# mims-harvard/SubGNN

Measured on AMD Instinct MI355X. Metric: subgraphs/sec fwd+bwd (all 3 channels on) + achieved HBM GB/s, higher is better.
Workload: dtype f32; 1 GPU; synthetic DENSITY-style BA base graph n=1000000 m=10 (9998512 undirected edges), 50000 BFS subgraphs x 20 nodes per GPU (weak form; BASELINE configs[3] "50k sharded across 8" as worded is --scaling strong), all_density hparams (N 10/43, P 57/183, S 42, 1 layer), D=64, full pass = sampling + similarities + fwd + bwd + Adam; subgraphs_per_gpu=50000, subgraphs_total=50000

## Files before the change

### include/subgnn_hip.h

```cpp
#ifndef SUBGNN_HIP_H
#define SUBGNN_HIP_H

#include <stdint.h>

#ifdef __cplusplus
extern "C" {
#endif

#define SGNN_OK                  0
#define SGNN_ERR_BAD_ARG        -1
#define SGNN_ERR_SET_TOO_LARGE  -2
#define SGNN_ERR_NNZ_TOO_LARGE  -3
#define SGNN_ERR_LAUNCH         -4
#define SGNN_ERR_UNSUPPORTED_D  -5

#define SGNN_ABI_VERSION 12
int sgnn_abi_version(void);
int sgnn_warm_up(void* stream);
const char* sgnn_last_error(void);

int sgnn_degree_sequence(const int64_t* rowptr, const int32_t* col, int64_t nnz,
                         const int32_t* full_degree, const uint8_t* self_loops,
                         const int64_t* set_ptr, const int32_t* set_nodes, int64_t n_sets,
                         int64_t max_set_size, int sorted,
// ... 25 lines not shown
                   int32_t* out_nodes, int32_t* out_pos, void* stream);
int sgnn_cc_compact_stats(const int64_t* sub_ptr, const int32_t* sub_nodes, const int32_t* labels,
                          int64_t n_subgraphs, int64_t max_sub_len, int32_t* out_n_components,
                          int32_t* out_longest, void* stream);
int sgnn_cc_compact(const int64_t* sub_ptr, const int32_t* sub_nodes, const int32_t* labels,
                    int64_t n_subgraphs, int64_t max_sub_len, int64_t C, int64_t L, int64_t* out, void* stream);
int64_t sgnn_cc_huge_workspace_bytes(int64_t total_nodes);
int sgnn_cc_labels_huge(const int64_t* rowptr, const int32_t* col, int64_t nnz, const int64_t* sub_ptr,
                        const int32_t* sub_nodes, int64_t n_subgraphs, int64_t total_nodes, int32_t* out_label,
                        void* workspace, int64_t workspace_bytes, void* stream);
int sgnn_cc_compact_huge(const int64_t* sub_ptr, const int32_t* sub_nodes, const int32_t* labels,
                         int64_t n_subgraphs, int64_t total_nodes, int write, int64_t C, int64_t L,
                         int32_t* out_n_components, int32_t* out_longest, int64_t* out, void* workspace,
                         int64_t workspace_bytes, void* stream);

int64_t sgnn_subgraph_properties_workspace_bytes(int64_t total_nodes);
int sgnn_subgraph_properties(const int64_t* rowptr, const int32_t* col_sorted, int64_t nnz, int64_t max_id, int rows_simple,
                             const int64_t* sub_ptr, const int32_t* sub_nodes, int64_t n_sets, int64_t max_len,
                             int64_t total_nodes, int64_t* out_counts, int32_t* out_core, void* workspace,
                             int64_t workspace_bytes, void* stream);

int64_t sgnn_khop_border_workspace_bytes(int64_t max_id, int64_t n_sets, int bitmap_in_lds);
int sgnn_khop_border_bitmap_fits_lds(int64_t max_id);
int sgnn_khop_border(const int64_t* rowptr, const int32_t* col, int64_t nnz, int64_t max_id,
                     const int64_t* set_ptr, const int32_t* set_nodes, int64_t n_sets,
                     int k, int ego_dict_mode,
                     int64_t* out_count, const int64_t* out_ptr, int32_t* out_nodes, uint8_t* out_hop,
                     void* workspace, int64_t workspace_bytes, int bitmap_in_lds, void* stream);
int sgnn_khop_border_arena(const int64_t* rowptr, const int32_t* col, int64_t nnz, int64_t max_id,
                           const int64_t* set_ptr, const int32_t* set_nodes, int64_t n_sets, int k,
                           const int64_t* arena_off, int32_t* arena, int64_t* out_count,
                           void* workspace, int64_t workspace_bytes, int bitmap_in_lds, void* stream);
int64_t sgnn_khop_border_sample_workspace_bytes(int64_t max_id, int64_t n_sets, int k, int rows_sorted, int bitmap_in_lds);
int sgnn_khop_border_sample(const int64_t* rowptr, const int32_t* col, const int32_t* col_sorted, int64_t nnz, int64_t max_id,
                            const int64_t* set_ptr, const int32_t* set_nodes, int64_t n_sets, int k,
                            int64_t n_slots, uint64_t seed, uint64_t stream_id, int64_t item_base,
                            int64_t* out_anchor, uint8_t* out_hop, uint8_t* out_allneg, int64_t* out_count,
                            const int32_t* set_order ,
                            void* workspace, int64_t workspace_bytes, int bitmap_in_lds, void* stream);
int sgnn_khop_sample_finish(int64_t* anchor, const uint8_t* hop, const uint8_t* allneg, const int64_t* counts,
                            const int64_t* width, int64_t n_sets, int64_t n_slots, float* sims, void* stream);
int sgnn_khop1_border_sorted(const int64_t* rowptr, const int32_t* col, const int32_t* col_sorted, int64_t nnz, int64_t max_id,
                             const int64_t* set_ptr, const int32_t* set_nodes, int64_t n_sets,
                             int64_t* out_count, const int64_t* out_ptr , int32_t* out_ids ,
                             void* workspace, int64_t workspace_bytes, int bitmap_in_lds, void* stream);

int sgnn_first_occurrence_mask(const int64_t* ids, int64_t n_rows, int64_t row_len, uint8_t* keep, void* stream);
int sgnn_filter_sets(const int64_t* set_ptr, const int32_t* set_nodes, const uint8_t* flags, int64_t n_sets, int64_t* counts,
                     const int64_t* out_ptr, int32_t* out_nodes, void* stream);
int sgnn_pack_rows_count(const int64_t* ids, const uint8_t* mask, int64_t n_rows, int64_t row_len, int64_t* counts,
                         void* stream);
int sgnn_pack_rows_write(const int64_t* ids, const uint8_t* mask, int64_t n_rows, int64_t row_len, const int64_t* ptr,
                         int32_t* nodes, void* stream);
int64_t sgnn_pack_fused_max_rows(void);
int64_t sgnn_pack_fused_max_entries(void);
int sgnn_pack_rows_fused(const int64_t* ids, const uint8_t* mask, int mode, int64_t n_rows, int64_t row_len, int64_t* ptr,
                         int32_t* nodes, void* stream);
int sgnn_filter_sets_fused(const int64_t* set_ptr, const int32_t* set_nodes, const uint8_t* flags, int64_t n_sets,
                           int64_t arena_entries, int64_t* out_ptr, int32_t* out_nodes, void* stream);

int sgnn_sample_anchors_padded(const int64_t* ids, int64_t n_rows, int64_t L, int64_t n_slots,
                               uint64_t seed, uint64_t stream_id, int64_t* out, void* stream);
int sgnn_sample_anchors_ragged(const int64_t* set_ptr, const int32_t* set_nodes, int64_t n_sets,
                               const uint8_t* row_has_pad, int64_t n_slots,
                               uint64_t seed, uint64_t stream_id, int64_t item_base, int64_t* out, void* stream);
int sgnn_sample_border_anchors(const int64_t* ptr, const int32_t* ids, const int64_t* counts, int64_t n_sets,
                               const int64_t* width, int64_t n_slots, uint64_t seed, uint64_t stream_id, int64_t item_base,
                               int hop, int64_t* out_anchor, float* out_sims, void* stream);

int sgnn_choice_ragged(const int64_t* ptr, const int32_t* seq, int64_t n_items, int64_t n_draws,
                       uint64_t seed, uint64_t stream_id, int64_t item_base, int64_t* out, void* stream);

int sgnn_set_keys(const int64_t* set_ptr, const int32_t* set_nodes, int64_t n_sets, uint64_t* out_keys, void* stream);
int sgnn_sample_anchors_ragged_keyed(const int64_t* set_ptr, const int32_t* set_nodes, int64_t n_sets,
                                     const uint8_t* row_has_pad, const uint64_t* keys, int64_t n_slots,
                                     uint64_t seed, uint64_t stream_id, int64_t* out, void* stream);
int sgnn_choice_ragged_keyed(const int64_t* ptr, const int32_t* seq, int64_t n_items, const uint64_t* keys, int64_t n_draws,
                             uint64_t seed, uint64_t stream_id, int64_t* out, void* stream);
int sgnn_sample_border_anchors_keyed(const int64_t* ptr, const int32_t* ids, const uint8_t* hops, int64_t n_sets,
                                     const uint8_t* row_has_pad, const uint64_t* keys, int64_t n_slots, uint64_t seed,
                                     uint64_t stream_id, int64_t* out_anchor, float* out_sims, void* stream);

#define SGNN_OCC_NODE 0
#define SGNN_OCC_COMPONENT 1
int64_t sgnn_occlusion_lds_max(void);
int64_t sgnn_occlusion_workspace_bytes(int64_t total_entries);
int sgnn_occlusion_count(const int64_t* set_ptr, const int32_t* set_nodes, int64_t n_sets, int64_t max_set_len, int mode,
                         const int32_t* labels, int64_t* out_units, int64_t* out_variants, int64_t* out_len,
                         int64_t total_entries, void* workspace, int64_t workspace_bytes, void* stream);
int sgnn_occlusion_write(const int64_t* set_ptr, const int32_t* set_nodes, int64_t n_sets, int64_t max_set_len, int mode,
                         const int32_t* labels, const int64_t* var_ptr, const int64_t* len_scan, int64_t n_variants,
                         int64_t* out_ptr, int32_t* out_nodes, int32_t* out_parent, int32_t* out_unit, uint64_t* out_keys,
                         int64_t total_entries, void* workspace, int64_t workspace_bytes, void* stream);

int sgnn_triangular_walks(const int64_t* rowptr, const int32_t* col, const int32_t* col_sorted, int64_t nnz,
                          const int32_t* node_order, int64_t n_nodes,
                          const int64_t* patch_ptr, const int32_t* patch_nodes,
                          const int64_t* inb_ptr, const int32_t* inb_nodes,
                          int mode, int64_t n_items, int64_t walks_per_patch, int64_t walk_len, double beta,
                          uint64_t seed, uint64_t stream_id, int64_t item_base, int64_t max_id, int kernel, int64_t* out,
                          void* stream);
int sgnn_triangular_walks_both(const int64_t* rowptr, const int32_t* col, const int32_t* col_sorted, int64_t nnz,
                               const int64_t* patch_ptr, const int32_t* patch_nodes, const int64_t* inb_ptr,
                               const int32_t* inb_nodes, int64_t n_items, int64_t walks_per_patch, int64_t walk_len,
                               double beta, uint64_t seed, uint64_t stream_id_int, uint64_t stream_id_bor,
                               int64_t item_base, int64_t max_id, int64_t* out, void* stream);

int sgnn_patch_in_border(const int64_t* rowptr, const int32_t* col, int64_t nnz,
                         const int32_t* node_order, const int32_t* node_pos, int64_t n_nodes,
                         const int64_t* patch_ptr, const int32_t* patch_nodes, int64_t n_patches,
                         uint8_t* out_flag, void* stream);
int64_t sgnn_patch_in_border_huge_workspace_bytes(int64_t total_nodes);
int sgnn_patch_in_border_huge(const int64_t* rowptr, const int32_t* col, int64_t nnz,
                              const int32_t* node_order, const int32_t* node_pos, int64_t n_nodes,
                              const int64_t* patch_ptr, const int32_t* patch_nodes, int64_t n_patches,
                              int64_t total_nodes, uint8_t* out_flag, void* workspace, int64_t workspace_bytes,
                              void* stream);

int sgnn_sp_similarity_dense(const double* apsp, int64_t n_cols,
                             const int64_t* set_ptr, const int32_t* set_nodes, int64_t n_sets,
                             float* out, void* stream);
int64_t sgnn_bfs_hops_workspace_bytes(int64_t max_id, int64_t n_sources, int max_hops);
int sgnn_bfs_hops(const int64_t* rowptr, const int32_t* col, int64_t nnz, int64_t max_id,
                  const int32_t* sources, int64_t n_sources, int max_hops, int node_major, int pull_alpha,
                  uint8_t* dist, void* workspace, int64_t workspace_bytes, void* stream);
int sgnn_min_hops_to_sets(const uint8_t* dist, int64_t n_sources, int64_t max_id, int node_major,
                          const int64_t* set_ptr, const int32_t* set_nodes, int64_t n_sets,
                          float* out, void* stream);
int64_t sgnn_bfs_min_hops_workspace_bytes(int64_t max_id, int64_t n_sources, int max_hops, int64_t n_sets);
int sgnn_bfs_min_hops_to_sets(const int64_t* rowptr, const int32_t* col, int64_t nnz, int64_t max_id,
                              const int32_t* sources, int64_t n_sources, int max_hops, int pull_alpha, int push_levels,
                              const int64_t* set_ptr, const int32_t* set_nodes, int64_t n_sets,
                              float* out, int32_t* out_status, void* workspace, int64_t workspace_bytes, void* stream);
int64_t sgnn_graph_component_labels_workspace_bytes(int64_t max_id);
int sgnn_graph_component_labels(const int64_t* rowptr, const int32_t* col, int64_t nnz, int64_t max_id,
                                int32_t* labels, void* workspace, int64_t workspace_bytes, void* stream);
int64_t sgnn_bfs_min_hops_closing_workspace_bytes(int64_t max_id, int64_t n_sources, int max_hops, int64_t n_sets);
int sgnn_bfs_min_hops_to_sets_closing(const int64_t* rowptr, const int32_t* col, int64_t nnz, int64_t max_id,
                                      const int32_t* sources, int64_t n_sources, int max_hops, int pull_alpha, int push_levels,
                                      const int32_t* labels, const int64_t* set_ptr, const int32_t* set_nodes,
                                      int64_t n_sets, float* out, int32_t* out_status, void* workspace, int64_t workspace_bytes,
                                      void* stream);

int sgnn_dtw_order_keys(const int64_t* x_ptr, const int32_t* x_val, int64_t n_x, int64_t* out_keys, void* stream);
int64_t sgnn_dtw_workspace_bytes(int64_t n_x, int64_t max_x_len, int64_t n_y, int64_t max_y_len);
int sgnn_dtw_similarity(const int64_t* x_ptr, const int32_t* x_val, int64_t n_x, int64_t max_x_len,
                        const int64_t* y_ptr, const int32_t* y_val, int64_t n_y, int64_t max_y_len,
                        int tie_order, int kernel, const int32_t* x_order, float* out, void* workspace,
                        int64_t workspace_bytes, void* stream);
int sgnn_dtw_similarity_live(const int64_t* x_ptr, const int32_t* x_val, int64_t n_x, int64_t max_x_len,
                             const int64_t* y_ptr, const int32_t* y_val, int64_t n_y, int64_t max_y_len,
                             int tie_order, int kernel, const int32_t* x_order, const int64_t* x_live_range, float* out,
                             void* workspace, int64_t workspace_bytes, void* stream);

int64_t sgnn_dtw_exact_workspace_bytes(int64_t n_x, int64_t max_x_len, int64_t n_y, int64_t max_y_len);
int sgnn_dtw_exact_similarity(const int64_t* x_ptr, const int32_t* x_val, int64_t n_x, int64_t max_x_len,
                              const int64_t* y_ptr, const int32_t* y_val, int64_t n_y, int64_t max_y_len,
                              int kernel, const int32_t* x_order, float* out, void* workspace,
                              int64_t workspace_bytes, void* stream);
int sgnn_dtw_exact_similarity_live(const int64_t* x_ptr, const int32_t* x_val, int64_t n_x, int64_t max_x_len,
                                   const int64_t* y_ptr, const int32_t* y_val, int64_t n_y, int64_t max_y_len,
                                   int kernel, const int32_t* x_order, const int64_t* x_live_range, float* out,
                                   void* workspace, int64_t workspace_bytes, void* stream);

#define SGNN_TOPK_DOT    0
#define SGNN_TOPK_COSINE 1
#define SGNN_TOPK_L2     2
int64_t sgnn_topk_max_k(void);
int64_t sgnn_topk_rows_workspace_bytes(int64_t Q, int64_t N, int64_t k, int64_t splits);
int sgnn_topk_rows(const float* q, int64_t q_stride, int64_t Q, const float* bank, int64_t b_stride, int64_t N,
                   int64_t D, int64_t k, int metric, const float* q_aux, const float* b_aux, const int64_t* exclude,
                   int64_t splits, float* out_score, int64_t* out_index, void* workspace, int64_t workspace_bytes,
                   void* stream);

int sgnn_cc_embed_fwd(const float* E, int64_t D,
                      const int64_t* set_ptr, const int32_t* set_nodes, int64_t n_sets,
                      int aggregator, int64_t padded_len, float* out, int32_t* out_arg, void* stream);
int sgnn_cc_embed_fwd_f16(const uint16_t* E_half, int64_t D,
                          const int64_t* set_ptr, const int32_t* set_nodes, int64_t n_sets,
                          int aggregator, int64_t padded_len, float* out, int32_t* out_arg, void* stream);
int sgnn_cc_embed_bwd(const float* grad_out, int64_t D,
                      const int64_t* set_ptr, const int32_t* set_nodes, int64_t n_sets,
                      int aggregator, const int32_t* arg, float* grad_E, void* stream);

#define SGNN_SRC_DENSE  0
#define SGNN_SRC_GATHER 1
#define SGNN_SRC_SHARED 2

typedef struct sgnn_mpn_args {
    int32_t src;
    int32_t sims_per_edge;
    int64_t R, A, D;
    const float*   x;
    const int64_t* ids;
    int64_t        id_div;
    const uint8_t* edge_mask;
    const uint8_t* row_mask;
    const float*   sims;
    int64_t        sims_ld;
    const int64_t* sim_col;
    const float*   wp;
    const float*   bp;
    int32_t        x_f16;
    const float*   z_act;
    int32_t        flags;
} sgnn_mpn_args;
#define SGNN_MPN_WP_PARTIAL 1
#define SGNN_MPN_RELU_Z     2

int sgnn_mpn_fwd_chunks(const sgnn_mpn_args* args);
int sgnn_mpn_fwd(const sgnn_mpn_args* args, float* agg , float* z , void* stream);
int64_t sgnn_mpn_fwd_many_max_bodies(void);
int sgnn_mpn_fwd_many(int64_t n, const sgnn_mpn_args* args, float* const* agg, float* const* z, void* stream);
int sgnn_mpn_bwd(const sgnn_mpn_args* args, const float* grad_agg, const float* grad_z,
                 float* grad_x, float* grad_wp, void* stream);

int sgnn_attn_scores_epilogue(const float* XU, const float* qW, const float* v, int64_t R, int64_t H,
                              int64_t rows_per_batch, float* out, void* stream);
int64_t sgnn_attn_scores_f16_workspace_bytes(int64_t H);
int sgnn_attn_scores_fwd_f16(const float* X, const float* U, const float* qW, const float* v,
                             int64_t R, int64_t H, int64_t rows_per_batch, float* out,
                             void* workspace, int64_t workspace_bytes, void* stream);

int sgnn_lstm_supported(int64_t hidden_size);
int sgnn_lstm_fwd(const float* pre_x, const float* whh_f, const float* whh_r, const float* bhh_f, const float* bhh_r,
                  int64_t B, int64_t T, int64_t hidden_size, float* y, float* gates, float* cell, float* hprev, void* stream);
int sgnn_lstm_bwd(const float* whh_f, const float* whh_r, const float* gates, const float* cell, const float* dy,
                  int64_t B, int64_t T, int64_t hidden_size, float* dgates, void* stream);

int sgnn_rows_gemm(const float* X, const int64_t* ids, int64_t ldx, int64_t R, int64_t K, const float* W0, const float* W1,
                   const float* b0, const float* b1, int64_t N, float* out, float* x_copy, void* stream);
int sgnn_rows_gemm_nt(const float* A, int64_t R, int64_t K, const float* W0, const float* W1, int64_t N, float* out, void* stream);
int sgnn_lstm_tail_fwd(const float* y, int64_t n_patches, int64_t n_walks, int64_t T, int64_t H2, int last_only,
                       const float* W_lin, const float* b_lin, int64_t D, float* s_out, float* X, void* stream);
int sgnn_lstm_tail_bwd(const float* dX, const float* s, int64_t n_patches, int64_t n_walks, int64_t T, int64_t H2,
                       int last_only, const float* W_lin, int64_t D, float* dy, float* dW_lin, float* db_lin, void* stream);

int sgnn_masked_sum_fwd(const float* x, const uint8_t* mask, int64_t B, int64_t C, int64_t H,
                        float* out, void* stream);
int sgnn_masked_sum_bwd(const float* grad_out, const uint8_t* mask, int64_t B, int64_t C, int64_t H,
                        float* grad_x, void* stream);

int sgnn_masked_sum_slot_fwd(const float* x, const uint8_t* mask, int64_t B, int64_t C, int64_t W, float* out,
                             int64_t out_ld, void* stream);
int sgnn_masked_sum_slot_bwd(const float* grad_out, int64_t grad_ld, const uint8_t* mask, int64_t B, int64_t C,
                             int64_t W, float* grad_x, void* stream);
int sgnn_masked_sum_slots_fwd(const float* const* xs, const int64_t* widths, const int64_t* offsets, int64_t n_pieces,
                              const uint8_t* mask, int64_t B, int64_t C, float* out, int64_t out_ld, void* stream);
int sgnn_masked_sum_slots_bwd(const float* grad_out, int64_t grad_ld, const uint8_t* mask, int64_t B, int64_t C,
                              float* const* grad_xs, const int64_t* widths, const int64_t* offsets, int64_t n_pieces, void* stream);

int64_t sgnn_cross_entropy_workspace_bytes(int64_t B);
int sgnn_cross_entropy_fwd(const float* logits, const int64_t* labels, int64_t B, int64_t K, float* lse, float* loss,
                           float* accuracy, void* workspace, int64_t workspace_bytes, void* stream);
int sgnn_cross_entropy_bwd(const float* logits, const int64_t* labels, const float* lse, const float* grad_loss,
                           int64_t B, int64_t K, float* grad_logits, void* stream);

int64_t sgnn_bce_logits_workspace_bytes(int64_t B);
int sgnn_bce_logits_fwd(const float* logits, const int64_t* targets, int64_t B, int64_t K, float* loss, float* accuracy,
                        void* workspace, int64_t workspace_bytes, void* stream);
int sgnn_bce_logits_bwd(const float* logits, const int64_t* targets, const float* grad_loss, int64_t B, int64_t K,
                        float* grad_logits, void* stream);

int64_t sgnn_column_sum_workspace_bytes(int64_t R, int64_t A);
int sgnn_column_sum(const float* x, int64_t ld, int64_t R, int64_t A, float* out, void* workspace, int64_t workspace_bytes,
                    void* stream);

int sgnn_readout_sum_fwd(const float* sims, int64_t sims_ld, const int64_t* sim_col, const float* s, const float* bp,
                         const uint8_t* row_mask, int64_t B, int64_t C, int64_t A, float* out, int64_t out_ld,
                         void* stream);
int64_t sgnn_readout_sum_bwd_workspace_bytes(int64_t B, int64_t C, int64_t A);
int sgnn_readout_sum_bwd(const float* grad_out, int64_t grad_ld, const float* sims, int64_t sims_ld,
                         const int64_t* sim_col, const float* s, const float* bp, const uint8_t* row_mask, int64_t B,
                         int64_t C, int64_t A, float* grad_s, float* grad_bp, void* workspace, int64_t workspace_bytes,
                         void* stream);

int64_t sgnn_readout_many_max(void);
int sgnn_readout_many_fwd(int64_t n, const float* const* sims, const int64_t* sims_ld, const int64_t* const* sim_col,
                          const float* const* X, const float* const* wp, const float* const* bp,
                          const int64_t* const* ids, const uint8_t* const* row_mask, float* const* s, const int64_t* A,
                          const int64_t* off, int64_t D, int64_t B, int64_t C, float* out, int64_t out_ld, void* stream);
int64_t sgnn_readout_many_bwd_workspace_bytes(int64_t n, const int64_t* A, int64_t B, int64_t C);
int sgnn_readout_many_bwd(int64_t n, const float* grad_out, int64_t grad_ld, const float* const* sims, const int64_t* sims_ld,
                          const int64_t* const* sim_col, const float* const* X, const float* const* wp,
                          const float* const* bp, const int64_t* const* ids, const uint8_t* const* row_mask,
                          float* const* s, const int64_t* A, const int64_t* off, int64_t D, int64_t B, int64_t C,
                          float* const* grad_X, float* const* grad_wp, float* const* grad_bp, void* workspace,
                          int64_t workspace_bytes, unsigned* tickets, void* stream);

int64_t sgnn_scatter_add_rows_workspace_bytes(int64_t n_edges, int64_t D);
int64_t sgnn_sort_edges_by_key_workspace_bytes(int64_t n_edges, int64_t max_key);
int sgnn_sort_edges_by_key(const int32_t* keys, int64_t n_edges, int64_t max_key, int32_t* key_sorted, int32_t* order,
                           void* workspace, int64_t workspace_bytes, void* stream);
int sgnn_scatter_add_rows_sorted(const int32_t* order, const int32_t* key_sorted, int64_t n_edges,
                                 const int32_t* edge_row, int64_t edges_per_row,
                                 const float* G, int64_t D, const float* c1, const float* c2, const float* v,
                                 const int32_t* arg, float* table,
                                 void* workspace, int64_t workspace_bytes, void* stream);
int64_t sgnn_scatter_add_rows_multi_workspace_bytes(int64_t total_edges, int64_t D, int64_t max_key);
int sgnn_scatter_add_rows_multi(int64_t n_lists, const int32_t* const* keys, const int64_t* n_edges,
                                const int32_t* const* edge_row, const int64_t* edges_per_row, const float* const* G,
                                const float* const* c1, const float* const* c2, const float* const* v, int64_t D,
                                int64_t max_key, float* table, void* workspace, int64_t workspace_bytes, void* stream);
int64_t sgnn_mpn_bwd_shared_det_workspace_bytes(int64_t R, int64_t A, int64_t D);
int sgnn_mpn_bwd_shared_det(const struct sgnn_mpn_args* args, const float* grad_agg, const float* grad_z,
                            float* grad_x, float* grad_wp, float* grad_bp, void* workspace, int64_t workspace_bytes,
                            void* stream);
int sgnn_mpn_bwd_edges(const struct sgnn_mpn_args* args, const float* grad_z, int32_t* out_keys, float* out_c1,
                       float* out_c2, void* stream);
int sgnn_mpn_bwd_wp_partial(const struct sgnn_mpn_args* args, const float* grad_z, float* partial, int64_t partial_ld,
                            void* stream);
int sgnn_mpn_bwd_edges_many(int64_t n, const struct sgnn_mpn_args* args, const float* const* grad_z, int32_t* const* out_keys,
                            float* const* out_c1, float* const* out_c2, void* stream);

int sgnn_update_fwd(const float* x, const float* aggr, const float* W, const float* b, int64_t R, int64_t D,
                    float* out, void* stream);
// ... 88 lines not shown
```

### subgnn_amd/SubGNN.py

```python
import json
import os
from pathlib import Path

import numpy as np
import torch
import torch.nn as nn
import torch.nn.functional as F
from torch.nn.parameter import Parameter

from . import config, gamma, ops, subgraph_utils
from . import anchor_patch_samplers as aps
from .datasets import SubgraphDataset
from .graph import load_graph
from .subgraph_mpn import SG_MPN

CHANNELS = (('neighborhood', 'N', 'use_neighborhood', 'neighborhood_mpns'),
            ('position', 'P', 'use_position', 'position_mpns'),
            ('structure', 'S', 'use_structure', 'structure_mpns'))
CC_SLOTS = ('N_I', 'N_B', 'S_I', 'S_B', 'P_I', 'P_B')


class LSTM(nn.Module):

    def __init__(self, n_features, h, dropout=0.0, num_layers=1, batch_first=True, aggregator='last'):
# ... 4 lines not shown
        self.lstm = nn.LSTM(n_features, h, num_layers=num_layers, batch_first=batch_first, dropout=dropout,
                            bidirectional=True)
        self.linear = nn.Linear(h * 2, n_features)

    def _fused(self, input):
        m = self.lstm
        out = input
        for l in range(self.num_layers):
            params = [getattr(m, '%s_l%d%s' % (n, l, sfx)) for sfx in ('', '_reverse')
                      for n in ('weight_ih', 'weight_hh', 'bias_ih', 'bias_hh')]
            out = ops.bilstm_layer(out, params)
            if l < self.num_layers - 1 and m.dropout > 0 and self.training:
                out = nn.functional.dropout(out, m.dropout, True)
        return out

    def forward_walks(self, table, walk_ids, n_walks):
        m = self.lstm
        if not (table.is_cuda and table.dtype == torch.float32 and m.batch_first and m.bias and walk_ids.dim() == 2
                and getattr(table, '_sgnn_half', None) is None and table.shape[1] == m.input_size
                and ops.lstm_fused_supported(m.input_size, m.hidden_size) and walk_ids.shape[0] % n_walks == 0):
            return None
        out = None
        for l in range(self.num_layers):
            params = [getattr(m, '%s_l%d%s' % (n, l, sfx)) for sfx in ('', '_reverse')
                      for n in ('weight_ih', 'weight_hh', 'bias_ih', 'bias_hh')]
            out = ops.bilstm_layer_fused(table, params, ids=walk_ids) if l == 0 else ops.bilstm_layer_fused(out, params)
            if l < self.num_layers - 1 and m.dropout > 0 and self.training:
                out = nn.functional.dropout(out, m.dropout, True)
        return ops.lstm_tail(out, self.linear.weight, self.linear.bias, n_walks, self.aggregator == 'last')

    def forward(self, input):
        m = self.lstm
        if (input.is_cuda and input.dtype == torch.float32 and m.batch_first and m.bias and input.dim() == 3
                and ops.lstm_supported(m.input_size, m.hidden_size)):
            out = self._fused(input)
        else:
            out, _ = m(input)
        agg = out[:, -1, :] if self.aggregator == 'last' else out.sum(dim=1)
        return self.linear(agg)


class _DeviceLoader:

    def __init__(self, model, split, batch_size, shuffle, drop_last):
        self.m, self.split, self.bs, self.shuffle, self.drop_last = model, split, batch_size, shuffle, drop_last
        self.n = len(getattr(model, split + '_sub_G'))

    def __len__(self):
        return self.n // self.bs if self.drop_last else (self.n + self.bs - 1) // self.bs

    def index_batches(self):
        order = torch.randperm(self.n) if self.shuffle else torch.arange(self.n)
        for i in range(len(self)):
            yield order[i * self.bs:(i + 1) * self.bs]

    def __iter__(self):
        for idx in self.index_batches():
            yield self.m.make_batch(self.split, idx)


def _save_npy(fname, arr):
    fname = Path(fname)
    tmp = fname.with_name('.%s.%d.tmp' % (fname.name, os.getpid()))
    try:
        with open(tmp, 'wb') as f:
            np.save(f, arr)
        os.replace(tmp, fname)
    finally:
        if tmp.exists():
            tmp.unlink()


class SubGNN(nn.Module):
    def __init__(self, hparams, graph_path, subgraph_path, embedding_path, similarities_path, shortest_paths_path,
                 degree_dict_path, ego_graph_path, _memory=None):
        super().__init__()
        self._memory = _memory
        self.device = torch.device('cuda' if torch.cuda.is_available() else 'cpu')
        self.hparams = hparams
        self.graph_path, self.subgraph_path, self.embedding_path = graph_path, subgraph_path, embedding_path
        self.similarities_path = Path(similarities_path)
        self.shortest_paths_path, self.degree_dict_path, self.ego_graph_path = \
            shortest_paths_path, degree_dict_path, ego_graph_path
        self.read_data()

        hp = self.hparams
        D, nl = hp['node_embed_size'], hp['n_layers']
        hid_dim = D
        for channel, tag, flag, attr in CHANNELS:
            layers = nn.ModuleList()
            if hp[flag]:
                if tag == 'N':
                    hid_dim += nl * 2 * D
                elif tag == 'P':
                    hid_dim += (hp['n_anchor_patches_pos_in'] + hp['n_anchor_patches_pos_out']) * nl
                else:
                    hid_dim += 2 * hp['n_anchor_patches_structure'] * nl
                for _ in range(nl):
                    layer = nn.ModuleDict({'internal': SG_MPN(hp), 'border': SG_MPN(hp)})
                    if hp.get('batch_norm', False):
                        layer['batch_norm'] = nn.BatchNorm1d(D)
                        layer['batch_norm_out'] = nn.BatchNorm1d(D)
                    layers.append(layer)
            setattr(self, attr, layers)
        self.hid_dim = hid_dim
        self.lin = nn.Linear(hid_dim, hp['linear_hidden_dim_1'])
        self.lin2 = nn.Linear(hp['linear_hidden_dim_1'], hp['linear_hidden_dim_2'])
        self.lin3 = nn.Linear(hp['linear_hidden_dim_2'], self.num_classes)
        self.lin_dropout = nn.Dropout(p=hp['lin_dropout'])
        self.lin_dropout2 = nn.Dropout(p=hp['lin_dropout'])
        self.loss = nn.BCEWithLogitsLoss() if self.multilabel else nn.CrossEntropyLoss()
        self.lstm = LSTM(D, D, dropout=hp['lstm_dropout'], num_layers=hp['lstm_n_layers'],
                         aggregator=hp['lstm_aggregator'])
        if hp.get('ff_attn', False):
            from .attention import AdditiveAttention
            self.attn_vector = Parameter(torch.zeros((hid_dim, 1), dtype=torch.float))
            nn.init.xavier_uniform_(self.attn_vector)
            self.attention = AdditiveAttention(hid_dim, hid_dim, half_operands=str(hp.get('embedding_dtype', 'fp32')).lower()
                                               in ('fp16', 'float16', 'half'))
        hp.setdefault('structure_similarity_fn', 'dtw')
        hp.setdefault('dtw_tie_order', config.DTW_TIE_ORDER)
        if hp['dtw_tie_order'] not in (0, 1, 2):
            raise ValueError("hparams['dtw_tie_order'] must be 0, 1 or 2")
        self._deterministic = bool(hp.get('deterministic', True))
        self.metric_scores = []
        self.to(self.device)
        self.warm_up_s = ops.warm_up(self.device) if (self.device.type == 'cuda' and hp.get('warm_up', True)) else 0.0

    def read_data(self):
        if self._memory is not None:
            return self._read_memory(self._memory)
        root = Path(config.PROJECT_ROOT)
        self.networkx_graph = load_graph(root / self.graph_path, self.device, root / self.degree_dict_path)
        (self.train_sub_G, self.train_sub_G_label, self.val_sub_G, self.val_sub_G_label, self.test_sub_G,
         self.test_sub_G_label) = subgraph_utils.read_subgraphs(root / self.subgraph_path)
        self.multilabel = isinstance(self.train_sub_G_label, list)
        self.multilabel_binarizer = None
        if self.multilabel:
            from sklearn.preprocessing import MultiLabelBinarizer
            self.multilabel_binarizer = MultiLabelBinarizer().fit(
                self.train_sub_G_label + self.val_sub_G_label + self.test_sub_G_label)
        if self.hparams.get('subset_data', False):
            bs = self.hparams['batch_size']
            for sp in ('train', 'val', 'test'):
                setattr(self, sp + '_sub_G', getattr(self, sp + '_sub_G')[:bs])
                setattr(self, sp + '_sub_G_label', getattr(self, sp + '_sub_G_label')[:bs])
        if self.multilabel:
            self.num_classes = max(max(l) for l in self.train_sub_G_label + self.val_sub_G_label + self.test_sub_G_label) + 1
        else:
            self.num_classes = int(torch.max(torch.cat((self.train_sub_G_label.view(-1), self.val_sub_G_label.view(-1),
                                                        self.test_sub_G_label.view(-1))))) + 1
        for sp in ('train', 'val', 'test'):
            setattr(self, sp + '_sub_G', [[n + 1 for n in sg] for sg in getattr(self, sp + '_sub_G')])
        pre = torch.load(root / self.embedding_path, map_location='cpu')
        self.hparams['node_embed_size'] = pre.shape[1]
        table = torch.cat((torch.zeros(1, pre.shape[1]), pre.float()), 0)
        self.node_embeddings = nn.Embedding.from_pretrained(table, freeze=self.hparams['freeze_node_embeds'],
                                                            padding_idx=config.PAD_VALUE)

    def _read_memory(self, mem):
        self.networkx_graph = mem['graph']
        for sp in ('train', 'val', 'test'):
            setattr(self, sp + '_sub_G', mem['sub_G'].get(sp, []))
            setattr(self, sp + '_sub_G_label', mem['labels'].get(sp, torch.zeros(0, dtype=torch.int64)))
        self.multilabel, self.multilabel_binarizer = False, None
        self.num_classes = mem.get('num_classes') or int(max(int(l.max()) for l in mem['labels'].values() if l.numel() > 0)) + 1
        pre = mem['embeddings']
        self.hparams['node_embed_size'] = pre.shape[1]
        table = torch.cat((torch.zeros(1, pre.shape[1], device=pre.device), pre.float()), 0)
        self.node_embeddings = nn.Embedding.from_pretrained(table, freeze=self.hparams['freeze_node_embeds'],
                                                            padding_idx=config.PAD_VALUE)

    @classmethod
    def from_memory(cls, hparams, graph, sub_G, labels, embeddings, num_classes=None):
        return cls(hparams, None, None, None, 'similarities', None, None, None,
                   _memory=dict(graph=graph, sub_G=sub_G, labels=labels, embeddings=embeddings, num_classes=num_classes))

    def initialize_cc_ids(self, subgraph_ids):
        subs = ops.Ragged.from_lists(subgraph_ids, self.device)
        labels = ops.cc_labels(self.networkx_graph, subs)
        return subgraph_utils.components_from_labels(subs.ptr, subs.nodes, labels, subs.max_len)

    def _half_table(self):
        if str(self.hparams.get('embedding_dtype', 'fp32')).lower() not in ('fp16', 'float16', 'half'):
            return None
        w = self.node_embeddings.weight
        st = self.__dict__.get('_half_state')
        if st is None or st[1].device != w.device or st[1].shape != w.shape:
            st = self.__dict__['_half_state'] = [None, torch.empty(w.shape, dtype=torch.float16, device=w.device), True]
        capturing = w.is_cuda and torch.cuda.is_current_stream_capturing()
        training_read = torch.is_grad_enabled() and w.requires_grad
        if st[2] or st[0] != w._version or capturing or training_read:
            st[1].copy_(w.detach())
            st[0] = w._version
        st[2] = training_read or capturing
        return st[1]

    def invalidate_half_table(self):
        st = self.__dict__.get('_half_state')
        if st is not None:
            st[2] = True

    def _table(self):
        t = self.__dict__.get('_tapped_table')
        if t is not None:
            return t
        half = self._half_table()
        return self.node_embeddings.weight if half is None else ops.tap_table(self.node_embeddings.weight, half)

    def initialize_cc_embeddings(self, cc_id_list, aggregator='sum'):
        S, C, L = cc_id_list.shape
        ids = getattr(cc_id_list, '_sgnn_ids32', None)
        if ids is None or ids.numel() != S * C * L:
            ids = cc_id_list.to(self.device).reshape(S * C * L).to(torch.int32)
        memo = self.__dict__.setdefault('_fixed_stride_ptr', {})
        ptr = memo.get((S * C, L))
        if ptr is None:
            if len(memo) > 64:
                memo.clear()
            ptr = memo[(S * C, L)] = torch.arange(S * C + 1, dtype=torch.int64, device=self.device) * L
        sets = ops.Ragged(ptr, ids.contiguous() if ids.numel() else torch.zeros(1, dtype=torch.int32, device=self.device),
                          max_len=L)
        pre = getattr(cc_id_list, '_sgnn_member_order', None)
        if pre is not None and pre[0].numel() != ids.numel():
            pre = None
        return ops.cc_embed(self._table(), sets, aggregator, padded_len=0, stride=L, presorted=pre).view(S, C, -1)

    def initialize_channel_embeddings(self, cc_embeddings, trainable=False):
        if trainable:
            return tuple(Parameter(cc_embeddings.detach().clone()) for _ in CC_SLOTS)
        return tuple(cc_embeddings for _ in CC_SLOTS)

    def init_all_embeddings(self, split='all', trainable=False, lazy=False):
        which = {'all': ('train', 'val', 'test'), 'train_val': ('train', 'val')}.get(split, (split,))
        pending = self.__dict__.setdefault('_lazy_cc_embed', set())
        for sp in which:
            if lazy and not (trainable and sp == 'train'):
                for nm in CC_SLOTS:
                    self.__dict__.pop('%s_%s_cc_embed' % (sp, nm), None)
                pending.add(sp)
                continue
            pending.discard(sp)
            with torch.no_grad():
                emb = self.initialize_cc_embeddings(getattr(self, sp + '_cc_ids'), self.hparams['cc_aggregator'])
            six = self.initialize_channel_embeddings(emb, trainable and sp == 'train')
            for nm, t in zip(CC_SLOTS, six):
                setattr(self, '%s_%s_cc_embed' % (sp, nm), t)

    def __getattr__(self, name):
        if name.endswith('_cc_embed'):
            sp = name.split('_', 1)[0]
            if sp in self.__dict__.get('_lazy_cc_embed', ()):
                self.init_all_embeddings(split=sp, trainable=False)
                return self.__dict__[name]
        return super().__getattr__(name)

    def _sim_dir(self):
        d = Path(config.PROJECT_ROOT) / self.similarities_path
        d.mkdir(parents=True, exist_ok=True)
        return d

    def _cached(self, fname, compute, dtype=None):
        if fname.exists() and not self.hparams['compute_similarities']:
            t = torch.from_numpy(np.load(fname, allow_pickle=True))
            return t.to(self.device) if dtype is None else t.to(self.device, dtype)
        t = compute()
        _save_npy(fname, t.detach().cpu().numpy())
        return t

    def initialize_border_sets(self, fname, cc_ids, radius, ego_graph_dict=None):
        t = subgraph_utils.border_sets(self.networkx_graph, cc_ids, radius, ego_dict_mode=ego_graph_dict is not None)
        _save_npy(fname, t.cpu().numpy())
        return t

    def get_border_sets(self, split):
        hp = self.hparams
        need = hp['use_neighborhood'] or (hp['use_structure'] and hp['structure_similarity_fn'] == 'edit_distance')
        splits = ('test',) if split == 'test' else ('train', 'val')
        if not need:
            for sp in splits:
                setattr(self, sp + '_N_border', None)
            return
        ego = (Path(config.PROJECT_ROOT) / self.ego_graph_path).exists()
        for sp in splits:
            f = self._sim_dir() / ('%d_%d_%s_border_set.npy' % (hp['neigh_sample_border_size'], config.PAD_VALUE, sp))
            cc = getattr(self, sp + '_cc_ids')
            setattr(self, sp + '_N_border', self._cached(
                f, lambda: subgraph_utils.border_sets(self.networkx_graph, cc, hp['neigh_sample_border_size'], ego)))

    def compute_shortest_path_similarities(self, fname, shortest_paths, cc_ids):
        S, C, L = cc_ids.shape
        sets = ops.Ragged.from_padded(cc_ids.reshape(S * C, L))
        sims = ops.sp_similarity_dense(shortest_paths, sets).view(S, C, -1)
        _save_npy(fname, sims.cpu().numpy())
        return sims

    def compute_structure_patch_similarities(self, degree_dict, fname, internal, cc_ids, sim_path=None,
                                             dataset_type=None, border_set=None):
        fn = self.hparams['structure_similarity_fn']
        if fn not in ops.DTW_FNS:
            raise NotImplementedError
        S, C, L = cc_ids.shape
        g = self.networkx_graph
        use_dict = g.full_degree is not None
        a_sets, a_seq = gamma.degree_sequences(g, self.structure_anchors, internal, use_dict)
        c_sets, c_seq = gamma.degree_sequences(g, cc_ids.reshape(S * C, L), internal, use_dict)
        sims = gamma.dtw_similarity_matrix(c_sets, c_seq, a_sets, a_seq, self.hparams['dtw_tie_order'], fn=fn).view(S, C, -1)
        _save_npy(fname, sims.cpu().numpy())
        return sims

    def get_similarities(self, split):
        hp = self.hparams
        d = self._sim_dir()
        splits = ('test',) if split == 'test' else ('train', 'val')
        pad = config.PAD_VALUE
        if hp['use_position'] or hp['use_neighborhood']:
            apsp = None
# ... 653 lines not shown
```

### subgnn_amd/_lib.py

```python
import ctypes
import os

_HERE = os.path.dirname(os.path.abspath(__file__))
LIB_PATH = os.path.join(_HERE, 'lib', 'libsubgnn_hip.so')

c_i64 = ctypes.c_int64
c_u64 = ctypes.c_uint64
c_int = ctypes.c_int
c_dbl = ctypes.c_double
c_ptr = ctypes.c_void_p


class MpnArgs(ctypes.Structure):
    _fields_ = [('src', ctypes.c_int32), ('sims_per_edge', ctypes.c_int32),
                ('R', c_i64), ('A', c_i64), ('D', c_i64),
                ('x', c_ptr), ('ids', c_ptr), ('id_div', c_i64), ('edge_mask', c_ptr), ('row_mask', c_ptr),
                ('sims', c_ptr), ('sims_ld', c_i64), ('sim_col', c_ptr), ('wp', c_ptr), ('bp', c_ptr),
                ('x_f16', ctypes.c_int32), ('z_act', c_ptr), ('flags', ctypes.c_int32)]


SIGNATURES = {
    'sgnn_abi_version': (c_int, []),
    'sgnn_warm_up': (c_int, [c_ptr]),
    'sgnn_last_error': (ctypes.c_char_p, []),
    'sgnn_degree_sequence': (c_int, [c_ptr, c_ptr, c_i64, c_ptr, c_ptr, c_ptr, c_ptr, c_i64, c_i64, c_int, c_ptr, c_ptr,
                                     c_ptr, c_ptr]),
    'sgnn_degree_sequence_sorted_rows': (c_int, [c_ptr, c_ptr, c_ptr, c_i64, c_ptr, c_ptr, c_ptr, c_ptr, c_i64, c_i64, c_int,
                                                 c_ptr, c_ptr, c_ptr, c_ptr]),
    'sgnn_degree_sequence_hub_bitmaps': (c_int, [c_ptr, c_ptr, c_ptr, c_i64, c_ptr, c_ptr, c_ptr, c_ptr, c_i64, c_ptr, c_int,
                                                 c_ptr, c_ptr, c_i64, c_i64, c_int, c_ptr, c_ptr, c_ptr, c_ptr]),
    'sgnn_degree_sequence_search_threshold': (c_i64, []),
    'sgnn_cc_embed_fwd_f16': (c_int, [c_ptr, c_i64, c_ptr, c_ptr, c_i64, c_int, c_i64, c_ptr, c_ptr, c_ptr]),
    'sgnn_cc_labels': (c_int, [c_ptr, c_ptr, c_i64, c_ptr, c_ptr, c_i64, c_i64, c_ptr, c_ptr]),
    'sgnn_cc_compact_stats': (c_int, [c_ptr, c_ptr, c_ptr, c_i64, c_i64, c_ptr, c_ptr, c_ptr]),
    'sgnn_cc_compact': (c_int, [c_ptr, c_ptr, c_ptr, c_i64, c_i64, c_i64, c_i64, c_ptr, c_ptr]),
    'sgnn_cc_huge_workspace_bytes': (c_i64, [c_i64]),
    'sgnn_degree_sequence_huge_workspace_bytes': (c_i64, [c_i64]),
    'sgnn_degree_sequence_huge': (c_int, [c_ptr, c_ptr, c_i64, c_ptr, c_ptr, c_ptr, c_i64, c_i64, c_ptr, c_ptr, c_ptr, c_i64, c_ptr]),
    'sgnn_cc_labels_huge': (c_int, [c_ptr, c_ptr, c_i64, c_ptr, c_ptr, c_i64, c_i64, c_ptr, c_ptr, c_i64, c_ptr]),
    'sgnn_cc_compact_huge': (c_int, [c_ptr, c_ptr, c_ptr, c_i64, c_i64, c_int, c_i64, c_i64, c_ptr, c_ptr, c_ptr, c_ptr, c_i64, c_ptr]),
    'sgnn_subgraph_properties_workspace_bytes': (c_i64, [c_i64]),
    'sgnn_subgraph_properties': (c_int, [c_ptr, c_ptr, c_i64, c_i64, c_int, c_ptr, c_ptr, c_i64, c_i64, c_i64, c_ptr, c_ptr, c_ptr, c_i64,
                                         c_ptr]),
    'sgnn_patch_in_border_huge_workspace_bytes': (c_i64, [c_i64]),
    'sgnn_patch_in_border_huge': (c_int, [c_ptr, c_ptr, c_i64, c_ptr, c_ptr, c_i64, c_ptr, c_ptr, c_i64, c_i64, c_ptr, c_ptr, c_i64, c_ptr]),
    'sgnn_sort_sets': (c_int, [c_ptr, c_ptr, c_i64, c_i64, c_ptr, c_ptr, c_ptr]),
    'sgnn_khop_border_workspace_bytes': (c_i64, [c_i64, c_i64, c_int]),
    'sgnn_khop_border_bitmap_fits_lds': (c_int, [c_i64]),
    'sgnn_khop_border': (c_int, [c_ptr, c_ptr, c_i64, c_i64, c_ptr, c_ptr, c_i64, c_int, c_int, c_ptr, c_ptr, c_ptr,
                                 c_ptr, c_ptr, c_i64, c_int, c_ptr]),
    'sgnn_khop_border_arena': (c_int, [c_ptr, c_ptr, c_i64, c_i64, c_ptr, c_ptr, c_i64, c_int, c_ptr, c_ptr, c_ptr, c_ptr,
                                       c_i64, c_int, c_ptr]),
    'sgnn_khop_border_sample_workspace_bytes': (c_i64, [c_i64, c_i64, c_int, c_int, c_int]),
    'sgnn_khop_border_sample': (c_int, [c_ptr, c_ptr, c_ptr, c_i64, c_i64, c_ptr, c_ptr, c_i64, c_int, c_i64, c_u64, c_u64, c_i64,
                                        c_ptr, c_ptr, c_ptr, c_ptr, c_ptr, c_ptr, c_i64, c_int, c_ptr]),
    'sgnn_khop1_border_sorted': (c_int, [c_ptr, c_ptr, c_ptr, c_i64, c_i64, c_ptr, c_ptr, c_i64, c_ptr, c_ptr, c_ptr, c_ptr, c_i64,
                                         c_int, c_ptr]),
    'sgnn_sample_border_anchors': (c_int, [c_ptr, c_ptr, c_ptr, c_i64, c_ptr, c_i64, c_u64, c_u64, c_i64, c_int, c_ptr, c_ptr,
                                           c_ptr]),
    'sgnn_sample_anchors_padded': (c_int, [c_ptr, c_i64, c_i64, c_i64, c_u64, c_u64, c_ptr, c_ptr]),
    'sgnn_sample_anchors_ragged': (c_int, [c_ptr, c_ptr, c_i64, c_ptr, c_i64, c_u64, c_u64, c_i64, c_ptr, c_ptr]),
    'sgnn_choice_ragged': (c_int, [c_ptr, c_ptr, c_i64, c_i64, c_u64, c_u64, c_i64, c_ptr, c_ptr]),
    'sgnn_set_keys': (c_int, [c_ptr, c_ptr, c_i64, c_ptr, c_ptr]),
    'sgnn_occlusion_lds_max': (c_i64, []),
    'sgnn_occlusion_workspace_bytes': (c_i64, [c_i64]),
    'sgnn_occlusion_count': (c_int, [c_ptr, c_ptr, c_i64, c_i64, c_int, c_ptr, c_ptr, c_ptr, c_ptr, c_i64, c_ptr, c_i64, c_ptr]),
    'sgnn_occlusion_write': (c_int, [c_ptr, c_ptr, c_i64, c_i64, c_int, c_ptr, c_ptr, c_ptr, c_i64, c_ptr, c_ptr, c_ptr, c_ptr, c_ptr,
                                     c_i64, c_ptr, c_i64, c_ptr]),
    'sgnn_sample_anchors_ragged_keyed': (c_int, [c_ptr, c_ptr, c_i64, c_ptr, c_ptr, c_i64, c_u64, c_u64, c_ptr, c_ptr]),
    'sgnn_choice_ragged_keyed': (c_int, [c_ptr, c_ptr, c_i64, c_ptr, c_i64, c_u64, c_u64, c_ptr, c_ptr]),
    'sgnn_sample_border_anchors_keyed': (c_int, [c_ptr, c_ptr, c_ptr, c_i64, c_ptr, c_ptr, c_i64, c_u64, c_u64, c_ptr, c_ptr,
                                                 c_ptr]),
    'sgnn_triangular_walks_both': (c_int, [c_ptr, c_ptr, c_ptr, c_i64, c_ptr, c_ptr, c_ptr, c_ptr, c_i64, c_i64, c_i64, c_dbl, c_u64,
                                           c_u64, c_u64, c_i64, c_i64, c_ptr, c_ptr]),
    'sgnn_triangular_walks': (c_int, [c_ptr, c_ptr, c_ptr, c_i64, c_ptr, c_i64, c_ptr, c_ptr, c_ptr, c_ptr, c_int,
                                      c_i64, c_i64, c_i64, c_dbl, c_u64, c_u64, c_i64, c_i64, c_int, c_ptr, c_ptr]),
    'sgnn_patch_in_border': (c_int, [c_ptr, c_ptr, c_i64, c_ptr, c_ptr, c_i64, c_ptr, c_ptr, c_i64, c_ptr, c_ptr]),
    'sgnn_sp_similarity_dense': (c_int, [c_ptr, c_i64, c_ptr, c_ptr, c_i64, c_ptr, c_ptr]),
    'sgnn_bfs_hops_workspace_bytes': (c_i64, [c_i64, c_i64, c_int]),
    'sgnn_bfs_min_hops_workspace_bytes': (c_i64, [c_i64, c_i64, c_int, c_i64]),
    'sgnn_bfs_min_hops_to_sets': (c_int, [c_ptr, c_ptr, c_i64, c_i64, c_ptr, c_i64, c_int, c_int, c_int, c_ptr, c_ptr, c_i64, c_ptr, c_ptr,
                                          c_ptr, c_i64, c_ptr]),
    'sgnn_graph_component_labels_workspace_bytes': (c_i64, [c_i64]),
    'sgnn_graph_component_labels': (c_int, [c_ptr, c_ptr, c_i64, c_i64, c_ptr, c_ptr, c_i64, c_ptr]),
    'sgnn_bfs_min_hops_closing_workspace_bytes': (c_i64, [c_i64, c_i64, c_int, c_i64]),
    'sgnn_bfs_min_hops_to_sets_closing': (c_int, [c_ptr, c_ptr, c_i64, c_i64, c_ptr, c_i64, c_int, c_int, c_int, c_ptr, c_ptr,
                                                  c_ptr, c_i64, c_ptr, c_ptr, c_ptr, c_i64, c_ptr]),
    'sgnn_bfs_hops': (c_int, [c_ptr, c_ptr, c_i64, c_i64, c_ptr, c_i64, c_int, c_int, c_int, c_ptr, c_ptr, c_i64, c_ptr]),
    'sgnn_min_hops_to_sets': (c_int, [c_ptr, c_i64, c_i64, c_int, c_ptr, c_ptr, c_i64, c_ptr, c_ptr]),
    'sgnn_dtw_workspace_bytes': (c_i64, [c_i64, c_i64, c_i64, c_i64]),
    'sgnn_dtw_similarity': (c_int, [c_ptr, c_ptr, c_i64, c_i64, c_ptr, c_ptr, c_i64, c_i64, c_int, c_int, c_ptr, c_ptr, c_ptr,
                                    c_i64, c_ptr]),
    'sgnn_dtw_order_keys': (c_int, [c_ptr, c_ptr, c_i64, c_ptr, c_ptr]),
    'sgnn_dtw_similarity_live': (c_int, [c_ptr, c_ptr, c_i64, c_i64, c_ptr, c_ptr, c_i64, c_i64, c_int, c_int, c_ptr, c_ptr, c_ptr,
                                         c_ptr, c_i64, c_ptr]),
    'sgnn_topk_max_k': (c_i64, []),
    'sgnn_topk_rows_workspace_bytes': (c_i64, [c_i64, c_i64, c_i64, c_i64]),
    'sgnn_topk_rows': (c_int, [c_ptr, c_i64, c_i64, c_ptr, c_i64, c_i64, c_i64, c_i64, c_int, c_ptr, c_ptr, c_ptr, c_i64, c_ptr,
                               c_ptr, c_ptr, c_i64, c_ptr]),
    'sgnn_dtw_exact_workspace_bytes': (c_i64, [c_i64, c_i64, c_i64, c_i64]),
    'sgnn_dtw_exact_similarity': (c_int, [c_ptr, c_ptr, c_i64, c_i64, c_ptr, c_ptr, c_i64, c_i64, c_int, c_ptr, c_ptr, c_ptr,
                                          c_i64, c_ptr]),
    'sgnn_dtw_exact_similarity_live': (c_int, [c_ptr, c_ptr, c_i64, c_i64, c_ptr, c_ptr, c_i64, c_i64, c_int, c_ptr, c_ptr, c_ptr,
                                               c_ptr, c_i64, c_ptr]),
    'sgnn_cc_embed_fwd': (c_int, [c_ptr, c_i64, c_ptr, c_ptr, c_i64, c_int, c_i64, c_ptr, c_ptr, c_ptr]),
    'sgnn_cc_embed_bwd': (c_int, [c_ptr, c_i64, c_ptr, c_ptr, c_i64, c_int, c_ptr, c_ptr, c_ptr]),
    'sgnn_mpn_fwd_chunks': (c_int, [ctypes.POINTER(MpnArgs)]),
    'sgnn_mpn_fwd': (c_int, [ctypes.POINTER(MpnArgs), c_ptr, c_ptr, c_ptr]),
    'sgnn_mpn_fwd_many_max_bodies': (c_i64, []),
    'sgnn_mpn_fwd_many': (c_int, [c_i64, c_ptr, c_ptr, c_ptr, c_ptr]),
    'sgnn_mpn_bwd': (c_int, [ctypes.POINTER(MpnArgs), c_ptr, c_ptr, c_ptr, c_ptr, c_ptr]),
    'sgnn_attn_scores_epilogue': (c_int, [c_ptr, c_ptr, c_ptr, c_i64, c_i64, c_i64, c_ptr, c_ptr]),
    'sgnn_attn_scores_f16_workspace_bytes': (c_i64, [c_i64]),
    'sgnn_attn_scores_fwd_f16': (c_int, [c_ptr, c_ptr, c_ptr, c_ptr, c_i64, c_i64, c_i64, c_ptr, c_ptr, c_i64, c_ptr]),
    'sgnn_lstm_supported': (c_int, [c_i64]),
    'sgnn_lstm_fwd': (c_int, [c_ptr, c_ptr, c_ptr, c_ptr, c_ptr, c_i64, c_i64, c_i64, c_ptr, c_ptr, c_ptr, c_ptr, c_ptr]),
    'sgnn_lstm_bwd': (c_int, [c_ptr, c_ptr, c_ptr, c_ptr, c_ptr, c_i64, c_i64, c_i64, c_ptr, c_ptr]),
    'sgnn_masked_sum_fwd': (c_int, [c_ptr, c_ptr, c_i64, c_i64, c_i64, c_ptr, c_ptr]),
    'sgnn_masked_sum_bwd': (c_int, [c_ptr, c_ptr, c_i64, c_i64, c_i64, c_ptr, c_ptr]),
    'sgnn_masked_sum_slot_fwd': (c_int, [c_ptr, c_ptr, c_i64, c_i64, c_i64, c_ptr, c_i64, c_ptr]),
    'sgnn_masked_sum_slot_bwd': (c_int, [c_ptr, c_i64, c_ptr, c_i64, c_i64, c_i64, c_ptr, c_ptr]),
    'sgnn_masked_sum_slots_fwd': (c_int, [c_ptr, c_ptr, c_ptr, c_i64, c_ptr, c_i64, c_i64, c_ptr, c_i64, c_ptr]),
    'sgnn_masked_sum_slots_bwd': (c_int, [c_ptr, c_i64, c_ptr, c_i64, c_i64, c_ptr, c_ptr, c_ptr, c_i64, c_ptr]),
    'sgnn_readout_sum_fwd': (c_int, [c_ptr, c_i64, c_ptr, c_ptr, c_ptr, c_ptr, c_i64, c_i64, c_i64, c_ptr, c_i64, c_ptr]),
    'sgnn_first_occurrence_mask': (c_int, [c_ptr, c_i64, c_i64, c_ptr, c_ptr]),
    'sgnn_filter_sets': (c_int, [c_ptr, c_ptr, c_ptr, c_i64, c_ptr, c_ptr, c_ptr, c_ptr]),
    'sgnn_pack_rows_count': (c_int, [c_ptr, c_ptr, c_i64, c_i64, c_ptr, c_ptr]),
    'sgnn_pack_rows_write': (c_int, [c_ptr, c_ptr, c_i64, c_i64, c_ptr, c_ptr, c_ptr]),
    'sgnn_pack_fused_max_rows': (c_i64, []),
    'sgnn_pack_fused_max_entries': (c_i64, []),
    'sgnn_pack_rows_fused': (c_int, [c_ptr, c_ptr, c_int, c_i64, c_i64, c_ptr, c_ptr, c_ptr]),
    'sgnn_filter_sets_fused': (c_int, [c_ptr, c_ptr, c_ptr, c_i64, c_i64, c_ptr, c_ptr, c_ptr]),
    'sgnn_khop_sample_finish': (c_int, [c_ptr, c_ptr, c_ptr, c_ptr, c_ptr, c_i64, c_i64, c_ptr, c_ptr]),
    'sgnn_cross_entropy_workspace_bytes': (c_i64, [c_i64]),
    'sgnn_cross_entropy_fwd': (c_int, [c_ptr, c_ptr, c_i64, c_i64, c_ptr, c_ptr, c_ptr, c_ptr, c_i64, c_ptr]),
    'sgnn_cross_entropy_bwd': (c_int, [c_ptr, c_ptr, c_ptr, c_ptr, c_i64, c_i64, c_ptr, c_ptr]),
    'sgnn_bce_logits_workspace_bytes': (c_i64, [c_i64]),
    'sgnn_bce_logits_fwd': (c_int, [c_ptr, c_ptr, c_i64, c_i64, c_ptr, c_ptr, c_ptr, c_i64, c_ptr]),
    'sgnn_bce_logits_bwd': (c_int, [c_ptr, c_ptr, c_ptr, c_i64, c_i64, c_ptr, c_ptr]),
    'sgnn_column_sum_workspace_bytes': (c_i64, [c_i64, c_i64]),
    'sgnn_column_sum': (c_int, [c_ptr, c_i64, c_i64, c_i64, c_ptr, c_ptr, c_i64, c_ptr]),
    'sgnn_readout_sum_bwd_workspace_bytes': (c_i64, [c_i64, c_i64, c_i64]),
    'sgnn_readout_sum_bwd': (c_int, [c_ptr, c_i64, c_ptr, c_i64, c_ptr, c_ptr, c_ptr, c_ptr, c_i64, c_i64, c_i64, c_ptr, c_ptr,
                                     c_ptr, c_i64, c_ptr]),
    'sgnn_gather_rows_many_max': (c_i64, []),
    'sgnn_rows_gemm': (c_int, [c_ptr, c_ptr, c_i64, c_i64, c_i64, c_ptr, c_ptr, c_ptr, c_ptr, c_i64, c_ptr, c_ptr, c_ptr]),
    'sgnn_rows_gemm_nt': (c_int, [c_ptr, c_i64, c_i64, c_ptr, c_ptr, c_i64, c_ptr, c_ptr]),
    'sgnn_lstm_tail_fwd': (c_int, [c_ptr, c_i64, c_i64, c_i64, c_i64, c_int, c_ptr, c_ptr, c_i64, c_ptr, c_ptr, c_ptr]),
    'sgnn_lstm_tail_bwd': (c_int, [c_ptr, c_ptr, c_i64, c_i64, c_i64, c_i64, c_int, c_ptr, c_i64, c_ptr, c_ptr, c_ptr, c_ptr]),
    'sgnn_readout_many_max': (c_i64, []),
    'sgnn_readout_many_fwd': (c_int, [c_i64, c_ptr, c_ptr, c_ptr, c_ptr, c_ptr, c_ptr, c_ptr, c_ptr, c_ptr, c_ptr, c_ptr, c_i64, c_i64,
                                      c_i64, c_ptr, c_i64, c_ptr]),
    'sgnn_readout_many_bwd_workspace_bytes': (c_i64, [c_i64, c_ptr, c_i64, c_i64]),
    'sgnn_readout_many_bwd': (c_int, [c_i64, c_ptr, c_i64, c_ptr, c_ptr, c_ptr, c_ptr, c_ptr, c_ptr, c_ptr, c_ptr, c_ptr, c_ptr, c_ptr,
                                      c_i64, c_i64, c_i64, c_ptr, c_ptr, c_ptr, c_ptr, c_i64, c_ptr, c_ptr]),
    'sgnn_gather_rows_many': (c_int, [c_i64, c_ptr, c_ptr, c_ptr, c_ptr, c_ptr, c_i64, c_ptr, c_ptr]),
    'sgnn_head_supported': (c_int, [c_i64, c_i64, c_i64]),
    'sgnn_head_blocks': (c_i64, [c_i64]),
    'sgnn_head_partial_floats': (c_i64, [c_i64, c_i64, c_i64]),
    'sgnn_head_fwd_workspace_bytes': (c_i64, [c_i64]),
    'sgnn_head_fwd': (c_int, [c_ptr, c_i64, c_i64, c_i64, c_i64, c_ptr, c_ptr, c_ptr, c_ptr, c_ptr, ctypes.c_float, c_ptr, c_ptr, c_ptr,
                              c_ptr, c_ptr, c_ptr, c_ptr, c_i64, c_ptr]),
    'sgnn_head_bwd': (c_int, [c_ptr, c_ptr, c_ptr, c_ptr, c_ptr, c_ptr, c_ptr, c_ptr, c_ptr, c_ptr, c_i64, c_i64, c_i64, c_i64,
                              ctypes.c_float, c_ptr, c_ptr, c_ptr]),
    'sgnn_head_fwd_ml': (c_int, [c_ptr, c_i64, c_i64, c_i64, c_i64, c_ptr, c_ptr, c_ptr, c_ptr, c_ptr, ctypes.c_float, c_ptr, c_ptr, c_ptr,
                                 c_ptr, c_ptr, c_ptr, c_i64, c_ptr]),
    'sgnn_head_bwd_ml': (c_int, [c_ptr, c_ptr, c_ptr, c_ptr, c_ptr, c_ptr, c_ptr, c_ptr, c_ptr, c_i64, c_i64, c_i64, c_i64,
                                 ctypes.c_float, c_ptr, c_ptr, c_ptr]),
    'sgnn_contract_rows_max_jobs': (c_i64, []),
    'sgnn_contract_rows_blocks': (c_i64, [c_i64, c_i64, c_i64]),
    'sgnn_contract_rows_partial': (c_int, [c_i64, c_ptr, c_ptr, c_ptr, c_ptr, c_ptr, c_ptr, c_ptr, c_ptr, c_ptr, c_ptr]),
    'sgnn_reduce_partials_max_jobs': (c_i64, []),
    'sgnn_reduce_partials': (c_int, [c_i64, c_ptr, c_ptr, c_ptr, c_ptr, c_ptr]),
    'sgnn_probe_stream_copy': (c_int, [c_ptr, c_ptr, c_i64, c_int, c_ptr]),
    'sgnn_scatter_add_rows_workspace_bytes': (c_i64, [c_i64, c_i64]),
    'sgnn_mpn_bwd_shared_det_workspace_bytes': (c_i64, [c_i64, c_i64, c_i64]),
    'sgnn_mpn_bwd_shared_det': (c_int, [c_ptr, c_ptr, c_ptr, c_ptr, c_ptr, c_ptr, c_ptr, c_i64, c_ptr]),
    'sgnn_adam_step': (c_int, [c_ptr, c_ptr, c_ptr, c_ptr, c_i64, ctypes.c_float, ctypes.c_float, ctypes.c_float, ctypes.c_float,
                               ctypes.c_float, c_i64, c_ptr, c_ptr]),
    'sgnn_optim_partials': (c_i64, [c_ptr, c_i64]),
    'sgnn_optim_sumsq': (c_int, [c_ptr, c_ptr, c_i64, c_ptr, c_ptr, c_ptr, c_ptr]),
    'sgnn_optim_count': (c_int, [c_ptr, c_ptr, c_i64, c_ptr]),
    'sgnn_optim_adam': (c_int, [c_ptr, c_ptr, c_ptr, c_ptr, c_ptr, c_ptr, c_i64, ctypes.c_float, ctypes.c_float, ctypes.c_float,
                                ctypes.c_float, c_ptr, c_ptr, c_ptr, c_ptr, c_ptr, c_ptr, c_i64, ctypes.c_float, c_ptr, c_ptr]),
    'sgnn_optim_adam_lr_table': (c_int, [c_ptr, c_ptr, c_ptr, c_ptr, c_ptr, c_ptr, c_i64, c_ptr, c_i64, ctypes.c_float,
                                         ctypes.c_float, ctypes.c_float, c_ptr, c_ptr, c_ptr, c_ptr, c_ptr, c_ptr, c_i64,
                                         ctypes.c_float, c_ptr, c_ptr]),
    'sgnn_update_fwd': (c_int, [c_ptr, c_ptr, c_ptr, c_ptr, c_i64, c_i64, c_ptr, c_ptr]),
    'sgnn_update_fwd_chunks_max_rows': (c_i64, []),
    'sgnn_update_fwd_chunks': (c_int, [c_ptr, c_ptr, c_i64, c_ptr, c_ptr, c_i64, c_i64, c_ptr, c_ptr, c_ptr]),
    'sgnn_update_many_max_bodies': (c_i64, []),
    'sgnn_update_fwd_many': (c_int, [c_i64, c_ptr, c_ptr, c_ptr, c_ptr, c_ptr, c_i64, c_i64, c_ptr, c_ptr, c_ptr]),
    'sgnn_update_bwd_many': (c_int, [c_i64, c_ptr, c_ptr, c_ptr, c_ptr, c_ptr, c_i64, c_i64, c_ptr, c_ptr, c_ptr, c_ptr, c_ptr, c_i64,
                                     c_ptr]),
    'sgnn_update_bwd_workspace_bytes': (c_i64, [c_i64, c_i64]),
    'sgnn_update_bwd': (c_int, [c_ptr, c_ptr, c_ptr, c_ptr, c_ptr, c_i64, c_i64, c_ptr, c_ptr, c_ptr, c_ptr, c_ptr, c_i64, c_ptr]),
    'sgnn_sort_edges_by_key_workspace_bytes': (c_i64, [c_i64, c_i64]),
    'sgnn_sort_edges_by_key': (c_int, [c_ptr, c_i64, c_i64, c_ptr, c_ptr, c_ptr, c_i64, c_ptr]),
    'sgnn_scatter_add_rows_sorted': (c_int, [c_ptr, c_ptr, c_i64, c_ptr, c_i64, c_ptr, c_i64, c_ptr, c_ptr, c_ptr, c_ptr, c_ptr,
                                             c_ptr, c_i64, c_ptr]),
    'sgnn_scatter_add_rows_multi_workspace_bytes': (c_i64, [c_i64, c_i64, c_i64]),
    'sgnn_scatter_add_rows_multi': (c_int, [c_i64, c_ptr, c_ptr, c_ptr, c_ptr, c_ptr, c_ptr, c_ptr, c_ptr, c_i64, c_i64, c_ptr, c_ptr,
                                            c_i64, c_ptr]),
    'sgnn_mpn_bwd_edges': (c_int, [ctypes.POINTER(MpnArgs), c_ptr, c_ptr, c_ptr, c_ptr, c_ptr]),
    'sgnn_mpn_bwd_edges_many': (c_int, [c_i64, c_ptr, c_ptr, c_ptr, c_ptr, c_ptr, c_ptr]),
    'sgnn_mpn_bwd_wp_partial': (c_int, [ctypes.POINTER(MpnArgs), c_ptr, c_ptr, c_i64, c_ptr]),
    'sgnn_ne_chunk_entries': (c_i64, []),
    'sgnn_ne_aggregate': (c_int, [c_ptr, c_ptr, c_ptr, c_ptr, c_ptr, c_ptr, c_i64, c_i64, c_ptr, c_ptr, c_i64, c_ptr, c_ptr, c_i64,
                                  c_int, ctypes.c_uint32, ctypes.c_float, c_u64, c_u64, c_ptr, c_ptr, c_ptr]),
    'sgnn_ne_relu_drop_bwd': (c_int, [c_ptr, c_ptr, c_ptr, c_i64, ctypes.c_float, c_ptr]),
    'sgnn_ne_negatives': (c_int, [c_ptr, c_ptr, c_i64, c_i64, c_u64, c_u64, c_i64, c_int, c_ptr, c_ptr, c_ptr]),
    'sgnn_ne_link_loss_workspace_bytes': (c_i64, []),
    'sgnn_ne_link_loss': (c_int, [c_ptr, c_i64, c_ptr, c_ptr, c_i64, c_i64, c_ptr, c_ptr, c_ptr, c_ptr, c_i64, c_ptr]),
}

ERRORS = {-1: 'SGNN_ERR_BAD_ARG', -2: 'SGNN_ERR_SET_TOO_LARGE', -3: 'SGNN_ERR_NNZ_TOO_LARGE',
          -4: 'SGNN_ERR_LAUNCH', -5: 'SGNN_ERR_UNSUPPORTED_D'}

_lib = None


class SubgnnHipError(RuntimeError):
    pass


def load():
    global _lib
    if _lib is not None:
        return _lib
    import torch
    if not os.path.exists(LIB_PATH):
        raise SubgnnHipError('libsubgnn_hip.so is missing (%s): build it with `python -m subgnn_amd.build`; '
                             'this package has no CPU fallback' % LIB_PATH)
    lib = ctypes.CDLL(LIB_PATH)
    for name, (res, args) in SIGNATURES.items():
        fn = getattr(lib, name)
        fn.restype = res
        fn.argtypes = args
    if lib.sgnn_abi_version() != 12:
        raise SubgnnHipError('ABI version mismatch')
    _lib = lib
    return lib


def check(rc, what):
    if rc != 0:
        lib = load()
        detail = lib.sgnn_last_error().decode() if rc == -4 else ''
# ... 2 lines not shown
```

### subgnn_amd/csrc/dtw.hip

```cpp
#include "common.h"
#include "dtw_cost.h"
#include <type_traits>
#include <cstdlib>

#define DTW_THREADS 256
#ifndef DTW_BLOCKS
#define DTW_BLOCKS (256 * 2)
#endif
#define DTW_NT ((int64_t)DTW_THREADS * DTW_BLOCKS)
#ifndef DTW_REG_BLOCKS
#define DTW_REG_BLOCKS (256 * 32)
#endif
#define DTW_REG_NT ((int64_t)DTW_THREADS * DTW_REG_BLOCKS)
#define DTW_MAX_LEVELS 16

struct DtwLayout {
    int64_t MX, MY;
    int64_t XL, YL;
    int64_t n_dbl;
    int64_t n_i32;
    int64_t n_dir;
    int64_t xoff[DTW_MAX_LEVELS], yoff[DTW_MAX_LEVELS];
};

// ... 623 lines not shown
#undef DTW2_CELL
#undef DTW2_PAIR
#undef DTW2_COLUMN
    if constexpr (!ROW_MAJOR) {
        if (!act) return;
        DTW_BACKTRACE_CELLS(false)
    } else {
#ifndef DTW_PROBE_NO_BACKTRACK
        int j = act ? ly - 1 : -1;
#pragma unroll
        for (int i = RR - 1; i >= 0; --i) {
            const uint32_t h = hull[i >> 1];
            const int uhi = (int)(h & 0xffffu) - 1, ulo = 0x7fff - (int)(h >> 16);
            if (i < lx && j >= 0) {
                const int pos = uhi - j;
                const uint32_t valid = (uhi - ulo + 1) >= 32 ? ~0u : ((1u << (uhi - ulo + 1)) - 1u);
                const uint32_t A = mA[i], B = mB[i];
                const uint32_t is_left = (TIE == 0 ? (~A & B) : (~A & ~B)) & valid;
                const uint32_t tl = (pos >= 0 && pos < 32) ? (is_left >> pos) : 0u;
                int run = __ffs((int)~tl) - 1;
                if (run < 0) run = 32;
                if (run > j) run = j;
                const int first = j - run;
                FLQ(i) = (j << 16) | first;
                const int p2 = pos + run;
                const uint32_t a2 = (p2 >= 0 && p2 < 32) ? ((A >> p2) & 1u) : 0u, b2 = (p2 >= 0 && p2 < 32) ? ((B >> p2) & 1u) : 0u;
                const bool up = TIE == 0 ? (a2 != 0u) : (a2 == 0u && b2 != 0u);
                const bool left_still = TIE == 0 ? (a2 == 0u && b2 != 0u) : (a2 == 0u && b2 == 0u);
                j = left_still ? -1 : (up ? first : first - 1);
            }
        }
#endif
    }
}
#undef FLQ
#undef DTW_LOAD_ROWS
#undef DTW_BACKTRACE_CELLS

template <int RMAX, int TIE, int MINB, bool WLDS>
__global__ __launch_bounds__(DTW_THREADS, MINB) void dtw_similarity_reg_kernel(
    const double* __restrict__ xpyr, const int32_t* __restrict__ xlen, int64_t n_x,
    const double* __restrict__ ypyr, const int32_t* __restrict__ ylen, int64_t n_y,
    float* __restrict__ out, uint32_t* __restrict__ wq, DtwLayout L, const int32_t* __restrict__ x_order,
    const int64_t* __restrict__ x_live)
{
    constexpr int RH = ((RMAX / 2) + 1) & ~1;
    __shared__ int32_t s_fl[RH * DTW_THREADS];
    extern __shared__ uint32_t s_words[];
    int32_t* fl = s_fl + threadIdx.x;
    uint32_t* wl = s_words + threadIdx.x;
    const int64_t NT = (int64_t)gridDim.x * blockDim.x;
    const int64_t tid = blockIdx.x * (int64_t)blockDim.x + threadIdx.x;
    const int lane = threadIdx.x & 63;
    const int64_t first_live = x_live ? x_live[0] : 0;
    const int64_t n_live = x_live ? x_live[1] : n_x;
    const int64_t chunks = (n_live + 63) / 64;
    const int64_t n_tasks = chunks * n_y;
    const int64_t n_waves = NT / 64;
    const int64_t wave0 = __builtin_amdgcn_readfirstlane((int)(tid >> 6));
    for (int64_t task = wave0; task < n_tasks; task += n_waves) {
        const int64_t a = task / chunks;
        const int64_t p0 = first_live + (task - a * chunks) * 64 + lane;
        const bool have = p0 < first_live + n_live;
        const int64_t pos = have ? p0 : first_live;
        const int64_t r = x_order ? x_order[pos] : pos;
        const int ly0 = ylen[a];
        const int lx0 = have ? xlen[pos] : 0;
        const bool valid = have && lx0 > 0 && ly0 > 0;
        int n_levels = 0;
        if (valid) {
            n_levels = 1;
            int lx = lx0, ly = ly0;
            while (lx >= 3 && ly >= 3) { lx >>= 1; ly >>= 1; ++n_levels; }
        }
        const int max_levels = (int)(dtw_wave_pkmax((uint32_t)n_levels) & 0xffff);
        const double* __restrict__ yp = ypyr + a * L.YL;
        double result = 0.0;
        for (int lev = max_levels - 1; lev >= 0; --lev) {
            const bool act = lev < n_levels;
            const int lx = act ? lx0 >> lev : 0, ly = ly0 >> lev;
            const int lxc = lx0 >> (lev + 1), lyc = ly0 >> (lev + 1);
            const double* xcol = xpyr + L.xoff[lev] * n_x + pos;
            const double* xrcol = xcol + L.XL * n_x;
            const double* ycol = yp + L.yoff[lev];
            const double* yrcol = ycol + L.YL * n_y;
            uint32_t* w = wq + (L.yoff[lev] - L.MY) * NT + tid;
            const bool coarsest = lev == n_levels - 1;
#ifdef DTW_PROBE_NO_FINEST
            if (lev == 0) continue;
#endif
#ifdef DTW_PROBE_NO_COARSE
            if (lev != 0) continue;
#endif
            if (lev == 0)
                result = dtw_wave_level<RMAX, TIE, WLDS, true>(fl, xcol, xrcol, n_x, ycol, yrcol, act, lx, ly, lxc, lyc,
                                                               coarsest, wl, w, NT, lev);
            else if constexpr (2 * RH <= 27) {
                if (WLDS && ly <= 32) {
                    constexpr int R2 = (((RMAX >> 2) + 1) & ~1) < 2 ? 2 : (((RMAX >> 2) + 1) & ~1);
                    constexpr int R3 = (((RMAX >> 3) + 1) & ~1) < 2 ? 2 : (((RMAX >> 3) + 1) & ~1);
                    if (lev == 1)
                        dtw_wave_level_2col<RH, TIE, WLDS, true>(fl, xcol, xrcol, n_x, ycol, yrcol, act, lx, ly, lxc, lyc, coarsest, wl, w, NT, lev);
                    else if (lev == 2)
                        dtw_wave_level_2col<R2, TIE, WLDS, true>(fl, xcol, xrcol, n_x, ycol, yrcol, act, lx, ly, lxc, lyc, coarsest, wl, w, NT, lev);
                    else
                        dtw_wave_level_2col<R3, TIE, WLDS, true>(fl, xcol, xrcol, n_x, ycol, yrcol, act, lx, ly, lxc, lyc, coarsest, wl, w, NT, lev);
                }
                else
                    dtw_wave_level_2col<RH, TIE, WLDS, false>(fl, xcol, xrcol, n_x, ycol, yrcol, act, lx, ly, lxc, lyc, coarsest, wl, w, NT, lev);
            }
            else
                dtw_wave_level<RH, TIE, WLDS, false>(fl, xcol, xrcol, n_x, ycol, yrcol, act, lx, ly, lxc, lyc, coarsest,
                                                     wl, w, NT, lev);
        }
        if (have) out[r * n_y + a] = valid ? (float)(1.0 / (result + 1.0)) : 0.f;
    }
}

__global__ void dtw_order_keys_kernel(const int64_t* __restrict__ x_ptr, const int32_t* __restrict__ x_val, int64_t n_x,
                                      int64_t* __restrict__ keys)
{
    const int64_t i = blockIdx.x * (int64_t)blockDim.x + threadIdx.x;
    if (i >= n_x) return;
    const int64_t b = x_ptr[i], len = x_ptr[i + 1] - b;
    int64_t key = (len > 0xFFF ? (int64_t)0xFFF : len) << 48;
#ifndef DTW_KEY_STEPS
#define DTW_KEY_STEPS 4.f
#endif
    auto q8 = [](float v) { const int q = (int)lrintf(DTW_KEY_STEPS * log2f(1.f + (v < 0.f ? 0.f : v))); return (int64_t)(q > 255 ? 255 : q); };
    const int64_t n2 = len / 4;
    if (n2 == 0) {
        for (int64_t f = 0; f < len; ++f) key |= q8((float)x_val[b + f]) << (40 - 8 * f);
    } else {
        const int64_t nf = n2 < 6 ? n2 : 6;
        for (int64_t f = 0; f < nf; ++f) {
            const int64_t g = b + 4 * ((f * n2) / nf);
            const float v = 0.25f * ((float)x_val[g] + (float)x_val[g + 1] + (float)x_val[g + 2] + (float)x_val[g + 3]);
            key |= q8(v) << (40 - 8 * f);
        }
    }
    keys[i] = key;
}

extern "C" int sgnn_dtw_order_keys(const int64_t* x_ptr, const int32_t* x_val, int64_t n_x, int64_t* out_keys, void* stream)
{
    if (!x_ptr || !x_val || !out_keys || n_x < 0) return SGNN_ERR_BAD_ARG;
    if (n_x == 0) return SGNN_OK;
    hipLaunchKernelGGL(dtw_order_keys_kernel, dim3((unsigned)((n_x + 255) / 256)), dim3(256), 0, (hipStream_t)stream, x_ptr,
                       x_val, n_x, out_keys);
    SGNN_CHECK_LAUNCH();
    return SGNN_OK;
}

static int dtw_run(const int64_t* x_ptr, const int32_t* x_val, int64_t n_x, int64_t max_x_len,
                   const int64_t* y_ptr, const int32_t* y_val, int64_t n_y, int64_t max_y_len,
                   int tie_order, int kernel, const int32_t* x_order, const int64_t* x_live, float* out, void* workspace,
                   int64_t workspace_bytes, void* stream)
{
    if (!x_ptr || !x_val || !y_ptr || !y_val || !out || !workspace || n_x < 0 || n_y < 0) return SGNN_ERR_BAD_ARG;
    if (tie_order < 0 || tie_order > 2 || kernel < 0 || kernel > 1) return SGNN_ERR_BAD_ARG;
    if (max_x_len < 1) max_x_len = 1;
    if (max_y_len < 1) max_y_len = 1;
    if (max_x_len > 32767 || max_y_len > 32767) return SGNN_ERR_SET_TOO_LARGE;
    if (workspace_bytes < sgnn_dtw_workspace_bytes(n_x, max_x_len, n_y, max_y_len)) return SGNN_ERR_BAD_ARG;
    if (n_x * n_y == 0) return SGNN_OK;
    const DtwLayout L = dtw_layout(max_x_len, max_y_len);
    hipStream_t st = (hipStream_t)stream;
    char* w = (char*)workspace;
    const int64_t scratch = dtw_scratch_bytes(L);
    double* wd = (double*)w;
    int32_t* wi = (int32_t*)(w + DTW_NT * L.n_dbl * 8);
    uint32_t* wb = (uint32_t*)(w + DTW_NT * (L.n_dbl * 8 + dtw_align8(L.n_i32 * 4)));
    uint32_t* wq = (uint32_t*)w;           w += scratch;
    double* xpyr = (double*)w;             w += 2 * n_x * L.XL * 8;
    double* ypyr = (double*)w;             w += 2 * n_y * L.YL * 8;
    int32_t* xlen = (int32_t*)w;           w += dtw_align8(n_x * 4);
    int32_t* ylen = (int32_t*)w;
    const bool use_reg = max_x_len <= DTW_R && kernel == 0;
    dtw_launch_pyramid(x_ptr, x_val, n_x, max_x_len, L.XL, 1, xpyr, xpyr + n_x * L.XL, xlen,
                       use_reg ? x_order : (const int32_t*)nullptr, st);
    SGNN_CHECK_LAUNCH();
    dtw_launch_pyramid(y_ptr, y_val, n_y, max_y_len, L.YL, 0, ypyr, ypyr + n_y * L.YL, ylen, (const int32_t*)nullptr, st);
    SGNN_CHECK_LAUNCH();
    if (use_reg) {
        const int64_t words = max_y_len >> 1;
        const bool wlds = dtw_words_in_lds(max_y_len);
        size_t dyn = wlds ? (size_t)((words > 0 ? words : 1) * DTW_THREADS * 4) : 0;
#ifdef DTW_PROBE_LDS_PAD
        static const long lds_pad = getenv("SGNN_DTW_LDS_PAD") ? atol(getenv("SGNN_DTW_LDS_PAD")) : 0;
        if (lds_pad > 0) dyn += (size_t)(lds_pad < (long)(48 * 1024 - (long)dyn) ? lds_pad : (48 * 1024 > (long)dyn ? 48 * 1024 - (long)dyn : 0));
#endif
#define DTW_LAUNCH2(RMAX, TIE, MINB, WL) \
        hipLaunchKernelGGL((dtw_similarity_reg_kernel<RMAX, TIE, MINB, WL>), dim3(DTW_REG_BLOCKS), dim3(DTW_THREADS), dyn, st, \
                           xpyr, xlen, n_x, ypyr, ylen, n_y, out, wq, L, x_order, x_live)
#define DTW_LAUNCH(RMAX, TIE, MINB) do { if (wlds) DTW_LAUNCH2(RMAX, TIE, MINB, true); else DTW_LAUNCH2(RMAX, TIE, MINB, false); } while (0)
#define DTW_LAUNCH_T(RMAX, MINB) do { if (tie_order == 0) DTW_LAUNCH(RMAX, 0, MINB); else if (tie_order == 1) DTW_LAUNCH(RMAX, 1, MINB); else DTW_LAUNCH(RMAX, 2, MINB); } while (0)
        if (max_x_len <= 12) DTW_LAUNCH_T(12, DTW_MINB12);
        else if (max_x_len <= 20) DTW_LAUNCH_T(20, DTW_MINB20);
        else DTW_LAUNCH_T(32, DTW_MINB32);
#undef DTW_LAUNCH_T
#undef DTW_LAUNCH2
#undef DTW_LAUNCH
    } else {
        hipLaunchKernelGGL(dtw_similarity_kernel, dim3(DTW_BLOCKS), dim3(DTW_THREADS), 0, st, xpyr, xlen, n_x, ypyr,
                           ylen, n_y, tie_order, out, wd, wi, wb, L);
    }
    SGNN_CHECK_LAUNCH();
    return SGNN_OK;
}

extern "C" int sgnn_dtw_similarity(const int64_t* x_ptr, const int32_t* x_val, int64_t n_x, int64_t max_x_len,
                                   const int64_t* y_ptr, const int32_t* y_val, int64_t n_y, int64_t max_y_len,
                                   int tie_order, int kernel, const int32_t* x_order, float* out, void* workspace,
                                   int64_t workspace_bytes, void* stream)
{
    return dtw_run(x_ptr, x_val, n_x, max_x_len, y_ptr, y_val, n_y, max_y_len, tie_order, kernel, x_order, nullptr, out, workspace,
                   workspace_bytes, stream);
}

extern "C" int sgnn_dtw_similarity_live(const int64_t* x_ptr, const int32_t* x_val, int64_t n_x, int64_t max_x_len,
                                        const int64_t* y_ptr, const int32_t* y_val, int64_t n_y, int64_t max_y_len,
                                        int tie_order, int kernel, const int32_t* x_order, const int64_t* x_live_range,
                                        float* out, void* workspace, int64_t workspace_bytes, void* stream)
{
    if (x_live_range && !x_order) return SGNN_ERR_BAD_ARG;
    return dtw_run(x_ptr, x_val, n_x, max_x_len, y_ptr, y_val, n_y, max_y_len, tie_order, kernel, x_order, x_live_range, out,
                   workspace, workspace_bytes, stream);
}

SGNN_DEFINE_WARM(dtw)
```

### subgnn_amd/csrc/dtw_exact.hip

```cpp
#include "common.h"
#include "dtw_cost.h"

#define DTWX_THREADS 256
#define DTWX_BLOCKS 256
#define DTWX_NT ((int64_t)DTWX_THREADS * DTWX_BLOCKS)
#define DTWX_REG_BLOCKS (256 * 32)
#define DTWX_R 32

static inline int64_t dtwx_align8(int64_t b) { return (b + 7) / 8 * 8; }

extern "C" int64_t sgnn_dtw_exact_workspace_bytes(int64_t n_x, int64_t max_x_len, int64_t n_y, int64_t max_y_len) {
    if (max_x_len < 1) max_x_len = 1;
    if (max_y_len < 1) max_y_len = 1;
    return DTWX_NT * max_x_len * 8
         + 2 * (n_x * max_x_len * 8 + n_y * max_y_len * 8)
         + dtwx_align8(n_x * 4) + dtwx_align8(n_y * 4);
}

__global__ void dtw_exact_prepare_kernel(const int64_t* __restrict__ ptr, const int32_t* __restrict__ val, int64_t n, int64_t M,
                                         int transposed, double* __restrict__ out, double* __restrict__ rec,
                                         int32_t* __restrict__ len_out, const int32_t* __restrict__ order)
{
    const int64_t total = n * M;
    for (int64_t idx = blockIdx.x * (int64_t)blockDim.x + threadIdx.x; idx < total; idx += (int64_t)gridDim.x * blockDim.x) {
        const int64_t s = transposed ? idx % n : idx / M, e = transposed ? idx / n : idx % M;
        const int64_t src = order ? order[s] : s;
        const int64_t b = ptr[src];
        int64_t len = ptr[src + 1] - b;
        if (len > M) len = M;
        if (e == 0) len_out[s] = (int32_t)len;
        if (e < len) {
            const double v1 = (double)val[b + e] + 1.0;
            out[idx] = v1;
            rec[idx] = 1.0 / v1;
        }
    }
}

__global__ __launch_bounds__(DTWX_THREADS) void dtw_exact_kernel(
    const double* __restrict__ xa, const double* __restrict__ xr, const int32_t* __restrict__ xlen, int64_t n_x,
    const double* __restrict__ ya, const double* __restrict__ yr, const int32_t* __restrict__ ylen, int64_t n_y, int64_t MY,
    float* __restrict__ out, double* __restrict__ wd)
{
    const int64_t NT = (int64_t)gridDim.x * blockDim.x;
    const int64_t tid = blockIdx.x * (int64_t)blockDim.x + threadIdx.x;
    const double INF = __longlong_as_double(0x7ff0000000000000ll);
    const int64_t total = n_x * n_y;
    for (int64_t pair = tid; pair < total; pair += NT) {
        const int64_t a = pair / n_x, r = pair % n_x;
        const int lx = xlen[r], ly = ylen[a];
        if (lx == 0 || ly == 0) { out[r * n_y + a] = 0.f; continue; }
        for (int i = 0; i < lx; ++i) wd[(int64_t)i * NT + tid] = INF;
        double up = INF;
        for (int j = 0; j < ly; ++j) {
            const double y1 = ya[a * MY + j], yrc = yr[a * MY + j];
            double diag = j == 0 ? 0.0 : INF;
            up = INF;
            for (int i = 0; i < lx; ++i) {
                const double c = dtw_cost_rcp(xa[(int64_t)i * n_x + r], xr[(int64_t)i * n_x + r], y1, yrc);
                const double old = wd[(int64_t)i * NT + tid];
                up = __dadd_rn(fmin(fmin(old, diag), up), c);
                wd[(int64_t)i * NT + tid] = up;
                diag = old;
            }
        }
        out[r * n_y + a] = (float)(1.0 / (up + 1.0));
    }
}

template <int RMAX, int MINB, bool KEEP>
__global__ __launch_bounds__(DTWX_THREADS, MINB) void dtw_exact_reg_kernel(
    const double* __restrict__ xa, const double* __restrict__ xr, const int32_t* __restrict__ xlen, int64_t n_x,
    const double* __restrict__ ya, const double* __restrict__ yr, const int32_t* __restrict__ ylen, int64_t n_y, int64_t MY,
    float* __restrict__ out, const int32_t* __restrict__ x_order, const int64_t* __restrict__ x_live)
{
    const int64_t NT = (int64_t)gridDim.x * blockDim.x;
    const int64_t tid = blockIdx.x * (int64_t)blockDim.x + threadIdx.x;
    const int lane = threadIdx.x & 63;
    const double INF = __longlong_as_double(0x7ff0000000000000ll);
    const int64_t first_live = x_live ? x_live[0] : 0;
    const int64_t n_live = x_live ? x_live[1] : n_x;
    const int64_t chunks = (n_live + 63) / 64;
    const int64_t n_tasks = chunks * n_y;
    const int64_t n_waves = NT / 64;
    const int64_t wave0 = __builtin_amdgcn_readfirstlane((int)(tid >> 6));
    for (int64_t task = wave0; task < n_tasks; task += n_waves) {
        const int64_t a = task / chunks;
        const int64_t p0 = first_live + (task - a * chunks) * 64 + lane;
        const bool have = p0 < first_live + n_live;
        const int64_t pos = have ? p0 : first_live;
        const int64_t r = x_order ? x_order[pos] : pos;
        const int ly = ylen[a];
        const int lx = have ? xlen[pos] : 0;
        int lxm = lx;
#pragma unroll
        for (int d = 32; d >= 1; d >>= 1) { const int o = __shfl_xor(lxm, d, 64); lxm = o > lxm ? o : lxm; }
        lxm = __builtin_amdgcn_readfirstlane(lxm);
        double x1[RMAX], xrc[RMAX], col[RMAX], cst[KEEP ? RMAX : 1];
#pragma unroll
        for (int i = 0; i < RMAX; ++i) {
            x1[i] = i < lx ? xa[(int64_t)i * n_x + pos] : 1.0;
            xrc[i] = i < lx ? xr[(int64_t)i * n_x + pos] : 1.0;
            col[i] = INF;
        }
        const long long* __restrict__ ybits = reinterpret_cast<const long long*>(ya + a * MY);
        const double* __restrict__ yrow_r = yr + a * MY;
        long long prev_bits = 0;
        for (int j = 0; j < ly; ++j) {
            const long long yb = ybits[j];
            const double y1 = __longlong_as_double(yb), yrc = yrow_r[j];
            if constexpr (KEEP) {
                if (j == 0 || yb != prev_bits) {
#pragma unroll
                    for (int i = 0; i < RMAX; ++i) {
                        if ((i & 1) == 0 && i >= lxm) break;
                        cst[i] = dtw_cost_rcp(x1[i], xrc[i], y1, yrc);
                    }
                }
                prev_bits = yb;
            }
            double diag = j == 0 ? 0.0 : INF, up = INF;
#pragma unroll
            for (int i = 0; i < RMAX; ++i) {
                if ((i & 1) == 0 && i >= lxm) break;
                const double c = KEEP ? cst[KEEP ? i : 0] : dtw_cost_rcp(x1[i], xrc[i], y1, yrc);
                const double old = col[i];
                up = __dadd_rn(fmin(fmin(old, diag), up), c);
                col[i] = up;
                diag = old;
            }
        }
        double result = 0.0;
#pragma unroll
        for (int i = 0; i < RMAX; ++i) result = i == lx - 1 ? col[i] : result;
        if (have) out[r * n_y + a] = (lx > 0 && ly > 0) ? (float)(1.0 / (result + 1.0)) : 0.f;
    }
}

#define DTWX_MINB12 4
#define DTWX_MINB20 2
#define DTWX_MINB32 2

static int dtw_exact_run(const int64_t* x_ptr, const int32_t* x_val, int64_t n_x, int64_t max_x_len,
                         const int64_t* y_ptr, const int32_t* y_val, int64_t n_y, int64_t max_y_len,
                         int kernel, const int32_t* x_order, const int64_t* x_live, float* out, void* workspace,
                         int64_t workspace_bytes, void* stream)
{
    if (!x_ptr || !x_val || !y_ptr || !y_val || !out || !workspace || n_x < 0 || n_y < 0) return SGNN_ERR_BAD_ARG;
    if (kernel < 0 || kernel > 1) return SGNN_ERR_BAD_ARG;
    if (max_x_len < 1) max_x_len = 1;
    if (max_y_len < 1) max_y_len = 1;
    if (max_x_len > 32767 || max_y_len > 32767) return SGNN_ERR_SET_TOO_LARGE;
    if (workspace_bytes < sgnn_dtw_exact_workspace_bytes(n_x, max_x_len, n_y, max_y_len)) return SGNN_ERR_BAD_ARG;
    if (n_x * n_y == 0) return SGNN_OK;
    hipStream_t st = (hipStream_t)stream;
    const int64_t MX = max_x_len, MY = max_y_len;
    char* w = (char*)workspace;
    double* wd = (double*)w;               w += DTWX_NT * MX * 8;
    double* xa = (double*)w;               w += n_x * MX * 8;
    double* xr = (double*)w;               w += n_x * MX * 8;
    double* ya = (double*)w;               w += n_y * MY * 8;
    double* yr = (double*)w;               w += n_y * MY * 8;
    int32_t* xlen = (int32_t*)w;           w += dtwx_align8(n_x * 4);
    int32_t* ylen = (int32_t*)w;
    const bool use_reg = MX <= DTWX_R && kernel == 0;
    hipLaunchKernelGGL(dtw_exact_prepare_kernel, dim3(sgnn_grid_for(n_x * MX, 256)), dim3(256), 0, st, x_ptr, x_val, n_x, MX, 1,
                       xa, xr, xlen, use_reg ? x_order : (const int32_t*)nullptr);
    SGNN_CHECK_LAUNCH();
    hipLaunchKernelGGL(dtw_exact_prepare_kernel, dim3(sgnn_grid_for(n_y * MY, 256)), dim3(256), 0, st, y_ptr, y_val, n_y, MY, 0,
                       ya, yr, ylen, (const int32_t*)nullptr);
    SGNN_CHECK_LAUNCH();
    if (use_reg) {
#define DTWX_LAUNCH(RMAX, MINB, KEEP) \
        hipLaunchKernelGGL((dtw_exact_reg_kernel<RMAX, MINB, KEEP>), dim3(DTWX_REG_BLOCKS), dim3(DTWX_THREADS), 0, st, \
                           xa, xr, xlen, n_x, ya, yr, ylen, n_y, MY, out, x_order, x_live)
        if (MX <= 12) DTWX_LAUNCH(12, DTWX_MINB12, true);
        else if (MX <= 20) DTWX_LAUNCH(20, DTWX_MINB20, true);
        else DTWX_LAUNCH(32, DTWX_MINB32, false);
#undef DTWX_LAUNCH
    } else {
        hipLaunchKernelGGL(dtw_exact_kernel, dim3(DTWX_BLOCKS), dim3(DTWX_THREADS), 0, st, xa, xr, xlen, n_x, ya, yr, ylen, n_y, MY,
                           out, wd);
    }
    SGNN_CHECK_LAUNCH();
    return SGNN_OK;
}

extern "C" int sgnn_dtw_exact_similarity(const int64_t* x_ptr, const int32_t* x_val, int64_t n_x, int64_t max_x_len,
                                         const int64_t* y_ptr, const int32_t* y_val, int64_t n_y, int64_t max_y_len,
                                         int kernel, const int32_t* x_order, float* out, void* workspace,
                                         int64_t workspace_bytes, void* stream)
{
    return dtw_exact_run(x_ptr, x_val, n_x, max_x_len, y_ptr, y_val, n_y, max_y_len, kernel, x_order, nullptr, out, workspace,
                         workspace_bytes, stream);
}

extern "C" int sgnn_dtw_exact_similarity_live(const int64_t* x_ptr, const int32_t* x_val, int64_t n_x, int64_t max_x_len,
                                              const int64_t* y_ptr, const int32_t* y_val, int64_t n_y, int64_t max_y_len,
                                              int kernel, const int32_t* x_order, const int64_t* x_live_range, float* out,
                                              void* workspace, int64_t workspace_bytes, void* stream)
{
    if (x_live_range && !x_order) return SGNN_ERR_BAD_ARG;
    return dtw_exact_run(x_ptr, x_val, n_x, max_x_len, y_ptr, y_val, n_y, max_y_len, kernel, x_order, x_live_range, out,
                         workspace, workspace_bytes, stream);
}

SGNN_DEFINE_WARM(dtw_exact)
```

### subgnn_amd/hotpath.py

```python
import time

import collections

import torch

from . import ops, tape, gamma, subgraph_utils
from .graph_step import record, recording_key
from . import anchor_patch_samplers as aps

MAX_PINT_BYTES = 16 << 30


class StageTimer:

    def __init__(self, enabled=True):
        self.enabled, self.marks, self.host = enabled, [], []

    def mark(self, name):
        if self.enabled:
            e = torch.cuda.Event(enable_timing=True)
            e.record()
            self.marks.append((name, e))
            self.host.append(time.perf_counter())

# ... 67 lines not shown
        last, more, first_pull = status.tolist()[:3]
        model.__dict__.setdefault('_bfs_push_hint', {})[key] = first_pull
        if more:
            raise RuntimeError('position-channel BFS: level %d still reached new nodes -- hparams["max_bfs_hops"] = %d '
                               'is smaller than the depth of this graph from the anchors' % (max_hops, max_hops))
        hint[key] = last
        return
    pool = model.__dict__.setdefault('_bfs_status_pool', [])
    host = pool.pop() if pool else torch.empty(4, dtype=torch.int32).pin_memory()
    host.copy_(status, non_blocking=True)
    ev = torch.cuda.Event()
    ev.record(torch.cuda.current_stream())
    st.bfs_checks.append((key, host, ev, max_hops, enqueued, redo))


class BfsLevelsExhausted(RuntimeError):
    """A recorded pass's hinted position-channel search ran out of levels (the hint has been raised to the cap)."""


def _verify_bfs(model, st, keep=False):
    hint = model.__dict__.setdefault('_bfs_level_hint', {})
    checks = list(st.bfs_checks)
    results = []
    try:
        for key, host, ev, cap, enqueued, redo in checks:
            if ev is not None:
                ev.synchronize()
            results.append((int(host[0]), int(host[1])))
            if int(host[2]) > 0:
                ph = model.__dict__.setdefault('_bfs_push_hint', {})
                ph[key] = max(ph.get(key) or 0, int(host[2]))
    finally:
        if not keep:
            st.bfs_checks = []
            pool = model.__dict__.setdefault('_bfs_status_pool', [])
            for key, host, ev, cap, enqueued, redo in checks:
                if ev is not None:
                    pool.append(host)
    for (key, host, ev, cap, enqueued, redo), (last, more) in zip(checks, results):
        if more and enqueued < cap:
            if redo is None:
                hint[key] = cap
                raise BfsLevelsExhausted(key)
            last, more = redo(cap)[:2]
            model.__dict__['_bfs_redone'] = model.__dict__.get('_bfs_redone', 0) + 1
        if more:
            raise RuntimeError('position-channel BFS: level %d still reached new nodes -- hparams["max_bfs_hops"] = %d '
                               'is smaller than the depth of this graph from the anchors' % (cap, cap))
        hint[key] = max(hint.get(key) or 0, last)


def release_checks(model, checks):
    pool = model.__dict__.setdefault('_bfs_status_pool', [])
    for c in checks:
        if c[1] is not None and not any(c[1] is h for h in pool):
            pool.append(c[1])


def check_pending(model):
    return None


def _pint_sims_streamed(g, uniq, inv, cc_sets, S, C, max_hops, chunk_bytes=1 << 30):
    U = int(uniq.numel())
    rows = S * C
    block = max(64, min(U, (chunk_bytes // (4 * max(rows, 1))) // 64 * 64))
    w = torch.zeros((S, C, inv.shape[1]), dtype=torch.float32, device=inv.device)
    src = uniq.to(torch.int32).contiguous()
    rix = (torch.arange(S, device=inv.device).view(S, 1, 1) * C + torch.arange(C, device=inv.device).view(1, C, 1))
    for a in range(0, U, block):
        b = min(U, a + block)
        part, status = ops.bfs_min_hops_to_sets(g, src[a:b], cc_sets, max_hops=max_hops, want_status=True)
        if int(status[1]):
            raise RuntimeError('position-channel BFS: level %d still reached new nodes -- hparams["max_bfs_hops"] = %d '
                               'is smaller than the depth of this graph from the anchors' % (max_hops, max_hops))
        hit = (inv >= a) & (inv < b)
        col = (inv - a).clamp(0, b - a - 1).view(S, 1, -1).expand(S, C, -1)
        got = part[rix.expand(S, C, inv.shape[1]), col]
        w = torch.where(hit.view(S, 1, -1), got, w)
    return w


def _deal_rows(shard, n, compute, tail_shape, dtype, device, key=None):
    from . import dist as sdist
    per = -(-n // shard.world)
    lo = min(shard.rank * per, n)
    hi = min(lo + per, n)
    part = compute(lo, hi) if hi > lo else torch.zeros((0,) + tuple(tail_shape), dtype=dtype, device=device)
    emu = getattr(shard, 'emulator', None)
    if emu is not None:
        def everybody():
            return torch.cat([compute(min(r * per, n), min(r * per + per, n)) for r in range(shard.world) if min(r * per, n) < n], 0)
        return emu.exchange(key, part, lo, hi, everybody)
    if part.shape[0] < per:
        part = torch.cat([part, part.new_zeros((per - part.shape[0],) + tuple(part.shape[1:]))], 0)
    return sdist.all_gather_rows(part.contiguous(), equal_rows=True)[:n]


def _emulated_position_sims(g, anchors, cc_sets, cc_ids, shard, max_hops, key):
    from . import dist as sdist
    emu = shard.emulator
    S, C, Lc = cc_ids.shape
    A = anchors.numel()
    rows = S * C
    mine = cc_ids.reshape(rows, Lc)
    all_cc = emu.exchange(('cc_ids', key), mine, shard.rank * rows, (shard.rank + 1) * rows, lambda: emu.provided['cc_ids_all'])
    if all_cc.shape[0] != rows * shard.world or all_cc.shape[1] != Lc:
        raise ValueError('EmulatedPeers: the supplied component ids are %s, this rank holds %s of %d ranks' % (tuple(all_cc.shape), (rows, Lc), shard.world))
    all_sets = ops.Ragged.from_padded(all_cc)
    a, b = sdist.shard_range(A, shard.rank, shard.world)
    status = torch.zeros(4, dtype=torch.int32, device=cc_ids.device)
    part = None
    if b > a:
        part, status = ops.bfs_min_hops_to_sets(g, anchors[a:b].to(torch.int32).contiguous(), all_sets, max_hops=max_hops, want_status=True)

    def everybody():
        full, st = ops.bfs_min_hops_to_sets(g, anchors.to(torch.int32).contiguous(), cc_sets, max_hops=max_hops, want_status=True)
        if int(st[1]):
            raise RuntimeError('position-channel BFS: hparams["max_bfs_hops"] = %d is smaller than the depth of this graph' % max_hops)
        return full
    block = part[shard.rank * rows:(shard.rank + 1) * rows] if part is not None else torch.zeros((rows, 0), dtype=torch.float32, device=cc_ids.device)
    return emu.exchange(('P_out', key), block, a, b, everybody, dim=1), status


def _dealt_position_sims(g, anchors, cc_sets, cc_ids, shard, max_hops):
    from . import dist as sdist
    S, C, Lc = cc_ids.shape
    A = anchors.numel()
    all_cc = sdist.all_gather_rows(cc_ids.reshape(S * C, Lc), equal_rows=True)
    all_sets = ops.Ragged.from_padded(all_cc)
    a, b = sdist.shard_range(A, shard.rank, shard.world)
    width = (A + shard.world - 1) // shard.world
    part = torch.zeros((all_sets.n, width), dtype=torch.float32, device=cc_ids.device)
    status = torch.zeros(4, dtype=torch.int32, device=cc_ids.device)
    if b > a:
        part[:, :b - a], status = ops.bfs_min_hops_to_sets(g, anchors[a:b].to(torch.int32).contiguous(), all_sets,
                                                           max_hops=max_hops, want_status=True)
    status = sdist.all_reduce_max_(status)
    got = sdist.all_to_all_row_blocks(part)
    rows = S * C
    cols = [got[j * rows:(j + 1) * rows, :sdist.shard_range(A, j, shard.world)[1] - sdist.shard_range(A, j, shard.world)[0]]
            for j in range(shard.world)]
    return torch.cat(cols, dim=1), status


class PassState:

    def __init__(self, split):
        self.split = split
        self.attrs = {}
        self.per_split = {}
        self.sim_cols = None
        self.dtw_inputs = None
        self.bfs_checks = []
        self.pool_reused = False

    def tensors(self):
        return [self.attrs, self.per_split, self.sim_cols[1] if self.sim_cols else None]


def pool_of(st):
    sp = st.split
    return {'structure_anchors': st.attrs['structure_anchors'],
            'int_w': st.attrs['int_structure_anchor_random_walks'], 'bor_w': st.attrs['bor_structure_anchor_random_walks'],
            'int_sims': st.attrs[sp + '_int_struc_similarities'], 'bor_sims': st.attrs[sp + '_bor_struc_similarities']}


def prepare_pass(model, split='train', timer=None, shard=None, defer_dtw=False, pool=None, epoch=None):
    hp, g, dev = model.hparams, model.networkx_graph, model.device
    if pool is not None and (shard is not None and shard.deal_shared):
        raise ValueError('pool reuse is not combined with the dealt (strong-scaling) form')
    seed = int(hp.get('seed', 0)) & tape.MASK64
    ep = int(model.__dict__.get('_resample_epoch', 0)) if epoch is None else int(epoch)
    st = PassState(split)
    st.pool_reused = pool is not None
    t = timer or StageTimer(False)
    L = hp['n_layers']
    main = torch.cuda.current_stream()
    if hp.get('overlap_streams', True) and (hp.get('overlap_streams_dealt', True) or not (shard is not None and shard.deal_shared)):
        if getattr(model, '_side_stream', None) is None:
            model._side_stream = torch.cuda.Stream()
        side = model._side_stream
    else:
        side = main
    t.mark('start')
    subs = ops.Ragged.from_lists(getattr(model, split + '_sub_G'), dev) if not hasattr(model, '_subs_' + split) \
        else getattr(model, '_subs_' + split)
    setattr(model, '_subs_' + split, subs)
    labels = ops.cc_labels(g, subs)
    kept = model.__dict__.setdefault('_cc_dims', {})
    tag = (id(getattr(model, split + '_sub_G')), subs.n)
    hit = kept.get(split)
    cc_ids = subgraph_utils.components_from_labels(subs.ptr, subs.nodes, labels, subs.max_len,
                                                   dims_reduce=shard.reduce_max if shard is not None else None,
                                                   dims=hit[1] if hit is not None and hit[0] == tag else None)
    kept[split] = (tag, tuple(cc_ids.shape[1:]))
    st.attrs[split + '_cc_ids'] = cc_ids
    S, C, Lc = cc_ids.shape
    if getattr(model, '_deterministic', ops.DETERMINISTIC):
        mo = model.__dict__.setdefault('_cc_member_order', {})
        if mo.get(split) is None or mo[split][0].numel() != cc_ids.numel():
            mo[split] = ops.sort_edges_by_key(cc_ids.reshape(-1).to(torch.int32), g.max_id)
        cc_ids._sgnn_member_order = mo[split]
    cc_ids._sgnn_ids32 = cc_ids.reshape(-1).to(torch.int32)
    base = shard.start if shard is not None else 0
    cc_sets = ops.Ragged.from_padded(cc_ids.reshape(S * C, Lc))
    real = (cc_ids[:, :, 0] != 0)
    cc_ids._sgnn_mask = real
    cc_ids._sgnn_mask_u8 = real.reshape(-1).to(torch.uint8)
    t.mark('components')
    orders = model.__dict__.setdefault('_degseq_order', {})
    if orders.get(split) is None or orders[split].numel() != cc_sets.n:
        orders[split] = ops.heaviest_first(g, cc_sets)
        t.mark('set_dispatch_order(first pass only)')
    set_order = orders[split]
    sims = {}
    a_sets = ai = ae = None
    det = bool(getattr(model, '_deterministic', ops.DETERMINISTIC))
    side.wait_stream(main)
    with torch.cuda.stream(side):
        new_patches = hp['use_structure'] and pool is None and (split != 'test' or getattr(model, 'structure_anchors', None) is None)
        structure_anchors = getattr(model, 'structure_anchors', None) if pool is None else pool['structure_anchors']
        if new_patches:
            if shard is not None and shard.deal_shared and hp['structure_patch_type'] == 'triangular_random_walk':
                n_p = hp['max_sim_epochs'] * hp['n_anchor_patches_structure'] * hp['n_layers']
                structure_anchors = _deal_rows(shard, n_p, lambda lo, hi: aps.sample_structure_anchor_patches(
                    hp, g, dev, hp['max_sim_epochs'], trim=False, share=(lo, hi)), (hp['sample_walk_len'],), torch.int64, dev,
                    key=('S_patches', split))
                st.attrs['structure_anchors'] = structure_anchors
            else:
                structure_anchors = st.attrs['structure_anchors'] = aps.sample_structure_anchor_patches(hp, g, dev, hp['max_sim_epochs'], trim=False)
            if side is main:
                t.mark('S_patches_walks')
        patch_ev = None
        if hp['use_structure'] and side is not main:
            patch_ev = torch.cuda.Event()
            patch_ev.record(side)
        def position_block():
            if hp['use_position']:
                anchors_pos_ext = getattr(model, 'anchors_pos_ext', None)
                if anchors_pos_ext is None or split != 'test':
                    anchors_pos_ext = st.attrs['anchors_pos_ext'] = aps.init_anchors_pos_ext(hp, g, dev, epoch=ep)
                    if det:
                        for v in anchors_pos_ext.values():
                            ops.presort_ids(v, g.max_id)
                pint = {l: ops.choice_ragged(subs, hp['n_anchor_patches_pos_in'], seed,
                                             tape.stream_id(tape.STREAM_P_INT, split, l, ep), item_base=base) for l in range(L)}
                st.per_split['anchors_pos_int'] = pint
                until = _position_until(hp)
                for l in range(L):
                    if shard is not None and shard.deal_shared:
                        cap = hp.get('max_bfs_hops', 32)
                        if getattr(shard, 'emulator', None) is not None:
                            w, status = _emulated_position_sims(g, anchors_pos_ext[l], cc_sets, cc_ids, shard, cap, (split, l))
                        else:
                            w, status = _dealt_position_sims(g, anchors_pos_ext[l], cc_sets, cc_ids, shard, cap)
                        w = w.view(S, C, -1)
                        model.__dict__.setdefault('_bfs_level_hint', {}).setdefault(('P_out_dealt', split, l), 0)
                        _bfs_note(model, st, ('P_out_dealt', split, l), status, cap, cap, None)
                    else:
                        cap = hp.get('max_bfs_hops', 32)
                        nlev = _bfs_levels(model, ('P_out', split, l), cap)
                        src = anchors_pos_ext[l].to(torch.int32).contiguous()
                        w, status = ops.bfs_min_hops_to_sets(g, src, cc_sets, max_hops=nlev, want_status=True,
                                                             push_levels=_bfs_push_levels(model, ('P_out', split, l)), until=until)

                        def redo(levels, src=src, l=l, sims=sims, until=until):
                            _hand_over(torch.cuda.current_stream(), src, cc_sets)
                            w2, st2 = ops.bfs_min_hops_to_sets(g, src, cc_sets, max_hops=levels, want_status=True, until=until)
                            sims[('P', 'out', l)] = w2.view(S, C, -1).contiguous()
                            return st2.tolist()
                        _bfs_note(model, st, ('P_out', split, l), status, cap, nlev, redo)
                        w = w.view(S, C, -1)
                    sims[('P', 'out', l)] = w.contiguous()
                    if C == 1:
                        sims[('P', 'in', l)] = ops.ZeroSims((S, C, hp['n_anchor_patches_pos_in']), dev)
                    else:
                        uniq, inv = torch.unique(pint[l], return_inverse=True)
                        if uniq.numel() * (g.max_id + 1) <= MAX_PINT_BYTES:
                            d = ops.bfs_hops(g, uniq.to(torch.int32).contiguous(), max_hops=hp.get('max_bfs_hops', 32),
                                             node_major=True)
                            full = ops.min_hops_to_sets(d, cc_sets, node_major=True).view(S, C, -1)
                            w = torch.gather(full, 2, inv.view(S, 1, -1).expand(S, C, -1))
                        else:
                            w = _pint_sims_streamed(g, uniq, inv, cc_sets, S, C, hp.get('max_bfs_hops', 32))
                        sims[('P', 'in', l)] = (w * real.unsqueeze(-1)).contiguous()
                if side is main:
                    t.mark('P_bfs_sims')
        late_bfs = bool(hp.get('bfs_beside_dtw', False)) and side is not main and hp['use_structure'] and hp['use_position'] \
            and not defer_dtw and not (shard is not None and shard.deal_shared)
        wos = hp.get('walks_on_side_stream')
        walks_on_side = (bool(wos) if wos is not None else cc_sets.n <= WALKS_ON_SIDE_MAX_SETS) and side is not main and hp['use_structure']

        def structure_walks(degree_sequences=True):
            nonlocal a_sets, ai, ae
            if new_patches and shard is not None and shard.deal_shared:
                W_, T_ = hp['n_triangular_walks'], hp['random_walk_len']

                def both(lo, hi):
                    mine = structure_anchors[lo:hi].contiguous()
                    v = aps.patch_node_views(mine)
                    iw, bw = aps.perform_random_walks_both(hp, g, mine, v, first_patch=lo)
                    return torch.stack([bw, iw], 1)
                walks = _deal_rows(shard, structure_anchors.shape[0], both, (2, W_, T_), torch.int64, dev, key=('S_walks', split))
                bor_w = st.attrs['bor_structure_anchor_random_walks'] = walks[:, 0].contiguous()
                int_w = st.attrs['int_structure_anchor_random_walks'] = walks[:, 1].contiguous()
            elif new_patches:
                views = aps.patch_node_views(structure_anchors)
                int_w, bor_w = aps.perform_random_walks_both(hp, g, structure_anchors, views)
                st.attrs['bor_structure_anchor_random_walks'], st.attrs['int_structure_anchor_random_walks'] = bor_w, int_w
            if pool is not None:
                int_w, bor_w = pool['int_w'], pool['bor_w']
                st.attrs['structure_anchors'] = structure_anchors
                st.attrs['int_structure_anchor_random_walks'], st.attrs['bor_structure_anchor_random_walks'] = int_w, bor_w
            if new_patches or pool is not None:
                a_struct = st.attrs['anchors_structure'] = aps.init_anchors_structure(hp, structure_anchors, int_w, bor_w,
                                                                                      indices_on_device=True, epoch=ep)
                if det:
                    for v in a_struct.values():
                        v[2]._sgnn_both = ops.presort_ids(torch.cat([v[2], v[3]], 0), g.max_id)
                    if L > 1:
                        a_struct[0][2]._sgnn_all = ops.presort_ids(
                            torch.cat([t for l in range(L) for t in (a_struct[l][2], a_struct[l][3])], 0), g.max_id)
                st.sim_cols = (a_struct, model.sim_cols_of(a_struct))
            if pool is not None or not degree_sequences:
                return
            patch_degree_sequences()

        def patch_degree_sequences():
            nonlocal a_sets, ai, ae
            a_sets = ops.Ragged.from_padded(structure_anchors)
            ai, ae = ops.degree_sequence(g, a_sets, sort=True, use_degree_dict=g.full_degree is not None)
        if walks_on_side:
            structure_walks(degree_sequences=False)
        if not late_bfs:
            position_block()
        if hp['use_structure'] and side is main:
            structure_walks()
            t.mark('S_patches_walks')
    if hp['use_neighborhood']:
        k = hp['neigh_sample_border_size']
        has_pad_c = (cc_sets.lengths < Lc).to(torch.uint8)
        cc_canon = ops.sort_ragged(cc_sets)
        ni, nb, plans = {}, {}, {}
        border = _kept_border(model, split, subs, cc_sets, k)
        for l in range(L):
            ni[l] = ops.sample_anchors_ragged(cc_canon, hp['n_anchor_patches_N_in'], seed,
                                              tape.stream_id(tape.STREAM_N_INT, split, l, ep), has_pad_c,
                                              canonical=True, item_base=base * C).view(S, C, -1)
            sims[('N', 'in', l)] = ops.ZeroSims(ni[l].shape, dev)
            widths = model.__dict__.setdefault('_border_width', {})
            wkey = (split, k, cc_sets.n, shard.world if shard is not None else 1)
            if border is not None:
                if wkey not in widths:
                    wmax = border.counts.max().view(1)
                    widths[wkey] = shard.reduce_max(wmax) if shard is not None else wmax
                a, w, counts = ops.draw_border_anchors(border, hp['n_anchor_patches_N_out'], seed,
                                                       tape.stream_id(tape.STREAM_N_BOR, split, l, ep), item_base=base * C,
                                                       width=widths[wkey])
            else:
                a, w, counts = ops.khop_border_sample(g, cc_sets, k, hp['n_anchor_patches_N_out'], seed,
                                                      tape.stream_id(tape.STREAM_N_BOR, split, l, ep),
                                                      item_base=base * C,
                                                      count_reduce=shard.reduce_max if shard is not None else None,
                                                      width=widths.get(wkey))
            if wkey not in widths:
                wmax = counts.max().view(1)
                widths[wkey] = shard.reduce_max(wmax) if shard is not None else wmax
            nb[l] = a.view(S, C, -1)
            sims[('N', 'out', l)] = w.view(S, C, -1).contiguous()
            D = hp['node_embed_size']
            if det and hp.get('fused_forward', True) and D % 4 == 0 and D <= 256 and (D // 4) & (D // 4 - 1) == 0:
                plan = ops.mpn_edge_plan(sims[('N', 'out', l)], nb[l], cc_ids._sgnn_mask_u8, R=S * C,
                                         A=nb[l].shape[-1], D=D, max_key=g.max_id, sims_per_edge=True)
                plan['anchors'] = nb[l]
                plans[('N', False, l)] = plan
        st.per_split['anchors_neigh_int'], st.per_split['anchors_neigh_border'] = ni, nb
        st.per_split['_mpn_edge_plans'] = plans
        t.mark('border_bfs+N_anchors')
    ci = ce = None
    if hp['use_structure'] and pool is None:
        ci, ce = ops.degree_sequence(g, cc_sets, sort=True, use_degree_dict=g.full_degree is not None,
                                     order=set_order)
        t.mark('degree_sequences')
    if hp['use_structure'] and side is not main:
        main.wait_event(patch_ev)
        _hand_over(main, structure_anchors)
        if walks_on_side:
            if pool is None:
                patch_degree_sequences()
            t.mark('S_patch_degree_sequences')
        else:
            structure_walks()
            t.mark('S_walks')
    st.dtw_inputs = (cc_sets, ci, ce, a_sets, ai, ae, (S, C)) if (hp['use_structure'] and pool is None) else None
    if pool is not None and hp['use_structure']:
        st.attrs[split + '_int_struc_similarities'], st.attrs[split + '_bor_struc_similarities'] = pool['int_sims'], pool['bor_sims']
    if late_bfs:
        dtw_ev = torch.cuda.Event()
        dtw_ev.record(main)
        with torch.cuda.stream(side):
            side.wait_event(dtw_ev)
            position_block()
    if not defer_dtw:
        finish_pass(model, st, t)
    if side is not main:
        main.wait_stream(side)
        _hand_over(main, sims, st.attrs.get('anchors_pos_ext'), st.per_split.get('anchors_pos_int'),
                   st.attrs.get('structure_anchors'), st.attrs.get('int_structure_anchor_random_walks'),
                   st.attrs.get('bor_structure_anchor_random_walks'), st.sim_cols[1] if st.sim_cols else None)
        for v in (st.attrs.get('anchors_structure') or {}).values():
            _hand_over(main, v[0], v[2], v[3])
    if side is not main:
        t.mark('side_stream_join(S_patches,P_bfs)')
    st.attrs[split + '_neigh_pos_similarities'] = sims if sims else None
    st.attrs[split + '_N_border'] = None
    return st


KEPT_BORDER_BYTES = 4 << 30


def _kept_border(model, split, subs, cc_sets, k):
    hp, g = model.hparams, model.networkx_graph
    budget = int(hp.get('kept_border_bytes', KEPT_BORDER_BYTES))
    if k != 1 or budget <= 0:
        return None
    kept = model.__dict__.setdefault('_kept_borders', {})
    sub_g = getattr(model, split + '_sub_G')
    tag = (id(sub_g), subs.n, cc_sets.n, id(g), budget)
    rec = kept.get(split)
    if rec is None or rec[0] != tag:
        if torch.cuda.is_current_stream_capturing():
            return None
        border = ops.khop1_borders_sorted(g, cc_sets, max_bytes=budget) if ops.khop1_applies(g, cc_sets.n) else None
        rec = kept[split] = (tag, border, sub_g, g)
    border = rec[1]
    if border is not None:
        border.wait(torch.cuda.current_stream())
    return border


def finish_pass(model, st, timer=None):
    t = timer or StageTimer(False)
    split = st.split
    if st.dtw_inputs is not None:
        cc_sets, ci, ce, a_sets, ai, ae, (S, C) = st.dtw_inputs
        st.dtw_inputs = None
        mx, my = max(cc_sets.max_len, 1), max(a_sets.max_len, 1)
        tie = int(model.hparams['dtw_tie_order'])
        fn = 'dtw_exact' if model.hparams.get('structure_similarity_fn') == 'dtw_exact' else 'dtw'
        group = model.__dict__.setdefault('_dtw_group_rows', {})
        rec = group.get(split)
        if rec is None or rec.n != cc_sets.n:
            rec = group[split] = _DtwRows(cc_sets.n, *(_DtwSide(ops.distinct_rows_async(cc_sets.ptr, x, mx)) for x in (ci, ce)))
            t.mark('dtw_row_grouping_counts_queued(first pass only)')
        elif rec.internal.group is None and not torch.cuda.is_current_stream_capturing():
            _settle_dtw_grouping(model, split, wait=False)
        for name, side, x, y in (('_int', rec.internal, ci, ai), ('_bor', rec.external, ce, ae)):
            sim = ops.dtw_similarity(cc_sets.ptr, x, mx, a_sets.ptr, y, my, tie, dedupe=bool(side.group), x_prep=side.prep, fn=fn)
            st.attrs[split + name + '_struc_similarities'] = sim.view(S, C, -1)
        t.mark('dtw')
    elif split + '_int_struc_similarities' not in st.attrs:
        st.attrs[split + '_int_struc_similarities'] = None
        st.attrs[split + '_bor_struc_similarities'] = None
    return st


class _DtwSide:

    def __init__(self, pending):
        self.group, self.pending, self.prep = None, pending, ops.DtwRowPrep()


_DtwRows = collections.namedtuple('_DtwRows', 'n internal external')


def _settle_dtw_grouping(model, split, wait):
    rec = model.__dict__.get('_dtw_group_rows', {}).get(split)
    if rec is None or rec.internal.group is not None:
        return
    sides = (rec.internal, rec.external)
    fr = [ops.distinct_rows_ready(s.pending, wait=wait) for s in sides]
    if all(f is not None for f in fr):
        for s, f in zip(sides, fr):
            s.group, s.pending, s.prep = f <= 0.5, None, ops.DtwRowPrep()


def install_pass(model, st, timer=None):
    t = timer or StageTimer(False)
    _verify_bfs(model, st)
    for k, v in st.attrs.items():
        setattr(model, k, v)
    for k, v in st.per_split.items():
        d = getattr(model, k, None)
        if d is None:
            d = {}
            setattr(model, k, d)
        d[st.split] = v
    if st.sim_cols is not None:
        model.set_sim_cols(*st.sim_cols)
    model._build_sim_cols()
    if getattr(model, '_table_sync', None) is not None:
        model._table_sync()
        t.mark('table_all_gather_wait')
    model.init_all_embeddings(split=st.split, trainable=model.hparams['trainable_cc'], lazy=True)
    t.mark('cc_embed')
    model.__dict__['_sparse_prepared'] = True
    model._bump_generation()
    return t


def prepare_sparse(model, split='train', timer=None, shard=None):
    t = timer or StageTimer(False)
    install_pass(model, prepare_pass(model, split, t, shard), t)
    return t


class PassPipeline:

    def __init__(self, model, split='train', shard=None, pool_epochs=1):
        self.model, self.split, self.shard = model, split, shard
        self.stream = torch.cuda.Stream()
        self.pending = collections.deque()
        self.timer = None
        self.pool_epochs, self._n_started, self._pool = max(1, int(pool_epochs)), 0, None

    @property
    def state(self):
        return self.pending[0][0] if self.pending else None

    def start(self, timed=False, after=None):
        main = torch.cuda.current_stream()
        if after is not None:
            self.stream.wait_event(after)
        else:
            self.stream.wait_stream(main)
        timer = StageTimer(timed)
        reuse = self._pool if (self.pool_epochs > 1 and self._n_started % self.pool_epochs != 0) else None
        with torch.cuda.stream(self.stream):
            state = prepare_pass(self.model, self.split, timer, self.shard, pool=reuse)
            if reuse is None and self.pool_epochs > 1 and self.model.hparams['use_structure']:
                self._pool = pool_of(state)
            self._n_started += 1
            timer.mark('prepared')
            done = torch.cuda.Event()
            done.record()
        self.pending.append((state, timer, done))

    def install(self, timer=None, installer=None):
        if not self.pending:
            raise RuntimeError('PassPipeline.install without a started pass')
        st, self.timer, done = self.pending.popleft()
        main = torch.cuda.current_stream()
        main.wait_event(done)
        _hand_over(main, *st.tensors())
        for v in (st.attrs.get('anchors_structure') or {}).values():
            _hand_over(main, v[0], v[2], v[3])
        if installer is not None:
            installer(st, timer)
            return timer
        return install_pass(self.model, st, timer)


_TENSOR_ATTRS = ('_sgnn_ids32', '_sgnn_sorted', '_sgnn_both', '_sgnn_all', '_sgnn_member_order', '_sgnn_mask', '_sgnn_mask_u8')


def _copy_into(dst, src, path, replaced, memo=None):
    memo = {} if memo is None else memo
    if isinstance(src, torch.Tensor):
        if isinstance(dst, torch.Tensor) and dst.shape == src.shape and dst.dtype == src.dtype and dst.device == src.device:
            key = (src.data_ptr(), src.numel(), src.dtype, dst.data_ptr())
            if dst.data_ptr() != src.data_ptr() and key not in memo:
                pairs = memo.get('__pairs__')
                if pairs is not None and dst.is_contiguous() and src.is_contiguous():
                    pairs.append((dst, src))
                else:
                    dst.copy_(src)
                memo[key] = True
            for nm in _TENSOR_ATTRS:
                v = getattr(src, nm, None)
                if v is not None:
                    setattr(dst, nm, _copy_into(getattr(dst, nm, None), v, path + '.' + nm, replaced, memo))
            return dst
        replaced.append(path)
        return src
    if isinstance(src, dict):
        if not isinstance(dst, dict):
            replaced.append(path)
            return src
        for k, v in src.items():
            dst[k] = _copy_into(dst.get(k), v, '%s[%r]' % (path, k), replaced, memo)
        return dst
    if isinstance(src, (list, tuple)):
        if not isinstance(dst, (list, tuple)) or len(dst) != len(src):
            replaced.append(path)
            return src
        return type(src)(_copy_into(d, v, '%s[%d]' % (path, i), replaced, memo) for i, (d, v) in enumerate(zip(dst, src)))
    return src


_SHAPE_ONLY = ('structure_anchors', 'anchors_structure', 'int_structure_anchor_random_walks', 'bor_structure_anchor_random_walks')


def install_pass_static(model, st, timer=None):
    t = timer or StageTimer(False)
    _verify_bfs(model, st)
    replaced, memo = [], {'__pairs__': []}
    for k, v in st.attrs.items():
        setattr(model, k, _copy_into(getattr(model, k, None), v, k, replaced, memo))
    for k, v in st.per_split.items():
        d = getattr(model, k, None)
        if d is None:
# ... 217 lines not shown
```

### subgnn_amd/ops.py

```python
import collections
import ctypes
import functools
import threading

import numpy as np
import torch

from . import _lib
from ._lib import MpnArgs, check

PAD = 0


def _ptr(t):
    return None if t is None else ctypes.c_void_p(t.data_ptr())


_RAW_STREAM = getattr(torch._C, '_cuda_getCurrentRawStream', None)
_CUR_DEVICE = getattr(torch._C, '_cuda_getDevice', None)


def _stream():
    if _RAW_STREAM is not None and _CUR_DEVICE is not None:
        return ctypes.c_void_p(_RAW_STREAM(_CUR_DEVICE()))
# ... 788 lines not shown
        out[0] = triangular_walks(g, 1, n_items, walk_len, beta, seed, stream_id_int, patches=patches,
                                  walks_per_patch=walks_per_patch, item_base=item_base)
        out[1] = triangular_walks(g, 2, n_items, walk_len, beta, seed, stream_id_bor, patches=patches, in_border=in_border,
                                  walks_per_patch=walks_per_patch, item_base=item_base)
        return out
    check(rc, 'sgnn_triangular_walks_both')
    return out


def patch_in_border(g, patches):
    lib = _lib.load()
    out = torch.zeros(patches.nodes.numel(), dtype=torch.uint8, device=g.device)
    check(lib.sgnn_patch_in_border(_ptr(g.rowptr), _ptr(g.col), g.nnz, _ptr(g.node_order), _ptr(g.node_pos),
                                   g.n_nodes, _ptr(patches.ptr), _ptr(patches.nodes), patches.n, _ptr(out), _stream()),
          'sgnn_patch_in_border')
    ws, wsb, total = _huge_ws(lib, patches.max_len, lambda: patches.total, g.device, 'sgnn_patch_in_border_huge_workspace_bytes')
    if ws is not None:
        check(lib.sgnn_patch_in_border_huge(_ptr(g.rowptr), _ptr(g.col), g.nnz, _ptr(g.node_order), _ptr(g.node_pos),
                                            g.n_nodes, _ptr(patches.ptr), _ptr(patches.nodes), patches.n, total, _ptr(out),
                                            _ptr(ws), wsb, _stream()), 'sgnn_patch_in_border_huge')
    return out


def sp_similarity_dense(apsp, sets):
    lib = _lib.load()
    _req(apsp, torch.float64, 'apsp')
    n_cols = apsp.shape[1]
    out = torch.empty((sets.n, n_cols), dtype=torch.float32, device=apsp.device)
    check(lib.sgnn_sp_similarity_dense(_ptr(apsp), n_cols, _ptr(sets.ptr), _ptr(sets.nodes), sets.n, _ptr(out),
                                       _stream()), 'sgnn_sp_similarity_dense')
    return out


def probe_stream_copy(src, dst, bytes_per_lane):
    nbytes = src.numel() * src.element_size()
    assert dst.numel() * dst.element_size() == nbytes and src.is_cuda and dst.is_cuda
    check(_lib.load().sgnn_probe_stream_copy(_ptr(src), _ptr(dst), nbytes, int(bytes_per_lane), _stream()),
          'sgnn_probe_stream_copy')


def bfs_hops(g, sources, max_hops=64, node_major=False, pull_alpha=-1):
    lib = _lib.load()
    _req(sources, torch.int32, 'sources')
    ns = sources.numel()
    shape = (g.max_id + 1, ns) if node_major else (ns, g.max_id + 1)
    dist = torch.empty(shape, dtype=torch.uint8, device=g.device)
    wsb = lib.sgnn_bfs_hops_workspace_bytes(g.max_id, ns, max_hops)
    ws = torch.empty(wsb // 8 + 1, dtype=torch.int64, device=g.device)
    check(lib.sgnn_bfs_hops(_ptr(g.rowptr), _ptr(g.col), g.nnz, g.max_id, _ptr(sources), ns, max_hops,
                            1 if node_major else 0, int(pull_alpha), _ptr(dist), _ptr(ws), wsb, _stream()), 'sgnn_bfs_hops')
    return dist


def bfs_min_hops_to_sets(g, sources, sets, max_hops=64, want_status=False, pull_alpha=-1, push_levels=-1, until='nodes'):
    lib = _lib.load()
    _req(sources, torch.int32, 'sources')
    ns = sources.numel()
    out = torch.empty((sets.n, ns), dtype=torch.float32, device=g.device)
    status = torch.zeros(4, dtype=torch.int32, device=g.device) if want_status else None
    if until == 'sets':
        labels = g.component_labels()
        wsb = lib.sgnn_bfs_min_hops_closing_workspace_bytes(g.max_id, ns, max_hops, sets.n)
        ws = torch.empty(wsb // 8 + 1, dtype=torch.int64, device=g.device)
        check(lib.sgnn_bfs_min_hops_to_sets_closing(_ptr(g.rowptr), _ptr(g.col), g.nnz, g.max_id, _ptr(sources), ns, max_hops,
                                                    int(pull_alpha), int(push_levels), _ptr(labels), _ptr(sets.ptr),
                                                    _ptr(sets.nodes), sets.n, _ptr(out), _ptr(status), _ptr(ws), wsb, _stream()),
              'sgnn_bfs_min_hops_to_sets_closing')
        return (out, status) if want_status else out
    if until != 'nodes':
        raise ValueError("until must be 'nodes' or 'sets', not %r" % (until,))
    wsb = lib.sgnn_bfs_min_hops_workspace_bytes(g.max_id, ns, max_hops, sets.n)
    ws = torch.empty(wsb // 8 + 1, dtype=torch.int64, device=g.device)
    check(lib.sgnn_bfs_min_hops_to_sets(_ptr(g.rowptr), _ptr(g.col), g.nnz, g.max_id, _ptr(sources), ns, max_hops,
                                        int(pull_alpha), int(push_levels), _ptr(sets.ptr), _ptr(sets.nodes), sets.n, _ptr(out), _ptr(status), _ptr(ws), wsb,
                                        _stream()), 'sgnn_bfs_min_hops_to_sets')
    return (out, status) if want_status else out


def min_hops_to_sets(dist, sets, node_major=False):
    lib = _lib.load()
    _req(dist, torch.uint8, 'dist')
    if node_major:
        n_ids, ns = dist.shape
    else:
        ns, n_ids = dist.shape
    out = torch.empty((sets.n, ns), dtype=torch.float32, device=dist.device)
    check(lib.sgnn_min_hops_to_sets(_ptr(dist), ns, n_ids - 1, 1 if node_major else 0, _ptr(sets.ptr), _ptr(sets.nodes),
                                    sets.n, _ptr(out), _stream()), 'sgnn_min_hops_to_sets')
    return out


_HASH_COEF = {}


def _row_representatives(rows):
    n, w = rows.shape
    dev = rows.device
    coef = _HASH_COEF.get((w, dev))
    if coef is None:
        g = torch.Generator(device='cpu').manual_seed(0x5DEECE66D)
        coef = _HASH_COEF[(w, dev)] = (torch.randint(-(1 << 62), 1 << 62, (w,), generator=g, dtype=torch.int64) | 1).to(dev)
    h = (rows.to(torch.int64) * coef).sum(dim=1)
    hs, perm = torch.sort(h)
    pos = torch.arange(n, device=dev)
    first = torch.ones(n, dtype=torch.bool, device=dev)
    if n > 1:
        first[1:] = hs[1:] != hs[:-1]
    gid = torch.cumsum(first, 0) - 1
    run_start = torch.empty(n + 1, dtype=torch.int64, device=dev)
    run_start.scatter_(0, torch.where(first, gid, n), pos)
    start = run_start[gid]
    rep = torch.empty(n, dtype=torch.int64, device=dev)
    rep[perm] = perm[start]
    same = (rows.index_select(0, rep) == rows).all(dim=1)
    return torch.where(same, rep, pos)


def _unique_rows(rows):
    rep = _row_representatives(rows)
    is_rep = rep == torch.arange(rows.shape[0], device=rows.device)
    gid = torch.cumsum(is_rep, 0) - 1
    return rows[is_rep], gid[rep]


def distinct_rows_async(x_ptr, x_val, max_x):
    n = x_ptr.numel() - 1
    if n <= 1024 or max_x > 64:
        return None
    rows = Ragged(x_ptr, x_val, max_len=max_x).to_padded(width=max_x, fill=-1, dtype=torch.int32)
    rep = _row_representatives(rows)
    cnt = (rep == torch.arange(n, device=rows.device)).sum().view(1)
    host = torch.empty(1, dtype=torch.int64).pin_memory()
    host.copy_(cnt, non_blocking=True)
    ev = torch.cuda.Event()
    ev.record()
    return host, ev, n


def distinct_rows_ready(pending, wait=False):
    if pending is None:
        return 1.0
    host, ev, n = pending
    if wait:
        ev.synchronize()
    elif not ev.query():
        return None
    return float(int(host[0])) / n


_DTW_ENTRIES = {
    'dtw': ('sgnn_dtw_workspace_bytes', 'sgnn_dtw_similarity', True),
    'dtw_exact': ('sgnn_dtw_exact_workspace_bytes', 'sgnn_dtw_exact_similarity', False),
}
DTW_FNS = tuple(_DTW_ENTRIES)

DtwGrouping = collections.namedtuple('DtwGrouping', 'ptr rep entry_dst live')


class DtwRowPrep:
    __slots__ = ('shape', 'grouping', 'order', 'grouped_order')

    def __init__(self):
        self.shape = self.grouping = self.order = self.grouped_order = None

    def fit(self, x_ptr, x_val):
        shape = (x_ptr.numel() - 1, x_val.numel())
        if shape != self.shape:
            self.shape, self.grouping, self.order, self.grouped_order = shape, None, None, None
        return self


def _group_rows(x_ptr, x_val, max_x, want_live):
    n, spare, dev = x_ptr.numel() - 1, x_val.numel(), x_ptr.device
    rows = Ragged(x_ptr, x_val, max_len=max_x).to_padded(width=max_x, fill=-1, dtype=torch.int32)
    rep = _row_representatives(rows)
    kept = rep == torch.arange(n, device=dev)
    lens = torch.where(kept, x_ptr[1:] - x_ptr[:-1], 0)
    uptr = torch.zeros(n + 1, dtype=torch.int64, device=dev)
    torch.cumsum(lens, 0, out=uptr[1:])
    e = torch.arange(spare, device=dev)
    shift = torch.cat([torch.where(kept, uptr[:-1] - x_ptr[:-1], spare), uptr.new_full((1,), spare)])
    entry_dst = (shift[torch.searchsorted(x_ptr[1:], e, right=True)] + e).clamp_(max=spare)
    live = None
    if want_live:
        n_live = (lens > 0).sum()
        live = torch.stack((n - n_live, n_live))
    return DtwGrouping(uptr, rep, entry_dst, live)


def _dtw_row_order(x_ptr, x_val):
    nx = x_ptr.numel() - 1
    key = torch.empty(nx, dtype=torch.int64, device=x_ptr.device)
    check(_lib.load().sgnn_dtw_order_keys(_ptr(x_ptr), _ptr(x_val), nx, _ptr(key), _stream()), 'sgnn_dtw_order_keys')
    return torch.argsort(key).to(torch.int32).contiguous()


def _dtw_launch(x_ptr, x_val, max_x, y_ptr, y_val, max_y, tie_order, kernel, fn, order, live):
    lib = _lib.load()
    for t, dt, nm in ((x_ptr, torch.int64, 'x_ptr'), (y_ptr, torch.int64, 'y_ptr'), (x_val, torch.int32, 'x_val'),
                      (y_val, torch.int32, 'y_val')):
        _req(t, dt, nm)
    nx, ny = x_ptr.numel() - 1, y_ptr.numel() - 1
    out = (torch.empty if live is None else torch.zeros)((nx, ny), dtype=torch.float32, device=x_ptr.device)
    ws_entry, entry, takes_tie = _DTW_ENTRIES[fn]
    wsb = getattr(lib, ws_entry)(nx, max_x, ny, max_y)
    ws = torch.empty(wsb // 8 + 1, dtype=torch.int64, device=x_ptr.device)
    args = [_ptr(x_ptr), _ptr(x_val), nx, max_x, _ptr(y_ptr), _ptr(y_val), ny, max_y]
    if takes_tie:
        args.append(tie_order)
    args += [int(kernel), _ptr(order)]
    if live is not None and order is not None:
        entry += '_live'
        args.append(_ptr(live))
    check(getattr(lib, entry)(*args, _ptr(out), _ptr(ws), wsb, _stream()), entry)
    return out


def dtw_similarity(x_ptr, x_val, max_x, y_ptr, y_val, max_y, tie_order=None, order_rows=True, dedupe=True, order=None,
                   x_prep=None, kernel=0, fn='dtw'):
    if fn not in DTW_FNS:
        raise ValueError('structure similarity function %r: one of %s' % (fn, ', '.join(map(repr, DTW_FNS))))
    if tie_order is None:
        from .config import DTW_TIE_ORDER as tie_order
    prep = (x_prep if x_prep is not None else DtwRowPrep()).fit(x_ptr, x_val)
    ptr, val, g = x_ptr, x_val, None
    if dedupe and x_ptr.numel() - 1 > 1024 and max_x <= 64:
        g = prep.grouping = prep.grouping or _group_rows(x_ptr, x_val, max_x, order is None and order_rows)
        ptr, val = g.ptr, torch.zeros(x_val.numel() + 1, dtype=torch.int32, device=x_ptr.device)
        val.scatter_(0, g.entry_dst, x_val)
    live = g.live if g is not None and order is None else None
    if order is not None:
        order = order.to(torch.int32).contiguous()
    elif order_rows and ptr.numel() - 1 > 64:
        which = 'order' if g is None else 'grouped_order'
        order = getattr(prep, which)
        if order is None:
            order = _dtw_row_order(ptr, val)
            setattr(prep, which, order)
    out = _dtw_launch(ptr, val, max_x, y_ptr, y_val, max_y, int(tie_order), kernel, fn, order, live)
    return out if g is None else out.index_select(0, g.rep)



DETERMINISTIC = True
_DET_SCOPE = None


class deterministic:

    def __init__(self, flag):
        self.flag = bool(flag)

    def __enter__(self):
        global _DET_SCOPE
        self.old, _DET_SCOPE = _DET_SCOPE, self.flag

    def __exit__(self, *exc):
        global _DET_SCOPE
        _DET_SCOPE = self.old


def _det_now():
    return DETERMINISTIC if _DET_SCOPE is None else _DET_SCOPE


def sort_edges_by_key(keys, max_key):
    lib = _lib.load()
    _req(keys, torch.int32, 'keys')
    E = keys.numel()
    sk, order = torch.empty_like(keys), torch.empty_like(keys)
    if E:
        wsb = lib.sgnn_sort_edges_by_key_workspace_bytes(E, int(max_key))
        if wsb < 0:
            raise RuntimeError('sgnn_sort_edges_by_key_workspace_bytes failed')
        ws = torch.empty(wsb // 8 + 1, dtype=torch.int64, device=keys.device)
        check(lib.sgnn_sort_edges_by_key(_ptr(keys), E, int(max_key), _ptr(sk), _ptr(order), _ptr(ws), wsb, _stream()),
              'sgnn_sort_edges_by_key')
    return sk, order


SCATTER_MAX_D = 256
SCATTER_TOGETHER_BELOW = 1 << 16


def scatter_add_rows(table, keys, G=None, edge_row=None, edges_per_row=1, c1=None, c2=None, v=None, arg=None,
                     presorted=None, together=None):
    lib = _lib.load()
    E = keys.numel()
    if E == 0:
        return table
    _req(keys, torch.int32, 'keys')
    _req(table, torch.float32, 'table')
    for t, nm in ((G, 'G'), (c1, 'c1'), (c2, 'c2'), (v, 'v')):
        _req(t, torch.float32, nm)
    _req(edge_row, torch.int32, 'edge_row')
    _req(arg, torch.int32, 'arg')
    D = table.shape[1]
    if together is not None and presorted is None and arg is None and E < SCATTER_TOGETHER_BELOW and D <= 256 \
            and (G is None or (G.dim() == 2 and G.shape[1] == D and G.is_contiguous())):
        together.jobs.append((keys.reshape(-1), G, edge_row, int(edges_per_row), c1, c2, v))
        return table
    sk, order = presorted if presorted is not None else sort_edges_by_key(keys.reshape(-1), table.shape[0] - 1)
    if sk.numel() != E or order.numel() != E:
        raise ValueError('presorted order does not belong to these keys')
    wsb = lib.sgnn_scatter_add_rows_workspace_bytes(E, D)
    ws = torch.empty(wsb // 4 + 1, dtype=torch.int32, device=table.device)
    check(lib.sgnn_scatter_add_rows_sorted(_ptr(order), _ptr(sk), E, _ptr(edge_row), int(edges_per_row), _ptr(G), D, _ptr(c1),
                                           _ptr(c2), _ptr(v), _ptr(arg), _ptr(table), _ptr(ws), wsb, _stream()),
          'sgnn_scatter_add_rows_sorted')
    return table


class _GradAcc:

    def __init__(self, owner=None):
        self.buf = None
        self.owner = owner
        self.jobs = []
        self.producers = []

    def buffer(self, shape, device):
        if self.buf is None:
            self.buf = take_zeroed(self.owner, shape, device)
        return self.buf

    def flush(self):
        producers, self.producers = self.producers, []
        lib = _lib.load()
        cap = int(lib.sgnn_mpn_fwd_many_max_bodies()) if producers else 1
        for lo in range(0, len(producers), cap):
            group = producers[lo:lo + cap]
            arr = (MpnArgs * len(group))(*[g[0] for g in group])
            pz, pk, p1, p2 = (_ptr_table([g[i] for g in group]) for i in (1, 2, 3, 4))
            check(lib.sgnn_mpn_bwd_edges_many(len(group), ctypes.cast(arr, ctypes.c_void_p), pz.ctypes.data, pk.ctypes.data,
                                              p1.ctypes.data, p2.ctypes.data, _stream()), 'sgnn_mpn_bwd_edges_many')
        jobs, self.jobs = self.jobs, []
        if not jobs:
            return
        if self.owner is None:
            raise RuntimeError('pending table-gradient lists without a table')
        table = self.buffer(tuple(self.owner.shape), jobs[0][0].device)
        if len(jobs) == 1:
            keys, G, edge_row, epr, c1, c2, v = jobs[0]
            scatter_add_rows(table, keys, G=G, edge_row=edge_row, edges_per_row=epr, c1=c1, c2=c2, v=v)
            return
        n = len(jobs)
        D = table.shape[1]

        def ptrs(k):
            return np.array([0 if j[k] is None else j[k].data_ptr() for j in jobs], dtype=np.uint64)
        keys_p, G_p, row_p, c1_p, c2_p, v_p = ptrs(0), ptrs(1), ptrs(2), ptrs(4), ptrs(5), ptrs(6)
        n_edges = np.array([j[0].numel() for j in jobs], dtype=np.int64)
        epr = np.array([j[3] for j in jobs], dtype=np.int64)
        total, max_key = int(n_edges.sum()), table.shape[0] - 1
        wsb = lib.sgnn_scatter_add_rows_multi_workspace_bytes(total, D, max_key)
        ws = torch.empty(wsb // 8 + 1, dtype=torch.int64, device=table.device)
        check(lib.sgnn_scatter_add_rows_multi(n, keys_p.ctypes.data, n_edges.ctypes.data, row_p.ctypes.data, epr.ctypes.data,
                                              G_p.ctypes.data, c1_p.ctypes.data, c2_p.ctypes.data, v_p.ctypes.data, D, max_key,
                                              _ptr(table), _ptr(ws), wsb, _stream()), 'sgnn_scatter_add_rows_multi')


def take_zeroed(owner, shape, device):
    buf = owner.__dict__.pop('_sgnn_zeroed', None) if owner is not None else None
    if buf is not None and tuple(buf.shape) == tuple(shape) and buf.device == torch.device(device):
        return buf
    return torch.zeros(shape, dtype=torch.float32, device=device)


def release_zeroed(owner, buf):
    owner._sgnn_zeroed = buf


def drop_zeroed(owner):
    owner.__dict__.pop('_sgnn_zeroed', None)


class _TableTap(torch.autograd.Function):

    @staticmethod
    def forward(ctx, E, acc):
        ctx.acc = acc
        ctx.set_materialize_grads(False)
        return E.view_as(E)

    @staticmethod
    def backward(ctx, g):
        ctx.acc.flush()
        buf, ctx.acc.buf = ctx.acc.buf, None
        if buf is None:
            return g, None
        return (buf if g is None else buf.add_(g)), None

# ... 1737 lines not shown
```

Baseline: 6.940 million subgraphs/s.

## Cache prepared DTW row pyramids and grouped values for fixed subgraph sets

Splits DTW into a prepare-rows step, which builds the x-side pyramid, and a similarity step that reads a prepared buffer through a header. This applies to both the heuristic and exact variants. When the x sets are fixed (per-split subgraph sets), the grouped values and prepared rows are cached on the row-prep object and reused across calls, with events handling cross-stream hand-off. The aim is to skip re-scattering and re-building the x pyramid every pass, at the cost of extra persistent memory and invalidation logic.

```diff
diff --git a/include/subgnn_hip.h b/include/subgnn_hip.h
--- a/include/subgnn_hip.h
+++ b/include/subgnn_hip.h
@@ -201,6 +201,19 @@
                              const int64_t* y_ptr, const int32_t* y_val, int64_t n_y, int64_t max_y_len,
                              int tie_order, int kernel, const int32_t* x_order, const int64_t* x_live_range, float* out,
                              void* workspace, int64_t workspace_bytes, void* stream);
+int64_t sgnn_dtw_rows_bytes(int64_t n_x, int64_t max_x_len);
+int64_t sgnn_dtw_rows_header_words(void);
+int64_t sgnn_dtw_rows_workspace_bytes(int64_t n_x, int64_t max_x_len, int64_t n_y, int64_t max_y_len);
+int sgnn_dtw_prepare_rows(const int64_t* x_ptr, const int32_t* x_val, int64_t n_x, int64_t max_x_len, int kernel,
+                          const int32_t* x_order, void* rows, int64_t rows_bytes, int64_t* header, void* stream);
+int sgnn_dtw_similarity_rows(const int64_t* rows_header, int64_t n_x, int64_t max_x_len,
+                             const int64_t* y_ptr, const int32_t* y_val, int64_t n_y, int64_t max_y_len,
+                             int tie_order, int kernel, const int32_t* x_order, float* out, void* workspace,
+                             int64_t workspace_bytes, void* stream);
+int sgnn_dtw_similarity_rows_live(const int64_t* rows_header, int64_t n_x, int64_t max_x_len,
+                                  const int64_t* y_ptr, const int32_t* y_val, int64_t n_y, int64_t max_y_len,
+                                  int tie_order, int kernel, const int32_t* x_order, const int64_t* x_live_range, float* out,
+                                  void* workspace, int64_t workspace_bytes, void* stream);
 
 int64_t sgnn_dtw_exact_workspace_bytes(int64_t n_x, int64_t max_x_len, int64_t n_y, int64_t max_y_len);
 int sgnn_dtw_exact_similarity(const int64_t* x_ptr, const int32_t* x_val, int64_t n_x, int64_t max_x_len,
@@ -211,6 +224,18 @@
                                    const int64_t* y_ptr, const int32_t* y_val, int64_t n_y, int64_t max_y_len,
                                    int kernel, const int32_t* x_order, const int64_t* x_live_range, float* out,
                                    void* workspace, int64_t workspace_bytes, void* stream);
+int64_t sgnn_dtwx_rows_bytes(int64_t n_x, int64_t max_x_len);
+int64_t sgnn_dtwx_rows_workspace_bytes(int64_t n_x, int64_t max_x_len, int64_t n_y, int64_t max_y_len);
+int sgnn_dtwx_prepare_rows(const int64_t* x_ptr, const int32_t* x_val, int64_t n_x, int64_t max_x_len, int kernel,
+                                const int32_t* x_order, void* rows, int64_t rows_bytes, int64_t* header, void* stream);
+int sgnn_dtwx_similarity_rows(const int64_t* rows_header, int64_t n_x, int64_t max_x_len,
+                                   const int64_t* y_ptr, const int32_t* y_val, int64_t n_y, int64_t max_y_len,
+                                   int kernel, const int32_t* x_order, float* out, void* workspace,
+                                   int64_t workspace_bytes, void* stream);
+int sgnn_dtwx_similarity_rows_live(const int64_t* rows_header, int64_t n_x, int64_t max_x_len,
+                                        const int64_t* y_ptr, const int32_t* y_val, int64_t n_y, int64_t max_y_len,
+                                        int kernel, const int32_t* x_order, const int64_t* x_live_range, float* out,
+                                        void* workspace, int64_t workspace_bytes, void* stream);
 
 #define SGNN_TOPK_DOT    0
 #define SGNN_TOPK_COSINE 1
diff --git a/subgnn_amd/SubGNN.py b/subgnn_amd/SubGNN.py
--- a/subgnn_amd/SubGNN.py
+++ b/subgnn_amd/SubGNN.py
@@ -180,17 +180,25 @@
                                                         self.test_sub_G_label.view(-1))))) + 1
         for sp in ('train', 'val', 'test'):
             setattr(self, sp + '_sub_G', [[n + 1 for n in sg] for sg in getattr(self, sp + '_sub_G')])
+        self._forget_split_caches()
         pre = torch.load(root / self.embedding_path, map_location='cpu')
         self.hparams['node_embed_size'] = pre.shape[1]
         table = torch.cat((torch.zeros(1, pre.shape[1]), pre.float()), 0)
         self.node_embeddings = nn.Embedding.from_pretrained(table, freeze=self.hparams['freeze_node_embeds'],
                                                             padding_idx=config.PAD_VALUE)
 
+    def _forget_split_caches(self):
+        from . import hotpath
+        hotpath.forget_split_facts(self)
+        for sp in ('train', 'val', 'test'):
+            self.__dict__.pop('_subs_' + sp, None)
+
     def _read_memory(self, mem):
         self.networkx_graph = mem['graph']
         for sp in ('train', 'val', 'test'):
             setattr(self, sp + '_sub_G', mem['sub_G'].get(sp, []))
             setattr(self, sp + '_sub_G_label', mem['labels'].get(sp, torch.zeros(0, dtype=torch.int64)))
+        self._forget_split_caches()
         self.multilabel, self.multilabel_binarizer = False, None
         self.num_classes = mem.get('num_classes') or int(max(int(l.max()) for l in mem['labels'].values() if l.numel() > 0)) + 1
         pre = mem['embeddings']
diff --git a/subgnn_amd/_lib.py b/subgnn_amd/_lib.py
--- a/subgnn_amd/_lib.py
+++ b/subgnn_amd/_lib.py
@@ -94,6 +94,21 @@
     'sgnn_dtw_order_keys': (c_int, [c_ptr, c_ptr, c_i64, c_ptr, c_ptr]),
     'sgnn_dtw_similarity_live': (c_int, [c_ptr, c_ptr, c_i64, c_i64, c_ptr, c_ptr, c_i64, c_i64, c_int, c_int, c_ptr, c_ptr, c_ptr,
                                          c_ptr, c_i64, c_ptr]),
+    'sgnn_dtw_rows_bytes': (c_i64, [c_i64, c_i64]),
+    'sgnn_dtw_rows_header_words': (c_i64, []),
+    'sgnn_dtw_rows_workspace_bytes': (c_i64, [c_i64, c_i64, c_i64, c_i64]),
+    'sgnn_dtw_prepare_rows': (c_int, [c_ptr, c_ptr, c_i64, c_i64, c_int, c_ptr, c_ptr, c_i64, c_ptr, c_ptr]),
+    'sgnn_dtw_similarity_rows': (c_int, [c_ptr, c_i64, c_i64, c_ptr, c_ptr, c_i64, c_i64, c_int, c_int, c_ptr, c_ptr, c_ptr,
+                                         c_i64, c_ptr]),
+    'sgnn_dtw_similarity_rows_live': (c_int, [c_ptr, c_i64, c_i64, c_ptr, c_ptr, c_i64, c_i64, c_int, c_int, c_ptr, c_ptr, c_ptr,
+                                              c_ptr, c_i64, c_ptr]),
+    'sgnn_dtwx_rows_bytes': (c_i64, [c_i64, c_i64]),
+    'sgnn_dtwx_rows_workspace_bytes': (c_i64, [c_i64, c_i64, c_i64, c_i64]),
+    'sgnn_dtwx_prepare_rows': (c_int, [c_ptr, c_ptr, c_i64, c_i64, c_int, c_ptr, c_ptr, c_i64, c_ptr, c_ptr]),
+    'sgnn_dtwx_similarity_rows': (c_int, [c_ptr, c_i64, c_i64, c_ptr, c_ptr, c_i64, c_i64, c_int, c_ptr, c_ptr, c_ptr,
+                                               c_i64, c_ptr]),
+    'sgnn_dtwx_similarity_rows_live': (c_int, [c_ptr, c_i64, c_i64, c_ptr, c_ptr, c_i64, c_i64, c_int, c_ptr, c_ptr, c_ptr,
+                                                    c_ptr, c_i64, c_ptr]),
     'sgnn_topk_max_k': (c_i64, []),
     'sgnn_topk_rows_workspace_bytes': (c_i64, [c_i64, c_i64, c_i64, c_i64]),
     'sgnn_topk_rows': (c_int, [c_ptr, c_i64, c_i64, c_ptr, c_i64, c_i64, c_i64, c_i64, c_int, c_ptr, c_ptr, c_ptr, c_i64, c_ptr,
diff --git a/subgnn_amd/csrc/dtw.hip b/subgnn_amd/csrc/dtw.hip
--- a/subgnn_amd/csrc/dtw.hip
+++ b/subgnn_amd/csrc/dtw.hip
@@ -799,34 +799,73 @@
     return SGNN_OK;
 }
 
-static int dtw_run(const int64_t* x_ptr, const int32_t* x_val, int64_t n_x, int64_t max_x_len,
-                   const int64_t* y_ptr, const int32_t* y_val, int64_t n_y, int64_t max_y_len,
-                   int tie_order, int kernel, const int32_t* x_order, const int64_t* x_live, float* out, void* workspace,
-                   int64_t workspace_bytes, void* stream)
-{
-    if (!x_ptr || !x_val || !y_ptr || !y_val || !out || !workspace || n_x < 0 || n_y < 0) return SGNN_ERR_BAD_ARG;
-    if (tie_order < 0 || tie_order > 2 || kernel < 0 || kernel > 1) return SGNN_ERR_BAD_ARG;
+#define DTW_ROWS_MAGIC 0x53474e4e44545752ll
+#define DTW_ROWS_HEAD 8
+enum { DTW_ROWS_ORDERED = 1, DTW_ROWS_NATURAL = 2 };
+
+static inline int64_t dtw_rows_bytes(int64_t n_x, const DtwLayout& L) { return 2 * n_x * L.XL * 8 + dtw_align8(n_x * 4); }
+static inline int dtw_rows_layout(int64_t max_x_len, int kernel, const int32_t* x_order) {
+    return (max_x_len <= DTW_R && kernel == 0 && x_order) ? DTW_ROWS_ORDERED : DTW_ROWS_NATURAL;
+}
+
+extern "C" int64_t sgnn_dtw_rows_bytes(int64_t n_x, int64_t max_x_len) {
     if (max_x_len < 1) max_x_len = 1;
-    if (max_y_len < 1) max_y_len = 1;
-    if (max_x_len > 32767 || max_y_len > 32767) return SGNN_ERR_SET_TOO_LARGE;
-    if (workspace_bytes < sgnn_dtw_workspace_bytes(n_x, max_x_len, n_y, max_y_len)) return SGNN_ERR_BAD_ARG;
-    if (n_x * n_y == 0) return SGNN_OK;
+    if (n_x < 0) n_x = 0;
+    return dtw_rows_bytes(n_x, dtw_layout(max_x_len, 1));
+}
+
+extern "C" int64_t sgnn_dtw_rows_header_words(void) { return DTW_ROWS_HEAD; }
+
+extern "C" int64_t sgnn_dtw_rows_workspace_bytes(int64_t n_x, int64_t max_x_len, int64_t n_y, int64_t max_y_len) {
+    return sgnn_dtw_workspace_bytes(n_x, max_x_len, n_y, max_y_len) - sgnn_dtw_rows_bytes(n_x, max_x_len);
+}
+
+static void dtw_prepare_rows(const int64_t* x_ptr, const int32_t* x_val, int64_t n_x, int64_t max_x_len, const DtwLayout& L,
+                             int layout, const int32_t* x_order, char* rows, hipStream_t st)
+{
+    double* xpyr = (double*)rows;
+    int32_t* xlen = (int32_t*)(rows + 2 * n_x * L.XL * 8);
+    dtw_launch_pyramid(x_ptr, x_val, n_x, max_x_len, L.XL, 1, xpyr, xpyr + n_x * L.XL, xlen,
+                       layout == DTW_ROWS_ORDERED ? x_order : (const int32_t*)nullptr, st);
+}
+
+extern "C" int sgnn_dtw_prepare_rows(const int64_t* x_ptr, const int32_t* x_val, int64_t n_x, int64_t max_x_len, int kernel,
+                                     const int32_t* x_order, void* rows, int64_t rows_bytes, int64_t* header, void* stream)
+{
+    if (!x_ptr || !x_val || !rows || !header || n_x < 0 || kernel < 0 || kernel > 1) return SGNN_ERR_BAD_ARG;
+    if (max_x_len < 1) max_x_len = 1;
+    if (max_x_len > 32767) return SGNN_ERR_SET_TOO_LARGE;
+    const DtwLayout L = dtw_layout(max_x_len, 1);
+    if (rows_bytes < dtw_rows_bytes(n_x, L)) return SGNN_ERR_BAD_ARG;
+    const int layout = dtw_rows_layout(max_x_len, kernel, x_order);
+    header[0] = 0;
+    if (n_x > 0) {
+        dtw_prepare_rows(x_ptr, x_val, n_x, max_x_len, L, layout, x_order, (char*)rows, (hipStream_t)stream);
+        SGNN_CHECK_LAUNCH();
+    }
+    header[1] = layout; header[2] = n_x; header[3] = max_x_len; header[4] = (int64_t)(intptr_t)rows; header[5] = rows_bytes;
+    header[6] = header[7] = 0;
+    header[0] = DTW_ROWS_MAGIC;
+    return SGNN_OK;
+}
+
+static int dtw_run_rows(const char* rows, int64_t n_x, int64_t max_x_len,
+                        const int64_t* y_ptr, const int32_t* y_val, int64_t n_y, int64_t max_y_len,
+                        int tie_order, int kernel, const int32_t* x_order, const int64_t* x_live, float* out, void* workspace,
+                        hipStream_t st)
+{
     const DtwLayout L = dtw_layout(max_x_len, max_y_len);
-    hipStream_t st = (hipStream_t)stream;
     char* w = (char*)workspace;
     const int64_t scratch = dtw_scratch_bytes(L);
     double* wd = (double*)w;
     int32_t* wi = (int32_t*)(w + DTW_NT * L.n_dbl * 8);
     uint32_t* wb = (uint32_t*)(w + DTW_NT * (L.n_dbl * 8 + dtw_align8(L.n_i32 * 4)));
     uint32_t* wq = (uint32_t*)w;           w += scratch;
-    double* xpyr = (double*)w;             w += 2 * n_x * L.XL * 8;
     double* ypyr = (double*)w;             w += 2 * n_y * L.YL * 8;
-    int32_t* xlen = (int32_t*)w;           w += dtw_align8(n_x * 4);
     int32_t* ylen = (int32_t*)w;
+    const double* xpyr = (const double*)rows;
+    const int32_t* xlen = (const int32_t*)(rows + 2 * n_x * L.XL * 8);
     const bool use_reg = max_x_len <= DTW_R && kernel == 0;
-    dtw_launch_pyramid(x_ptr, x_val, n_x, max_x_len, L.XL, 1, xpyr, xpyr + n_x * L.XL, xlen,
-                       use_reg ? x_order : (const int32_t*)nullptr, st);
-    SGNN_CHECK_LAUNCH();
     dtw_launch_pyramid(y_ptr, y_val, n_y, max_y_len, L.YL, 0, ypyr, ypyr + n_y * L.YL, ylen, (const int32_t*)nullptr, st);
     SGNN_CHECK_LAUNCH();
     if (use_reg) {
@@ -856,6 +895,45 @@
     return SGNN_OK;
 }
 
+static int dtw_run(const int64_t* x_ptr, const int32_t* x_val, int64_t n_x, int64_t max_x_len,
+                   const int64_t* y_ptr, const int32_t* y_val, int64_t n_y, int64_t max_y_len,
+                   int tie_order, int kernel, const int32_t* x_order, const int64_t* x_live, float* out, void* workspace,
+                   int64_t workspace_bytes, void* stream)
+{
+    if (!x_ptr || !x_val || !y_ptr || !y_val || !out || !workspace || n_x < 0 || n_y < 0) return SGNN_ERR_BAD_ARG;
+    if (tie_order < 0 || tie_order > 2 || kernel < 0 || kernel > 1) return SGNN_ERR_BAD_ARG;
+    if (max_x_len < 1) max_x_len = 1;
+    if (max_y_len < 1) max_y_len = 1;
+    if (max_x_len > 32767 || max_y_len > 32767) return SGNN_ERR_SET_TOO_LARGE;
+    if (workspace_bytes < sgnn_dtw_workspace_bytes(n_x, max_x_len, n_y, max_y_len)) return SGNN_ERR_BAD_ARG;
+    if (n_x * n_y == 0) return SGNN_OK;
+    const DtwLayout L = dtw_layout(max_x_len, max_y_len);
+    char* rows = (char*)workspace + sgnn_dtw_rows_workspace_bytes(n_x, max_x_len, n_y, max_y_len);
+    dtw_prepare_rows(x_ptr, x_val, n_x, max_x_len, L, dtw_rows_layout(max_x_len, kernel, x_order), x_order, rows, (hipStream_t)stream);
+    SGNN_CHECK_LAUNCH();
+    return dtw_run_rows(rows, n_x, max_x_len, y_ptr, y_val, n_y, max_y_len, tie_order, kernel, x_order, x_live, out, workspace,
+                        (hipStream_t)stream);
+}
+
+static int dtw_run_prepared(const int64_t* header, int64_t n_x, int64_t max_x_len,
+                            const int64_t* y_ptr, const int32_t* y_val, int64_t n_y, int64_t max_y_len,
+                            int tie_order, int kernel, const int32_t* x_order, const int64_t* x_live, float* out, void* workspace,
+                            int64_t workspace_bytes, void* stream)
+{
+    if (!header || !y_ptr || !y_val || !out || !workspace || n_x < 0 || n_y < 0) return SGNN_ERR_BAD_ARG;
+    if (tie_order < 0 || tie_order > 2 || kernel < 0 || kernel > 1) return SGNN_ERR_BAD_ARG;
+    if (max_x_len < 1) max_x_len = 1;
+    if (max_y_len < 1) max_y_len = 1;
+    if (max_x_len > 32767 || max_y_len > 32767) return SGNN_ERR_SET_TOO_LARGE;
+    if (header[0] != DTW_ROWS_MAGIC || header[2] != n_x || header[3] != max_x_len || !header[4]) return SGNN_ERR_BAD_ARG;
+    if (header[1] != dtw_rows_layout(max_x_len, kernel, x_order)) return SGNN_ERR_BAD_ARG;
+    if (header[5] < dtw_rows_bytes(n_x, dtw_layout(max_x_len, 1))) return SGNN_ERR_BAD_ARG;
+    if (workspace_bytes < sgnn_dtw_rows_workspace_bytes(n_x, max_x_len, n_y, max_y_len)) return SGNN_ERR_BAD_ARG;
+    if (n_x * n_y == 0) return SGNN_OK;
+    return dtw_run_rows((const char*)(intptr_t)header[4], n_x, max_x_len, y_ptr, y_val, n_y, max_y_len, tie_order, kernel, x_order,
+                        x_live, out, workspace, (hipStream_t)stream);
+}
+
 extern "C" int sgnn_dtw_similarity(const int64_t* x_ptr, const int32_t* x_val, int64_t n_x, int64_t max_x_len,
                                    const int64_t* y_ptr, const int32_t* y_val, int64_t n_y, int64_t max_y_len,
                                    int tie_order, int kernel, const int32_t* x_order, float* out, void* workspace,
@@ -875,4 +953,23 @@
                    workspace, workspace_bytes, stream);
 }
 
+extern "C" int sgnn_dtw_similarity_rows(const int64_t* rows_header, int64_t n_x, int64_t max_x_len,
+                                        const int64_t* y_ptr, const int32_t* y_val, int64_t n_y, int64_t max_y_len,
+                                        int tie_order, int kernel, const int32_t* x_order, float* out, void* workspace,
+                                        int64_t workspace_bytes, void* stream)
+{
+    return dtw_run_prepared(rows_header, n_x, max_x_len, y_ptr, y_val, n_y, max_y_len, tie_order, kernel, x_order, nullptr, out,
+                            workspace, workspace_bytes, stream);
+}
+
+extern "C" int sgnn_dtw_similarity_rows_live(const int64_t* rows_header, int64_t n_x, int64_t max_x_len,
+                                             const int64_t* y_ptr, const int32_t* y_val, int64_t n_y, int64_t max_y_len,
+                                             int tie_order, int kernel, const int32_t* x_order, const int64_t* x_live_range,
+                                             float* out, void* workspace, int64_t workspace_bytes, void* stream)
+{
+    if (x_live_range && !x_order) return SGNN_ERR_BAD_ARG;
+    return dtw_run_prepared(rows_header, n_x, max_x_len, y_ptr, y_val, n_y, max_y_len, tie_order, kernel, x_order, x_live_range,
+                            out, workspace, workspace_bytes, stream);
+}
+
 SGNN_DEFINE_WARM(dtw)
diff --git a/subgnn_amd/csrc/dtw_exact.hip b/subgnn_amd/csrc/dtw_exact.hip
--- a/subgnn_amd/csrc/dtw_exact.hip
+++ b/subgnn_amd/csrc/dtw_exact.hip
@@ -141,32 +141,66 @@
 #define DTWX_MINB20 2
 #define DTWX_MINB32 2
 
-static int dtw_exact_run(const int64_t* x_ptr, const int32_t* x_val, int64_t n_x, int64_t max_x_len,
-                         const int64_t* y_ptr, const int32_t* y_val, int64_t n_y, int64_t max_y_len,
-                         int kernel, const int32_t* x_order, const int64_t* x_live, float* out, void* workspace,
-                         int64_t workspace_bytes, void* stream)
-{
-    if (!x_ptr || !x_val || !y_ptr || !y_val || !out || !workspace || n_x < 0 || n_y < 0) return SGNN_ERR_BAD_ARG;
-    if (kernel < 0 || kernel > 1) return SGNN_ERR_BAD_ARG;
-    if (max_x_len < 1) max_x_len = 1;
-    if (max_y_len < 1) max_y_len = 1;
-    if (max_x_len > 32767 || max_y_len > 32767) return SGNN_ERR_SET_TOO_LARGE;
-    if (workspace_bytes < sgnn_dtw_exact_workspace_bytes(n_x, max_x_len, n_y, max_y_len)) return SGNN_ERR_BAD_ARG;
-    if (n_x * n_y == 0) return SGNN_OK;
-    hipStream_t st = (hipStream_t)stream;
-    const int64_t MX = max_x_len, MY = max_y_len;
+#define DTWX_ROWS_MAGIC 0x53474e4e44545758ll
+#define DTWX_ROWS_HEAD 8
+enum { DTWX_ROWS_ORDERED = 1, DTWX_ROWS_NATURAL = 2 };
+
+static inline int dtwx_rows_layout(int64_t MX, int kernel, const int32_t* x_order) {
+    return (MX <= DTWX_R && kernel == 0 && x_order) ? DTWX_ROWS_ORDERED : DTWX_ROWS_NATURAL;
+}
+
+extern "C" int64_t sgnn_dtwx_rows_bytes(int64_t n_x, int64_t max_x_len) {
+    if (max_x_len < 1) max_x_len = 1;
+    if (n_x < 0) n_x = 0;
+    return 2 * n_x * max_x_len * 8 + dtwx_align8(n_x * 4);
+}
+
+extern "C" int64_t sgnn_dtwx_rows_workspace_bytes(int64_t n_x, int64_t max_x_len, int64_t n_y, int64_t max_y_len) {
+    return sgnn_dtw_exact_workspace_bytes(n_x, max_x_len, n_y, max_y_len) - sgnn_dtwx_rows_bytes(n_x, max_x_len);
+}
+
+static void dtw_exact_prepare_rows(const int64_t* x_ptr, const int32_t* x_val, int64_t n_x, int64_t MX, int layout,
+                                   const int32_t* x_order, char* rows, hipStream_t st)
+{
+    double* xa = (double*)rows;
+    double* xr = xa + n_x * MX;
+    int32_t* xlen = (int32_t*)(rows + 2 * n_x * MX * 8);
+    hipLaunchKernelGGL(dtw_exact_prepare_kernel, dim3(sgnn_grid_for(n_x * MX, 256)), dim3(256), 0, st, x_ptr, x_val, n_x, MX, 1,
+                       xa, xr, xlen, layout == DTWX_ROWS_ORDERED ? x_order : (const int32_t*)nullptr);
+}
+
+extern "C" int sgnn_dtwx_prepare_rows(const int64_t* x_ptr, const int32_t* x_val, int64_t n_x, int64_t max_x_len, int kernel,
+                                           const int32_t* x_order, void* rows, int64_t rows_bytes, int64_t* header, void* stream)
+{
+    if (!x_ptr || !x_val || !rows || !header || n_x < 0 || kernel < 0 || kernel > 1) return SGNN_ERR_BAD_ARG;
+    if (max_x_len < 1) max_x_len = 1;
+    if (max_x_len > 32767) return SGNN_ERR_SET_TOO_LARGE;
+    if (rows_bytes < sgnn_dtwx_rows_bytes(n_x, max_x_len)) return SGNN_ERR_BAD_ARG;
+    const int layout = dtwx_rows_layout(max_x_len, kernel, x_order);
+    header[0] = 0;
+    if (n_x > 0) {
+        dtw_exact_prepare_rows(x_ptr, x_val, n_x, max_x_len, layout, x_order, (char*)rows, (hipStream_t)stream);
+        SGNN_CHECK_LAUNCH();
+    }
+    header[1] = layout; header[2] = n_x; header[3] = max_x_len; header[4] = (int64_t)(intptr_t)rows; header[5] = rows_bytes;
+    header[6] = header[7] = 0;
+    header[0] = DTWX_ROWS_MAGIC;
+    return SGNN_OK;
+}
+
+static int dtw_exact_run_rows(const char* rows, int64_t n_x, int64_t MX, const int64_t* y_ptr, const int32_t* y_val, int64_t n_y,
+                              int64_t MY, int kernel, const int32_t* x_order, const int64_t* x_live, float* out, void* workspace,
+                              hipStream_t st)
+{
     char* w = (char*)workspace;
     double* wd = (double*)w;               w += DTWX_NT * MX * 8;
-    double* xa = (double*)w;               w += n_x * MX * 8;
-    double* xr = (double*)w;               w += n_x * MX * 8;
     double* ya = (double*)w;               w += n_y * MY * 8;
     double* yr = (double*)w;               w += n_y * MY * 8;
-    int32_t* xlen = (int32_t*)w;           w += dtwx_align8(n_x * 4);
     int32_t* ylen = (int32_t*)w;
+    const double* xa = (const double*)rows;
+    const double* xr = xa + n_x * MX;
+    const int32_t* xlen = (const int32_t*)(rows + 2 * n_x * MX * 8);
     const bool use_reg = MX <= DTWX_R && kernel == 0;
-    hipLaunchKernelGGL(dtw_exact_prepare_kernel, dim3(sgnn_grid_for(n_x * MX, 256)), dim3(256), 0, st, x_ptr, x_val, n_x, MX, 1,
-                       xa, xr, xlen, use_reg ? x_order : (const int32_t*)nullptr);
-    SGNN_CHECK_LAUNCH();
     hipLaunchKernelGGL(dtw_exact_prepare_kernel, dim3(sgnn_grid_for(n_y * MY, 256)), dim3(256), 0, st, y_ptr, y_val, n_y, MY, 0,
                        ya, yr, ylen, (const int32_t*)nullptr);
     SGNN_CHECK_LAUNCH();
@@ -186,6 +220,45 @@
     return SGNN_OK;
 }
 
+static int dtw_exact_run(const int64_t* x_ptr, const int32_t* x_val, int64_t n_x, int64_t max_x_len,
+                         const int64_t* y_ptr, const int32_t* y_val, int64_t n_y, int64_t max_y_len,
+                         int kernel, const int32_t* x_order, const int64_t* x_live, float* out, void* workspace,
+                         int64_t workspace_bytes, void* stream)
+{
+    if (!x_ptr || !x_val || !y_ptr || !y_val || !out || !workspace || n_x < 0 || n_y < 0) return SGNN_ERR_BAD_ARG;
+    if (kernel < 0 || kernel > 1) return SGNN_ERR_BAD_ARG;
+    if (max_x_len < 1) max_x_len = 1;
+    if (max_y_len < 1) max_y_len = 1;
+    if (max_x_len > 32767 || max_y_len > 32767) return SGNN_ERR_SET_TOO_LARGE;
+    if (workspace_bytes < sgnn_dtw_exact_workspace_bytes(n_x, max_x_len, n_y, max_y_len)) return SGNN_ERR_BAD_ARG;
+    if (n_x * n_y == 0) return SGNN_OK;
+    char* rows = (char*)workspace + sgnn_dtwx_rows_workspace_bytes(n_x, max_x_len, n_y, max_y_len);
+    dtw_exact_prepare_rows(x_ptr, x_val, n_x, max_x_len, dtwx_rows_layout(max_x_len, kernel, x_order), x_order, rows,
+                           (hipStream_t)stream);
+    SGNN_CHECK_LAUNCH();
+    return dtw_exact_run_rows(rows, n_x, max_x_len, y_ptr, y_val, n_y, max_y_len, kernel, x_order, x_live, out, workspace,
+                              (hipStream_t)stream);
+}
+
+static int dtw_exact_run_prepared(const int64_t* header, int64_t n_x, int64_t max_x_len,
+                                  const int64_t* y_ptr, const int32_t* y_val, int64_t n_y, int64_t max_y_len,
+                                  int kernel, const int32_t* x_order, const int64_t* x_live, float* out, void* workspace,
+                                  int64_t workspace_bytes, void* stream)
+{
+    if (!header || !y_ptr || !y_val || !out || !workspace || n_x < 0 || n_y < 0) return SGNN_ERR_BAD_ARG;
+    if (kernel < 0 || kernel > 1) return SGNN_ERR_BAD_ARG;
+    if (max_x_len < 1) max_x_len = 1;
+    if (max_y_len < 1) max_y_len = 1;
+    if (max_x_len > 32767 || max_y_len > 32767) return SGNN_ERR_SET_TOO_LARGE;
+    if (header[0] != DTWX_ROWS_MAGIC || header[2] != n_x || header[3] != max_x_len || !header[4]) return SGNN_ERR_BAD_ARG;
+    if (header[1] != dtwx_rows_layout(max_x_len, kernel, x_order)) return SGNN_ERR_BAD_ARG;
+    if (header[5] < sgnn_dtwx_rows_bytes(n_x, max_x_len)) return SGNN_ERR_BAD_ARG;
+    if (workspace_bytes < sgnn_dtwx_rows_workspace_bytes(n_x, max_x_len, n_y, max_y_len)) return SGNN_ERR_BAD_ARG;
+    if (n_x * n_y == 0) return SGNN_OK;
+    return dtw_exact_run_rows((const char*)(intptr_t)header[4], n_x, max_x_len, y_ptr, y_val, n_y, max_y_len, kernel, x_order, x_live,
+                              out, workspace, (hipStream_t)stream);
+}
+
 extern "C" int sgnn_dtw_exact_similarity(const int64_t* x_ptr, const int32_t* x_val, int64_t n_x, int64_t max_x_len,
                                          const int64_t* y_ptr, const int32_t* y_val, int64_t n_y, int64_t max_y_len,
                                          int kernel, const int32_t* x_order, float* out, void* workspace,
@@ -205,4 +278,23 @@
                          workspace, workspace_bytes, stream);
 }
 
+extern "C" int sgnn_dtwx_similarity_rows(const int64_t* rows_header, int64_t n_x, int64_t max_x_len,
+                                              const int64_t* y_ptr, const int32_t* y_val, int64_t n_y, int64_t max_y_len,
+                                              int kernel, const int32_t* x_order, float* out, void* workspace,
+                                              int64_t workspace_bytes, void* stream)
+{
+    return dtw_exact_run_prepared(rows_header, n_x, max_x_len, y_ptr, y_val, n_y, max_y_len, kernel, x_order, nullptr, out,
+                                  workspace, workspace_bytes, stream);
+}
+
+extern "C" int sgnn_dtwx_similarity_rows_live(const int64_t* rows_header, int64_t n_x, int64_t max_x_len,
+                                                   const int64_t* y_ptr, const int32_t* y_val, int64_t n_y, int64_t max_y_len,
+                                                   int kernel, const int32_t* x_order, const int64_t* x_live_range, float* out,
+                                                   void* workspace, int64_t workspace_bytes, void* stream)
+{
+    if (x_live_range && !x_order) return SGNN_ERR_BAD_ARG;
+    return dtw_exact_run_prepared(rows_header, n_x, max_x_len, y_ptr, y_val, n_y, max_y_len, kernel, x_order, x_live_range, out,
+                                  workspace, workspace_bytes, stream);
+}
+
 SGNN_DEFINE_WARM(dtw_exact)
diff --git a/subgnn_amd/hotpath.py b/subgnn_amd/hotpath.py
--- a/subgnn_amd/hotpath.py
+++ b/subgnn_amd/hotpath.py
@@ -243,6 +243,7 @@
         self.per_split = {}
         self.sim_cols = None
         self.dtw_inputs = None
+        self.x_fixed = False
         self.bfs_checks = []
         self.pool_reused = False
 
@@ -275,31 +276,51 @@
     else:
         side = main
     t.mark('start')
-    subs = ops.Ragged.from_lists(getattr(model, split + '_sub_G'), dev) if not hasattr(model, '_subs_' + split) \
-        else getattr(model, '_subs_' + split)
-    setattr(model, '_subs_' + split, subs)
-    labels = ops.cc_labels(g, subs)
-    kept = model.__dict__.setdefault('_cc_dims', {})
-    tag = (id(getattr(model, split + '_sub_G')), subs.n)
-    hit = kept.get(split)
-    cc_ids = subgraph_utils.components_from_labels(subs.ptr, subs.nodes, labels, subs.max_len,
-                                                   dims_reduce=shard.reduce_max if shard is not None else None,
-                                                   dims=hit[1] if hit is not None and hit[0] == tag else None)
-    kept[split] = (tag, tuple(cc_ids.shape[1:]))
+    sub_g = getattr(model, split + '_sub_G')
+    srcs = model.__dict__.setdefault('_subs_src', {})
+    if not hasattr(model, '_subs_' + split) or srcs.get(split, sub_g) is not sub_g or getattr(model, '_subs_' + split).n != len(sub_g):
+        setattr(model, '_subs_' + split, ops.Ragged.from_lists(sub_g, dev))
+    srcs[split] = sub_g
+    subs = getattr(model, '_subs_' + split)
+    keep_facts = bool(hp.get('keep_split_facts', True))
+    facts = _split_facts(model, split, sub_g, subs.n, g, shard) if keep_facts else None
+    facts_new = keep_facts and facts is None and not torch.cuda.is_current_stream_capturing()
+    once = '(first pass only)' if facts_new else ''
+    det = bool(getattr(model, '_deterministic', ops.DETERMINISTIC))
+    if facts is not None:
+        facts.wait(main)
+        cc_ids, cc_sets, real = facts.cc_ids, facts.cc_sets, facts.real
+        S, C, Lc = cc_ids.shape
+    else:
+        labels = ops.cc_labels(g, subs)
+        kept = model.__dict__.setdefault('_cc_dims', {})
+        tag = (id(sub_g), subs.n)
+        hit = kept.get(split)
+        cc_ids = subgraph_utils.components_from_labels(subs.ptr, subs.nodes, labels, subs.max_len,
+                                                       dims_reduce=shard.reduce_max if shard is not None else None,
+                                                       dims=hit[1] if hit is not None and hit[0] == tag else None)
+        kept[split] = (tag, tuple(cc_ids.shape[1:]))
+        S, C, Lc = cc_ids.shape
     st.attrs[split + '_cc_ids'] = cc_ids
-    S, C, Lc = cc_ids.shape
-    if getattr(model, '_deterministic', ops.DETERMINISTIC):
+    if det:
         mo = model.__dict__.setdefault('_cc_member_order', {})
+        if facts_new:
+            mo.pop(split, None)
         if mo.get(split) is None or mo[split][0].numel() != cc_ids.numel():
             mo[split] = ops.sort_edges_by_key(cc_ids.reshape(-1).to(torch.int32), g.max_id)
         cc_ids._sgnn_member_order = mo[split]
-    cc_ids._sgnn_ids32 = cc_ids.reshape(-1).to(torch.int32)
+    elif getattr(cc_ids, '_sgnn_member_order', None) is not None:
+        del cc_ids._sgnn_member_order
     base = shard.start if shard is not None else 0
-    cc_sets = ops.Ragged.from_padded(cc_ids.reshape(S * C, Lc))
-    real = (cc_ids[:, :, 0] != 0)
-    cc_ids._sgnn_mask = real
-    cc_ids._sgnn_mask_u8 = real.reshape(-1).to(torch.uint8)
-    t.mark('components')
+    if facts is None:
+        cc_ids._sgnn_ids32 = cc_ids.reshape(-1).to(torch.int32)
+        cc_sets = ops.Ragged.from_padded(cc_ids.reshape(S * C, Lc))
+        real = (cc_ids[:, :, 0] != 0)
+        cc_ids._sgnn_mask = real
+        cc_ids._sgnn_mask_u8 = real.reshape(-1).to(torch.uint8)
+        if facts_new:
+            facts = _keep_split_facts(model, split, SplitFacts(sub_g, subs.n, g, shard, cc_ids, cc_sets, real))
+        t.mark('components' + once)
     orders = model.__dict__.setdefault('_degseq_order', {})
     if orders.get(split) is None or orders[split].numel() != cc_sets.n:
         orders[split] = ops.heaviest_first(g, cc_sets)
@@ -307,8 +328,9 @@
     set_order = orders[split]
     sims = {}
     a_sets = ai = ae = None
-    det = bool(getattr(model, '_deterministic', ops.DETERMINISTIC))
     side.wait_stream(main)
+    if facts is not None and side is not main:
+        facts.wait(side)
     with torch.cuda.stream(side):
         new_patches = hp['use_structure'] and pool is None and (split != 'test' or getattr(model, 'structure_anchors', None) is None)
         structure_anchors = getattr(model, 'structure_anchors', None) if pool is None else pool['structure_anchors']
@@ -431,8 +453,14 @@
             t.mark('S_patches_walks')
     if hp['use_neighborhood']:
         k = hp['neigh_sample_border_size']
-        has_pad_c = (cc_sets.lengths < Lc).to(torch.uint8)
-        cc_canon = ops.sort_ragged(cc_sets)
+        if facts is not None and facts.cc_canon is not None:
+            has_pad_c, cc_canon = facts.has_pad_c, facts.cc_canon
+        else:
+            has_pad_c = (cc_sets.lengths < Lc).to(torch.uint8)
+            cc_canon = ops.sort_ragged(cc_sets)
+            if facts is not None and not torch.cuda.is_current_stream_capturing():
+                facts.has_pad_c, facts.cc_canon = has_pad_c, cc_canon
+                facts.built()
         ni, nb, plans = {}, {}, {}
         border = _kept_border(model, split, subs, cc_sets, k)
         for l in range(L):
@@ -470,10 +498,17 @@
         st.per_split['_mpn_edge_plans'] = plans
         t.mark('border_bfs+N_anchors')
     ci = ce = None
+    x_fixed = False
     if hp['use_structure'] and pool is None:
-        ci, ce = ops.degree_sequence(g, cc_sets, sort=True, use_degree_dict=g.full_degree is not None,
-                                     order=set_order)
-        t.mark('degree_sequences')
+        if facts is not None and facts.ci is not None:
+            ci, ce, x_fixed = facts.ci, facts.ce, True
+        else:
+            ci, ce = ops.degree_sequence(g, cc_sets, sort=True, use_degree_dict=g.full_degree is not None,
+                                         order=set_order)
+            if facts is not None and not torch.cuda.is_current_stream_capturing():
+                facts.ci, facts.ce, x_fixed = ci, ce, True
+                facts.built()
+            t.mark('degree_sequences' + once)
     if hp['use_structure'] and side is not main:
         main.wait_event(patch_ev)
         _hand_over(main, structure_anchors)
@@ -485,6 +520,7 @@
             structure_walks()
             t.mark('S_walks')
     st.dtw_inputs = (cc_sets, ci, ce, a_sets, ai, ae, (S, C)) if (hp['use_structure'] and pool is None) else None
+    st.x_fixed = x_fixed
     if pool is not None and hp['use_structure']:
         st.attrs[split + '_int_struc_similarities'], st.attrs[split + '_bor_struc_similarities'] = pool['int_sims'], pool['bor_sims']
     if late_bfs:
@@ -509,6 +545,88 @@
     return st
 
 
+class SplitFacts:
+
+    def __init__(self, sub_g, n, graph, shard, cc_ids, cc_sets, real):
+        self.sub_g, self.n, self.graph = sub_g, n, graph
+        self.shard_key = self.shard_key_of(shard)
+        self.cc_ids, self.cc_sets, self.real = cc_ids, cc_sets, real
+        self.has_pad_c = self.cc_canon = self.ci = self.ce = None
+        self.ready, self._waited = None, set()
+        self.built()
+
+    @staticmethod
+    def shard_key_of(shard):
+        return None if shard is None else (int(shard.start), int(shard.world))
+
+    def matches(self, sub_g, n, graph, shard):
+        return self.sub_g is sub_g and self.n == n and len(sub_g) == n and self.graph is graph \
+            and self.shard_key == self.shard_key_of(shard)
+
+    def tensors(self):
+        cc = self.cc_ids
+        out = [cc, self.real, self.has_pad_c, self.ci, self.ce, self.cc_sets.ptr, self.cc_sets.nodes]
+        out += [getattr(cc, nm, None) for nm in ('_sgnn_ids32', '_sgnn_mask_u8')]
+        if self.cc_canon is not None:
+            out += [self.cc_canon.ptr, self.cc_canon.nodes]
+        return [t for t in out if t is not None]
+
+    @property
+    def nbytes(self):
+        seen = {}
+        for t in self.tensors():
+            seen[t.data_ptr()] = t.numel() * t.element_size()
+        return sum(seen.values())
+
+    def built(self):
+        if not self.cc_ids.is_cuda:
+            return
+        self.ready = torch.cuda.Event()
+        self.ready.record()
+        self._waited = {torch.cuda.current_stream().cuda_stream}
+
+    def wait(self, stream):
+        key = stream.cuda_stream
+        if key in self._waited or torch.cuda.is_current_stream_capturing():
+            return
+        self._waited.add(key)
+        for t in self.tensors():
+            t.record_stream(stream)
+        if not self.ready.query():
+            stream.wait_event(self.ready)
+
+
+def _split_facts(model, split, sub_g, n, graph, shard):
+    facts = model.__dict__.get('_split_facts', {}).get(split)
+    return facts if facts is not None and facts.matches(sub_g, n, graph, shard) else None
+
+
+def _keep_split_facts(model, split, facts):
+    kept = model.__dict__.setdefault('_split_facts', {})
+    if kept.get(split) is not None:
+        for name in ('_dtw_group_rows', '_degseq_order'):
+            model.__dict__.get(name, {}).pop(split, None)
+        widths = model.__dict__.get('_border_width', {})
+        for k in [k for k in widths if k[0] == split]:
+            widths.pop(k)
+    kept[split] = facts
+    return facts
+
+
+def forget_split_facts(model, split=None):
+    kept = model.__dict__.get('_split_facts')
+    if kept:
+        for sp in ([split] if split is not None else list(kept)):
+            kept.pop(sp, None)
+
+
+def split_facts_bytes(model, split='train'):
+    facts = model.__dict__.get('_split_facts', {}).get(split)
+    rec = model.__dict__.get('_dtw_group_rows', {}).get(split)
+    return (facts.nbytes if facts is not None else 0,
+            sum(s.prep.nbytes for s in (rec.internal, rec.external)) if rec is not None else 0)
+
+
 KEPT_BORDER_BYTES = 4 << 30
 
 
@@ -549,7 +667,8 @@
         elif rec.internal.group is None and not torch.cuda.is_current_stream_capturing():
             _settle_dtw_grouping(model, split, wait=False)
         for name, side, x, y in (('_int', rec.internal, ci, ai), ('_bor', rec.external, ce, ae)):
-            sim = ops.dtw_similarity(cc_sets.ptr, x, mx, a_sets.ptr, y, my, tie, dedupe=bool(side.group), x_prep=side.prep, fn=fn)
+            sim = ops.dtw_similarity(cc_sets.ptr, x, mx, a_sets.ptr, y, my, tie, dedupe=bool(side.group), x_prep=side.prep, fn=fn,
+                                     x_fixed=st.x_fixed)
             st.attrs[split + name + '_struc_similarities'] = sim.view(S, C, -1)
         t.mark('dtw')
     elif split + '_int_struc_similarities' not in st.attrs:
diff --git a/subgnn_amd/ops.py b/subgnn_amd/ops.py
--- a/subgnn_amd/ops.py
+++ b/subgnn_amd/ops.py
@@ -964,22 +964,78 @@
     'dtw': ('sgnn_dtw_workspace_bytes', 'sgnn_dtw_similarity', True),
     'dtw_exact': ('sgnn_dtw_exact_workspace_bytes', 'sgnn_dtw_exact_similarity', False),
 }
+_DTW_ROWS_ENTRIES = {
+    'dtw': ('sgnn_dtw_rows_bytes', 'sgnn_dtw_prepare_rows', 'sgnn_dtw_rows_workspace_bytes', 'sgnn_dtw_similarity_rows'),
+    'dtw_exact': ('sgnn_dtwx_rows_bytes', 'sgnn_dtwx_prepare_rows', 'sgnn_dtwx_rows_workspace_bytes', 'sgnn_dtwx_similarity_rows'),
+}
 DTW_FNS = tuple(_DTW_ENTRIES)
 
+
+class DtwRows:
+    __slots__ = ('buf', 'header', 'key', 'nbytes')
+
+    def __init__(self, buf, header, key, nbytes):
+        self.buf, self.header, self.key, self.nbytes = buf, header, key, nbytes
+
+    @property
+    def header_ptr(self):
+        return ctypes.addressof(self.header)
+
+
+def dtw_prepare_rows(x_ptr, x_val, max_x, kernel=0, fn='dtw', order=None, key=None):
+    lib = _lib.load()
+    _req(x_ptr, torch.int64, 'x_ptr')
+    _req(x_val, torch.int32, 'x_val')
+    size_q, entry = _DTW_ROWS_ENTRIES[fn][:2]
+    nx = x_ptr.numel() - 1
+    nbytes = getattr(lib, size_q)(nx, max_x)
+    buf = torch.empty(nbytes // 8 + 1, dtype=torch.int64, device=x_ptr.device)
+    header = (ctypes.c_int64 * int(lib.sgnn_dtw_rows_header_words()))()
+    check(getattr(lib, entry)(_ptr(x_ptr), _ptr(x_val), nx, max_x, int(kernel), _ptr(order), _ptr(buf), nbytes,
+                              ctypes.addressof(header), _stream()), entry)
+    return DtwRows(buf, header, key, nbytes)
+
 DtwGrouping = collections.namedtuple('DtwGrouping', 'ptr rep entry_dst live')
 
 
 class DtwRowPrep:
-    __slots__ = ('shape', 'grouping', 'order', 'grouped_order')
+    __slots__ = ('shape', 'grouping', 'order', 'grouped_order', 'grouped_val', 'rows', 'fixed_src', 'ready', '_waited')
 
     def __init__(self):
-        self.shape = self.grouping = self.order = self.grouped_order = None
-
-    def fit(self, x_ptr, x_val):
+        self.shape = None
+        self.forget()
+
+    def forget(self):
+        self.grouping = self.order = self.grouped_order = self.grouped_val = self.rows = self.fixed_src = self.ready = None
+        self._waited = set()
+
+    def fit(self, x_ptr, x_val, fixed=False):
         shape = (x_ptr.numel() - 1, x_val.numel())
-        if shape != self.shape:
-            self.shape, self.grouping, self.order, self.grouped_order = shape, None, None, None
+        if shape != self.shape or (fixed and self.fixed_src is not None and self.fixed_src is not x_val):
+            self.shape = shape
+            self.forget()
+        if fixed:
+            self.fixed_src = x_val
         return self
+
+    @property
+    def nbytes(self):
+        return (self.rows.nbytes if self.rows is not None else 0) + (self.grouped_val.numel() * 4 if self.grouped_val is not None else 0)
+
+    def built(self):
+        self.ready = torch.cuda.Event()
+        self.ready.record()
+        self._waited = {torch.cuda.current_stream().cuda_stream}
+
+    def hand_over(self, stream):
+        if self.ready is None or stream.cuda_stream in self._waited or torch.cuda.is_current_stream_capturing():
+            return
+        self._waited.add(stream.cuda_stream)
+        for t in (self.grouped_val, self.rows.buf if self.rows is not None else None, self.order, self.grouped_order):
+            if t is not None:
+                t.record_stream(stream)
+        if not self.ready.query():
+            stream.wait_event(self.ready)
 
 
 def _group_rows(x_ptr, x_val, max_x, want_live):
@@ -1007,7 +1063,7 @@
     return torch.argsort(key).to(torch.int32).contiguous()
 
 
-def _dtw_launch(x_ptr, x_val, max_x, y_ptr, y_val, max_y, tie_order, kernel, fn, order, live):
+def _dtw_launch(x_ptr, x_val, max_x, y_ptr, y_val, max_y, tie_order, kernel, fn, order, live, rows=None):
     lib = _lib.load()
     for t, dt, nm in ((x_ptr, torch.int64, 'x_ptr'), (y_ptr, torch.int64, 'y_ptr'), (x_val, torch.int32, 'x_val'),
                       (y_val, torch.int32, 'y_val')):
@@ -1015,9 +1071,11 @@
     nx, ny = x_ptr.numel() - 1, y_ptr.numel() - 1
     out = (torch.empty if live is None else torch.zeros)((nx, ny), dtype=torch.float32, device=x_ptr.device)
     ws_entry, entry, takes_tie = _DTW_ENTRIES[fn]
+    if rows is not None:
+        ws_entry, entry = _DTW_ROWS_ENTRIES[fn][2:]
     wsb = getattr(lib, ws_entry)(nx, max_x, ny, max_y)
     ws = torch.empty(wsb // 8 + 1, dtype=torch.int64, device=x_ptr.device)
-    args = [_ptr(x_ptr), _ptr(x_val), nx, max_x, _ptr(y_ptr), _ptr(y_val), ny, max_y]
+    args = ([_ptr(x_ptr), _ptr(x_val)] if rows is None else [rows.header_ptr]) + [nx, max_x, _ptr(y_ptr), _ptr(y_val), ny, max_y]
     if takes_tie:
         args.append(tie_order)
     args += [int(kernel), _ptr(order)]
@@ -1029,17 +1087,26 @@
 
 
 def dtw_similarity(x_ptr, x_val, max_x, y_ptr, y_val, max_y, tie_order=None, order_rows=True, dedupe=True, order=None,
-                   x_prep=None, kernel=0, fn='dtw'):
+                   x_prep=None, kernel=0, fn='dtw', x_fixed=False):
     if fn not in DTW_FNS:
         raise ValueError('structure similarity function %r: one of %s' % (fn, ', '.join(map(repr, DTW_FNS))))
     if tie_order is None:
         from .config import DTW_TIE_ORDER as tie_order
-    prep = (x_prep if x_prep is not None else DtwRowPrep()).fit(x_ptr, x_val)
+    fixed = bool(x_fixed) and x_prep is not None and order is None
+    prep = (x_prep if x_prep is not None else DtwRowPrep()).fit(x_ptr, x_val, fixed)
+    keep = fixed and not torch.cuda.is_current_stream_capturing()
+    if fixed:
+        prep.hand_over(torch.cuda.current_stream())
+    built = False
     ptr, val, g = x_ptr, x_val, None
     if dedupe and x_ptr.numel() - 1 > 1024 and max_x <= 64:
         g = prep.grouping = prep.grouping or _group_rows(x_ptr, x_val, max_x, order is None and order_rows)
-        ptr, val = g.ptr, torch.zeros(x_val.numel() + 1, dtype=torch.int32, device=x_ptr.device)
-        val.scatter_(0, g.entry_dst, x_val)
+        ptr, val = g.ptr, prep.grouped_val if fixed else None
+        if val is None:
+            val = torch.zeros(x_val.numel() + 1, dtype=torch.int32, device=x_ptr.device)
+            val.scatter_(0, g.entry_dst, x_val)
+            if keep:
+                prep.grouped_val, built = val, True
     live = g.live if g is not None and order is None else None
     if order is not None:
         order = order.to(torch.int32).contiguous()
@@ -1049,7 +1116,16 @@
         if order is None:
             order = _dtw_row_order(ptr, val)
             setattr(prep, which, order)
-    out = _dtw_launch(ptr, val, max_x, y_ptr, y_val, max_y, int(tie_order), kernel, fn, order, live)
+    rows = None
+    if fixed:
+        key = (fn, int(kernel), int(max_x), g is not None)
+        rows = prep.rows if prep.rows is not None and prep.rows.key == key else None
+        if rows is None and keep:
+            rows = prep.rows = dtw_prepare_rows(ptr, val, max_x, kernel, fn, order, key)
+            built = True
+    if built:
+        prep.built()
+    out = _dtw_launch(ptr, val, max_x, y_ptr, y_val, max_y, int(tie_order), kernel, fn, order, live, rows)
     return out if g is None else out.index_select(0, g.rep)
 
 
```

Measured after the change: 7.434 million subgraphs/s (median of 6 runs). 7.1% higher.
